# timsainb/noisereduce

Measured on AMD Instinct MI355X. Metric: Msamples/s reduce_noise (48 kHz mono, n_fft=1024), higher is better.
Workload: dtype f32

## Files before the change

include/mi355gate_debug.h:

```cpp
#ifndef MI355GATE_DEBUG_H
#define MI355GATE_DEBUG_H

#include "mi355gate.h"

#ifdef __cplusplus
extern "C" {
#endif

SG_API int sg_debug_dims(const sg_handle* h, int64_t dims[3]);
SG_API int sg_debug_range(const sg_handle* h, int64_t range[2]);
SG_API int sg_debug_counter(sg_handle* h, int32_t which, int64_t* value, void* stream);
SG_API int sg_debug_fetch(sg_handle* h, int32_t what, void* host, int64_t bytes, void* stream);

SG_API int sg_debug_clip_thresholds(sg_handle* h, double* host, int32_t n_noise, int32_t n_bins, void* stream);
SG_API int sg_debug_clip_batches(const sg_handle* h, int64_t* value);
SG_API int sg_debug_rows_batches(const sg_handle* h, int64_t* value);
#define SG_BWD_ROW 1
#define SG_BWD_FAST 2
#define SG_BWD_REG 3
#define SG_BWD_OLA 4
#define SG_BWD_ROWS 5
SG_API int sg_debug_backward_route(const sg_handle* h, int64_t* value);

#define SG_OPT_FORCE_UNFUSED 1
#define SG_OPT_FORCE_F64_DECIDE 3
#define SG_OPT_FORCE_NOSEAM 4
#define SG_OPT_FORCE_NOLEAN 5
#define SG_OPT_FORCE_SPLIT 6
#define SG_OPT_INJECT_HANDOFF_FAULT 7
#define SG_OPT_FORCE_NOROWGATE 10
#define SG_OPT_ROWGATE_TAP 11
#define SG_OPT_ROWGATE_SHAPE 12
#define SG_OPT_FLOOR_TEST 13
#define SG_OPT_TILE_ORDER 15
#define SG_OPT_EXACT_MATERIALISED 16
#define SG_OPT_FORCE_NOFAST 2

#define SG_STAGE_CHANNEL_MEAN 0
#define SG_STAGE_STFT_POWER 1
#define SG_STAGE_COLMAX 2
#define SG_STAGE_COLSTATS 3
#define SG_STAGE_DECIDE 4
#define SG_STAGE_STFT_MAG 5
#define SG_STAGE_NONSTAT_MASK 6
#define SG_STAGE_SMOOTH 7
#define SG_STAGE_APPLY_ISTFT 8
#define SG_STAGE_OLA 9
#define SG_STAGE_NOISE_STATS 10
#define SG_STAGE_PREP 11
#define SG_STAGE_STFT_MAX 12
#define SG_STAGE_STFT_BITS 13
#define SG_STAGE_APPLY_FAST 14
#define SG_STAGE_DECIDE_FAST 15
#define SG_STAGE_ONEPASS 16
#define SG_STAGE_ROW_GATE 17
#define SG_STAGE_IIR_CHAIN 18
#define SG_STAGE_IIR_MASK 19
#define SG_STAGE_RG_NOISE_POWER 20
#define SG_STAGE_RG_NOISE_FINAL 21
#define SG_STAGE_RG_DECIDE 22
#define SG_STAGE_RG_IIR 23
#define SG_STAGE_RG_FSMOOTH 24
#define SG_STAGE_RG_APPLY 25
#define SG_STAGE_RG_OLA 26
#define SG_N_STAGES 27
#define SG_STAGE_ST_EXPORT 27
#define SG_STAGE_ST_IMPORT 28
#define SG_N_STAGES_ALL 29
SG_API int sg_profile_enable(sg_handle* h, int32_t on);
SG_API int sg_profile_select(sg_handle* h, int64_t stage_mask);
SG_API int sg_profile_read(sg_handle* h, double* ms, int64_t* counts, int32_t n_stages, int32_t reset);
SG_API const char* sg_stage_name(int32_t stage);

#ifdef __cplusplus
}
#endif
#endif
```

noisereduce_amd/_ffi.py:

```python
import contextlib
import ctypes
import os
import threading
import weakref
from ctypes import (POINTER, Structure, byref, c_char_p, c_double, c_int, c_int32,
                    c_int64, c_void_p)

import numpy as np
import torch

_HERE = os.path.dirname(os.path.abspath(__file__))
LIB_PATH = os.path.join(_HERE, "libmi355gate.so")

SG_F32, SG_F64, SG_I16, SG_I32 = 0, 1, 2, 3
SG_VARIANT_S, SG_VARIANT_T = 0, 1
SG_E_INVALID, SG_E_UNSUPPORTED, SG_E_HIP, SG_E_NOMEM, SG_E_STATE, SG_E_HANDOFF = -1, -2, -3, -4, -5, -6
SG_N_STAGES = 27
SG_N_STAGES_ALL = 29
SG_OPT_FORCE_F64_DECIDE = 3
SG_OPT_FORCE_NOSEAM = 4
SG_OPT_FORCE_NOLEAN = 5
SG_OPT_FORCE_SPLIT = 6
SG_OPT_INJECT_HANDOFF_FAULT = 7
SG_OPT_FAST_INTEGER = 8
SG_OPT_FORCE_EXACT = 9
SG_OPT_FORCE_NOROWGATE = 10
SG_OPT_ROWGATE_TAP = 11
SG_OPT_ROWGATE_SHAPE = 12
SG_OPT_FLOOR_TEST = 13
SG_OPT_TILE_ORDER = 15
SG_OPT_EXACT_MATERIALISED = 16
SG_OPT_FORCE_UNFUSED = 1
SG_OPT_FORCE_NOFAST = 2
SG_BWD_ROW, SG_BWD_FAST, SG_BWD_REG, SG_BWD_OLA, SG_BWD_ROWS = 1, 2, 3, 4, 5

_TORCH_DTYPES = {torch.float32: SG_F32, torch.float64: SG_F64, torch.int16: SG_I16,
                 torch.int32: SG_I32}


class HandoffTimeout(RuntimeError):
    """SG_E_HANDOFF: a bounded inter-workgroup wait of a fused kernel timed out (the device was preempted for
    about a second); the outputs of the calls enqueued since the last check are invalid and must be re-run."""


class SgParams(Structure):
    _fields_ = [
        ("variant", c_int32), ("stationary", c_int32), ("n_fft", c_int32),
        ("win_length", c_int32), ("hop_length", c_int32), ("n_grad_freq", c_int32),
        ("n_grad_time", c_int32), ("smooth_mask", c_int32), ("chunk_size", c_int64),
        ("padding", c_int64), ("prop_decrease", c_double), ("n_std_thresh", c_double),
        ("top_db", c_double), ("ddof", c_int32), ("n_movemean", c_int32),
        ("nonstat_thresh", c_double), ("nonstat_slope", c_double), ("iir_b", c_double),
        ("max_workspace_bytes", c_int64),
    ]


class SgClip(Structure):
    _fields_ = [("x_offset", c_int64), ("n", c_int64), ("x_stride", c_int64), ("channels", c_int32),
                ("noise", c_int32), ("out_offset", c_int64), ("out_stride", c_int64)]


class SgNoiseSrc(Structure):
    _fields_ = [("offset", c_int64), ("n", c_int64), ("stride", c_int64), ("channels", c_int32), ("in_x", c_int32)]


class SgStreamRec(Structure):
    _fields_ = [("slot", c_int32), ("flush", c_int32), ("n_samples", c_int64), ("in_offset", c_int64),
                ("in_stride", c_int64), ("out_offset", c_int64), ("out_stride", c_int64)]


SG_STREAM_FIXED, SG_STREAM_NONSTATIONARY, SG_STREAM_ADAPTIVE = 0, 1, 2


class SgStreamDesc(Structure):
    _fields_ = [("n_slots", c_int32), ("channels", c_int32), ("max_block", c_int64), ("kind", c_int32),
                ("lookahead_frames", c_int32), ("forget", c_double), ("learn_frames", c_int64), ("exact", c_int32)]


SG_STREAM_HEAD_MAGIC, SG_STREAM_HEAD_VERSION = 0x54534753, 1


class SgStreamHead(Structure):
    _fields_ = [("magic", c_int32), ("version", c_int32), ("n_fft", c_int32), ("win_length", c_int32),
                ("hop_length", c_int32), ("channels", c_int32), ("kind", c_int32), ("n_grad_freq", c_int32),
# ... 707 lines not shown
```

noisereduce_amd/csrc/api.hip:

```cpp
#include <hip/hip_runtime.h>
#include <dlfcn.h>

#include <algorithm>
#include <cmath>
#include <cstdarg>
#include <cstdio>
#include <cstring>
#include <map>
#include <mutex>
#include <string>
#include <vector>

#include "../../include/mi355gate_debug.h"
#pragma clang fp contract(on)
#include "kernels.hpp"
#include "fused.hpp"
#include "czt.hpp"
#include "mixed.hpp"
#include "onepass.hpp"
#include "rowgate.hpp"
#include "rowbwd.hpp"
#include "fast512.hpp"
#include "onepass512.hpp"
#include "fast256.hpp"
// ... 11 lines not shown

#ifndef SG_TEAM_N
#define SG_TEAM_N 2048
#endif
#ifndef SG_SHORT_TEAMS
#define SG_SHORT_TEAMS 1
#endif
#ifndef SG_CHAIN_PAR
#define SG_CHAIN_PAR 1
#if OP_WHO
static unsigned* g_who_dev = nullptr;
#endif
#if OP_TRACE
static unsigned* g_trace_dev = nullptr;
static size_t g_trace_tiles = 0;
static int g_trace_ntt = 1;
#endif
#endif
#ifndef SG_STATS_TEAM
#define SG_STATS_TEAM 1
#endif
template <int N>
constexpr int team_threads() {
  return N >= SG_TEAM_N ? 256 : (!SG_SHORT_TEAMS ? 64 : (N <= 128 ? 16 : (N == 256 ? 32 : 64)));
}
template <int N>
constexpr int team_count(size_t elem) {
  return N >= SG_TEAM_N ? 1 : (team_threads<N>() < 64 ? 256 / team_threads<N>() : ((N * elem > 16384) ? 2 : 4));
}
#ifndef SG_APPLY_WAVES
#define SG_APPLY_WAVES 4
#endif

using namespace sg;

namespace {
thread_local std::string g_create_error;

struct DevBuf {
  void* p = nullptr;
  size_t bytes = 0;
};

std::string fmt(const char* f, ...) {
  char buf[512];
  va_list ap;
  va_start(ap, f);
  vsnprintf(buf, sizeof buf, f, ap);
  va_end(ap);
  return buf;
}
}

struct RegGeom;
struct sg_handle {
  sg_params p{};
  int n = 0, N = 0, W = 0, H = 0, F = 0, FS = 0, padL = 0;
  double sum_w = 0.0;
  double mag_scale = 1;
  DevBuf tw64, tw32, wfull64, wa32, ws32, wsq32, kf, kt;
  DevBuf thresh;
  bool has_thresh = false;
  DevBuf P, pmax, thr_rows, raw, M, seg, yn;
  DevBuf bits, K16, umax, need, T2;
  DevBuf nss;
  DevBuf alim;
  bool t2_ready = false;
  DevBuf logtab;
  DevBuf part;
  DevBuf tw512, invn;
  DevBuf seam;
  DevBuf ftab;
  int sm2_tt = 64;
  bool t_sm2_ok = true;
  DevBuf xbits, xpart, xticket, xtick2, ftab3, xexp, optab;
  DevBuf xin;
  DevBuf nsp, nsc;
  unsigned* err_host = nullptr;
  unsigned* err_dev = nullptr;
  unsigned inject_fault = 0;
  unsigned lose_now = 0;
  unsigned ticket_base = 0;
  unsigned epoch = 0;
  bool fast_integer = false;
  bool force_exact = false;
  bool exact_materialised = false;
  DevBuf norm64;
  unsigned need_era = 0;
  DevBuf xP, xraw, xM, xtmp, xseg;
  bool force_split = false;
  int rowgate_mode = 0;
  int64_t n_floor_lazy = 0, n_floor_apriori = 0;
  int tile_order = 0;
  int n_cu = 0;
  int floor_test = 0;
  int rg_shape = 16;
  bool rg_tap = false;
  bool dbg_rg = false;
  int dbg_bwd_route = 0;
  DevBuf rg_count;
  bool dbg_xbits = false;
  int dbg_trows = 16, dbg_tstep = 16, dbg_twords = 0, dbg_txw = 9;
  int64_t dbg_tf0 = 0;
  int dbg_ntt = 0;
  int big_M = 0;
  int big_czt = 0;
  DevBuf big_twM, big_tw2, big_ch, big_bh, big_W, big_W2;
  int czt_M = 0;
  bool mr_ok = false;
  MrPlan mr{};
  DevBuf mr_pt32, mr_pt64;
  DevBuf regtab;
  DevBuf czt_tw64, czt_ch64, czt_bh64, czt_tw32, czt_ch32, czt_bh32;
  bool force_noseam = false;
  bool force_nolean = false;
  bool fast_ok = false;
  const RegGeom* reg = nullptr;
  bool force_nofast = false;
  bool force_f64_decide = false;
  int64_t ktot = 1;
  bool fused_ok = false;
  double sum_abs_w = 0.0;
  int64_t dbg_units = 0, dbg_T = 0;
  bool dbg_has_P = false;
  bool dbg_has_raw = true;
  bool dbg_fused = false;
  bool dbg_fast = false;
  bool dbg_k16_only = false;
  Geom dbg_g{};
  int64_t dbg_db = 0, dbg_de = 0;
  bool force_unfused = false;
  bool roctx_on = false;
  bool prof_on = false;
  uint64_t prof_mask = ~0ull;
  int prof_override = -1;
// ... 95 lines not shown
    (void)hipEventCreate(&e);
    return e;
  }
  bool ranged = false;
  ProfScope(sg_handle* h_, int stage, hipStream_t st_) : h(h_), st(st_) {
    if (h->roctx_on && roctx().push) {
      roctx().push(sg_stage_name(h->prof_override >= 0 ? h->prof_override : stage));
      ranged = true;
    }
    if (!h->prof_on) return;
    const int booked = h->prof_override >= 0 ? h->prof_override : stage;
    if (!((h->prof_mask >> booked) & 1ull)) return;
    sg_handle::ProfRec r{h->prof_override >= 0 ? h->prof_override : stage, get(h), get(h)};
    (void)hipEventRecord(r.a, st);
    h->prof_live.push_back(r);
    idx = (int)h->prof_live.size() - 1;
  }
  ~ProfScope() {
    if (idx >= 0) (void)hipEventRecord(h->prof_live[idx].b, st);
    if (ranged) roctx().pop();
  }
};
}

#define HIPCHK(h, call)                                                                      \
  do {                                                                                       \
    hipError_t e_ = (call);                                                                  \
    if (e_ != hipSuccess) {                                                                  \
      (h)->err = fmt("%s failed: %s (%s:%d)", #call, hipGetErrorString(e_), __FILE__, __LINE__); \
      (void)hipGetLastError();  \
      return SG_E_HIP;                                                                       \
    }                                                                                        \
  } while (0)

#define FAIL(h, code, ...)      \
  do {                          \
    (h)->err = fmt(__VA_ARGS__); \
    return (code);              \
  } while (0)

static hipError_t set_lds(const void* kern, size_t bytes) {
  static std::mutex mu;
  static std::map<std::pair<int, const void*>, size_t> done;
  int dev = 0;
  (void)hipGetDevice(&dev);
  std::lock_guard<std::mutex> lk(mu);
  size_t& have = done[{dev, kern}];
  if (have >= bytes) return hipSuccess;
  hipError_t e = hipFuncSetAttribute(kern, hipFuncAttributeMaxDynamicSharedMemorySize, (int)bytes);
  if (e == hipSuccess) have = bytes;
  return e;
}

static int ensure(sg_handle* h, DevBuf& b, size_t bytes) {
  if (b.bytes >= bytes) return SG_OK;
  if (b.p) {
    HIPCHK(h, hipDeviceSynchronize());
    HIPCHK(h, hipFree(b.p));
    b.p = nullptr;
    b.bytes = 0;
  }
  hipError_t e = hipMalloc(&b.p, bytes);
  if (e != hipSuccess) {
    b.p = nullptr;
    FAIL(h, SG_E_NOMEM, "workspace allocation of %zu bytes failed: %s", bytes, hipGetErrorString(e));
  }
  b.bytes = bytes;
  return SG_OK;
}

static int ensure_zeroed(sg_handle* h, DevBuf& b, size_t bytes, hipStream_t st, bool* fresh = nullptr) {
  const bool grow = b.bytes < bytes;
  int rc = ensure(h, b, bytes);
  if (rc) return rc;
  if (fresh) *fresh = grow;
  if (grow) HIPCHK(h, hipMemsetAsync(b.p, 0, b.bytes, st));
  return SG_OK;
}

static int upload(sg_handle* h, DevBuf& b, const void* src, size_t bytes) {
  int rc = ensure(h, b, bytes);
  if (rc) return rc;
  HIPCHK(h, hipMemcpy(b.p, src, bytes, hipMemcpyHostToDevice));
  return SG_OK;
}

static void free_buf(DevBuf& b) {
  if (b.p) (void)hipFree(b.p);
  b.p = nullptr;
  b.bytes = 0;
}

static int64_t frames_for(const sg_handle* h, int64_t L) {
  if (h->p.variant == SG_VARIANT_S) return (L + 2 * (int64_t)(h->W / 2) - h->W) / h->H + 1;
  return 1 + (L + 2 * (int64_t)(h->n / 2) - h->n) / h->H;
}
static int64_t outlen_for(const sg_handle* h, int64_t L) {
  int64_t T = frames_for(h, L);
  if (h->p.variant == SG_VARIANT_S) return (T - 1) * h->H + h->W - 2 * (int64_t)(h->W / 2);
  return (T - 1) * (int64_t)h->H + (h->n - 2 * (int64_t)(h->n / 2));
}

static Geom make_geom(const sg_handle* h, int64_t Lp) {
  Geom g;
  g.n = h->n; g.W = h->W; g.H = h->H; g.F = h->F; g.FS = h->FS; g.padL = h->padL;
  g.T = frames_for(h, Lp);
  g.Lout = outlen_for(h, Lp);
  return g;
}
// ... 779 lines not shown
          {&h->tw512, fast::OP_TAB_TW512, 4096}, {&h->tw32, fast::OP_TAB_TW1024, 4096}, {&h->wfull64, fast::OP_TAB_WIN64, 8192},
          {&h->tw64, fast::OP_TAB_TW64, 8192}, {&h->ftab3, fast::OP_TAB_MCONST, 1536}, {&h->xexp, fast::OP_TAB_EXP8, 2048}};
      for (const auto& pt : parts) {
        if (!pt.b->p || pt.b->bytes < pt.bytes) { h->err = "one-pass table arena: a source table is missing"; rc = SG_E_STATE; break; }
        if (hipMemcpy((char*)h->optab.p + pt.off, pt.b->p, pt.bytes, hipMemcpyDeviceToDevice) != hipSuccess) {
          h->err = "one-pass table arena: hipMemcpy failed"; rc = SG_E_HIP; break;
        }
      }
    }
  }
  const RegGeom* rg = h->reg;
  if (!rc && rg && p->smooth_mask && p->n_grad_freq <= rg->op.max_nf && p->n_grad_time <= rg->op.max_nt) {
    const int nf = p->n_grad_freq, nt = p->n_grad_time;
    auto wt = [&](int d) { const int ad = d < 0 ? -d : d; return ad <= nt ? nt + 1 - ad : 0; };
    auto wf = [&](int d) { const int ad = d < 0 ? -d : d; return ad <= nf ? nf + 1 - ad : 0; };
    const bool two = rg == &REG2048;
    const int ex = 64 * (two ? 3 : 1 + rg->tab_kb);
    std::vector<unsigned long long> tb(ex + 256, 0ull);
    for (int l = 0; l < 64; ++l) {
      const int q = l / 16, j = l % 16;
      for (int e = 0; e < 8; ++e) {
        const int k = 8 * q + e;
        const int r1 = e < 4 ? 4 * q + e : 16 + 4 * q + (e - 4);
        if (two) {
          tb[l] |= (unsigned long long)wf(k - 24 - j) << (8 * e);
          tb[64 + l] |= (unsigned long long)wf(k + 8 - j) << (8 * e);
          tb[128 + l] |= (unsigned long long)wt(r1 - nt - j) << (8 * e);
        } else {
          tb[l] |= (unsigned long long)wf(k - 8 - j) << (8 * e);
          for (int b = 0; b < rg->tab_kb; ++b) tb[64 * (1 + b) + l] |= (unsigned long long)wt(32 * b + r1 - nt - j) << (8 * e);
        }
      }
    }
    for (int v = 0; v < 256; ++v)
      for (int e = 0; e < 8; ++e) tb[ex + v] |= (unsigned long long)((v >> e) & 1) << (8 * e);
    rc = upload(h, h->regtab, tb.data(), tb.size() * 8);
  }
  if (!rc) rc = ensure(h, h->thresh, (size_t)h->FS * sizeof(double));
  if (rc) {
    g_create_error = h->err;
    sg_destroy(h);
    return rc;
  }
  *out = h;
  return SG_OK;
}

extern "C" int sg_destroy(sg_handle* h) {
  if (!h) return SG_OK;
  (void)hipDeviceSynchronize();
  for (auto& r : h->prof_live) { (void)hipEventDestroy(r.a); (void)hipEventDestroy(r.b); }
  for (auto e : h->prof_pool) (void)hipEventDestroy(e);
  if (h->err_host) (void)hipHostFree(h->err_host);
  for (DevBuf* b : {&h->tw64, &h->tw32, &h->wfull64, &h->wa32, &h->ws32, &h->wsq32, &h->kf, &h->kt, &h->thresh,
                    &h->P, &h->pmax, &h->thr_rows, &h->raw, &h->M, &h->seg, &h->yn, &h->bits, &h->K16, &h->umax,
                    &h->need, &h->T2, &h->part, &h->tw512, &h->invn, &h->seam, &h->ftab, &h->xbits, &h->xpart,
                    &h->xticket, &h->xtick2, &h->ftab3, &h->xexp, &h->optab, &h->nsp, &h->nsc, &h->xin, &h->czt_tw64, &h->czt_ch64,
                    &h->czt_bh64, &h->czt_tw32, &h->czt_ch32, &h->czt_bh32, &h->logtab, &h->big_twM, &h->big_tw2,
                    &h->big_ch, &h->big_bh, &h->big_W, &h->big_W2, &h->xP, &h->xraw, &h->xM, &h->xtmp, &h->xseg, &h->rg_count, &h->alim, &h->nss, &h->mr_pt32, &h->mr_pt64, &h->regtab})
    free_buf(*b);
  sg::rg_free(h->rg);
  sg::rw_free(h->rw);
  delete h;
  return SG_OK;
}

extern "C" int sg_n_frames(const sg_handle* h, int64_t L, int64_t* n_frames) {
  if (!h || !n_frames) return SG_E_INVALID;
  *n_frames = frames_for(h, L);
  return SG_OK;
}
extern "C" int sg_output_length(const sg_handle* h, int64_t L, int64_t* out_len) {
  if (!h || !out_len) return SG_E_INVALID;
  *out_len = outlen_for(h, L);
  return SG_OK;
}

static int64_t ws_budget(const sg_handle* h) {
  return h->p.max_workspace_bytes > 0 ? h->p.max_workspace_bytes : (int64_t)8 << 30;
}

static size_t unit_bytes(const sg_handle* h, const Geom& g, bool lean) {
  size_t cells = (size_t)g.T * g.FS;
  if (lean) return (size_t)g.T * ((g.F + 63) / 64) * 8 + cells * 2 + (size_t)g.FS * 16 + 64 +
           (size_t)(g.T / 16 + 2) * 6 * 256 * 4;
  return cells * (8 + 4 + 4 + 2) + (size_t)g.T * g.n * 4 + (size_t)g.FS * 16 +
         (size_t)(g.T / NS_TT + 1) * 2 * g.FS * 8 * 2 +
         (size_t)(g.T / 8 + 1) * 2 * g.FS * 8;
}

static int64_t units_per_batch(const sg_handle* h, const Geom& g, int64_t total, bool lean = false) {
  int64_t ub = ws_budget(h) / (int64_t)unit_bytes(h, g, lean);
  ub = std::max<int64_t>(1, std::min<int64_t>(ub, 32768));
  return std::min(ub, total);
}

static int ensure_ws(sg_handle* h, const Geom& g, int64_t ub, bool lean = false) {
  size_t cells = (size_t)ub * g.T * g.FS;
  int rc;
  if (!lean) {
    if ((rc = ensure(h, h->P, cells * 8))) return rc;
    if ((rc = ensure(h, h->raw, cells * 4))) return rc;
    if ((rc = ensure(h, h->M, cells * 4))) return rc;
    if ((rc = ensure(h, h->seg, std::max((size_t)ub * g.T * g.n * 4, cells * 4)))) return rc;
  }
  if ((rc = ensure(h, h->pmax, (size_t)ub * g.FS * 8))) return rc;
  if ((rc = ensure(h, h->thr_rows, (size_t)ub * g.FS * 8))) return rc;
// ... 4 lines not shown
#define SG_STAT_SLICES_MAX 64
#endif
#ifndef SG_STAT_FRAMES_PER_SLICE
#define SG_STAT_FRAMES_PER_SLICE 36
#endif
static int stat_slices(const Geom& g, int64_t ub) {
  int64_t blocks = (int64_t)((g.F + 63) / 64) * ub;
  int64_t nts = (2048 + blocks - 1) / blocks;
  nts = std::max<int64_t>(1, std::min<int64_t>(nts, std::min<int64_t>(SG_STAT_SLICES_MAX, std::max<int64_t>(1, g.T / 16))));
  return (int)nts;
}

static int stage_power(sg_handle* h, const View& v, const Geom& g, int64_t ub, hipStream_t st) {
  if (ub >= 16) {
    HIPCHK(h, hipMemsetAsync(h->pmax.p, 0, (size_t)ub * g.FS * 8, st));
    ProfScope ps(h, SG_STAGE_STFT_POWER, st);
    HIPCHK(h, stft_any<double>(h, v, g, ub, (double*)h->P.p, nullptr, nullptr, 1.0, st,
                               (unsigned long long*)h->pmax.p));
    return SG_OK;
  }
  {
    ProfScope ps(h, SG_STAGE_STFT_POWER, st);
    HIPCHK(h, stft_any<double>(h, v, g, ub, (double*)h->P.p, nullptr, nullptr, 1.0, st));
  }
  ProfScope ps(h, SG_STAGE_COLMAX, st);
  const int nts = stat_slices(g, ub);
  int rc = ensure(h, h->part, (size_t)ub * nts * 2 * g.FS * 8);
  if (rc) return rc;
  dim3 grid((g.F + 63) / 64, (unsigned)ub, nts);
  hipLaunchKernelGGL(k_colmax, grid, dim3(64 * STAT_TG), 0, st, (const double*)h->P.p, g, (double*)h->part.p);
  HIPCHK(h, hipGetLastError());
  hipLaunchKernelGGL(k_colmax_final, dim3(grid_1d(ub * g.FS, 256)), dim3(256), 0, st, (const double*)h->part.p, g,
                     nts, (double*)h->pmax.p, ub);
  HIPCHK(h, hipGetLastError());
  return SG_OK;
}

static int stage_colstats(sg_handle* h, const Geom& g, int64_t ub, double* thresh_out, hipStream_t st) {
  ProfScope ps(h, SG_STAGE_COLSTATS, st);
  const int nts = stat_slices(g, ub);
  int rc = ensure(h, h->part, (size_t)ub * nts * 2 * g.FS * 8);
  if (rc) return rc;
  dim3 grid((g.F + 63) / 64, (unsigned)ub, nts);
  hipLaunchKernelGGL(k_colstats, grid, dim3(64 * STAT_TG), 0, st, (const double*)h->P.p, g,
                     (const double*)h->pmax.p, h->mag_scale, h->p.top_db, (double*)h->part.p);
  HIPCHK(h, hipGetLastError());
  hipLaunchKernelGGL(k_colstats_final, dim3(grid_1d(ub * g.FS, 256)), dim3(256), 0, st,
                     (const double*)h->part.p, g, nts, (const double*)h->pmax.p, h->mag_scale,
                     h->p.n_std_thresh, h->p.ddof, thresh_out, ub);
  HIPCHK(h, hipGetLastError());
  return SG_OK;
}

static int stage_stats(sg_handle* h, const View& v, const Geom& g, int64_t ub, double* thresh_out, hipStream_t st,
                       bool gate_consts = false) {
  if (ub < 16) {
    {
      ProfScope ps(h, SG_STAGE_STFT_POWER, st);
      HIPCHK(h, stft_any<double>(h, v, g, ub, (double*)h->P.p, nullptr, nullptr, 1.0, st));
    }
    ProfScope ps(h, SG_STAGE_COLSTATS, st);
    const int nts = (int)std::max<int64_t>(1, std::min<int64_t>(std::min(stat_slices(g, ub), STAT_TG * STAT1_MAXS), g.T / SG_STAT_FRAMES_PER_SLICE));
    int rc = ensure(h, h->part, (size_t)ub * nts * STAT1_NP * g.FS * 8);
    if (rc) return rc;
    dim3 grid((g.F + 63) / 64, (unsigned)ub, nts);
    hipLaunchKernelGGL(k_colstats1, grid, dim3(64 * STAT_TG), 0, st, (const double*)h->P.p, g, h->mag_scale,
                       (double*)h->part.p, db_fast_consts(h));
    HIPCHK(h, hipGetLastError());
    GateConsts gc{};
    if (gate_consts && ub == 1 && grid.x <= 62) {
      if ((rc = ensure(h, h->T2, (size_t)g.FS * 8))) return rc;
      if ((rc = ensure_zeroed(h, h->alim, 256, st))) return rc;
      gc.T2 = (double*)h->T2.p; gc.alim_b = (unsigned*)h->alim.p + 2; gc.sum_abs_w = h->sum_abs_w;
    }
    hipLaunchKernelGGL(k_colstats1_final, dim3((unsigned)((g.FS + 63) / 64), (unsigned)ub), dim3(64 * STAT_TG), 0, st,
                       (const double*)h->part.p, (const double*)h->P.p, g, nts, h->mag_scale, h->p.top_db,
                       h->p.n_std_thresh, h->p.ddof, (double*)h->pmax.p, thresh_out, gc);
    HIPCHK(h, hipGetLastError());
    if (gc.T2 != nullptr) h->t2_ready = true;
    return SG_OK;
  }
  int rc = stage_power(h, v, g, ub, st);
  if (rc) return rc;
  return stage_colstats(h, g, ub, thresh_out, st);
}

static int stage_decide(sg_handle* h, const Geom& g, int64_t ub, const double* thresh, int64_t ustride,
                        hipStream_t st) {
  ProfScope ps(h, SG_STAGE_DECIDE, st);
  int64_t cells = ub * g.T * g.FS;
  hipLaunchKernelGGL(k_decide, dim3(grid_1d(cells, 256)), dim3(256), 0, st, (const double*)h->P.p, g,
                     (const double*)h->pmax.p, thresh, ustride, h->mag_scale, h->p.top_db, (float*)h->raw.p, ub);
  HIPCHK(h, hipGetLastError());
  return SG_OK;
}

static int handoff_prepare(sg_handle* h, hipStream_t st);
static int handoff_next_epoch(sg_handle* h, hipStream_t st);
static int stage_prep_floor(sg_handle* h, const View& v, const Geom& g, int64_t ub, ThreshConsts* tc_out, hipStream_t st,
                            const View* v_exact, unsigned* live_host, unsigned stamp);
template <int MODE>
static hipError_t launch_bits_any(const sg_handle* h, const View& v, const Geom& g, int64_t units, const ThreshConsts& tc,
                                  unsigned long long* pmax_bits, unsigned long long* bits, int wpr, hipStream_t st);

static fast::RegArgs reg_args(const sg_handle* h, const RegGeom* r, const View& v, const Geom& g) {
  fast::RegArgs A{};
  A.view = v; A.g = g;
  A.win = (const float*)h->wa32.p;
  A.win64 = (const double*)h->wfull64.p;
  A.tw = (const fast::cf*)(h->*r->tw).p;
  A.tw64 = (const cx<double>*)h->tw64.p;
  A.mag_scale = h->mag_scale; A.top_db = h->p.top_db;
  A.wsq = (const float*)h->wsq32.p;
  A.invn = (const float*)h->invn.p;
  return A;
}

template <typename ARGS>
static hipError_t reg_launch(void (*kern)(ARGS), dim3 grid, size_t lds, hipStream_t st, const ARGS& A) {
  hipError_t e = set_lds(reinterpret_cast<const void*>(kern), lds);
  if (e != hipSuccess) return e;
  hipLaunchKernelGGL(kern, grid, dim3(256), lds, st, A);
  return hipGetLastError();
}

static int stage_decide_reg(sg_handle* h, const RegGeom* r, const View& v, const Geom& g, int64_t ub, const ThreshConsts& tc,
                            unsigned long long* bits, hipStream_t st, const FloorLazy& fl = FloorLazy{}, bool redo = false) {
  ProfScope ps(h, redo ? SG_STAGE_STFT_MAX : SG_STAGE_DECIDE_FAST, st);
  fast::RegArgs A = reg_args(h, r, v, g);
  A.tc = tc;
  A.bits = bits;
  A.fl = fl;
  HIPCHK(h, reg_launch(r->decide[redo], dim3((unsigned)((g.T + r->frames - 1) / r->frames), (unsigned)ub), r->lds, st, A));
// ... 10 lines not shown
  HIPCHK(h, reg_launch(r->mag, dim3((unsigned)((g.T + r->frames - 1) / r->frames), (unsigned)ub), r->lds, st, A));
  return SG_OK;
}

static int launch_seam(sg_handle* h, const RegGeom* r, const fast::RegArgs& A, int64_t ub, hipStream_t st) {
  if (A.n_tiles < 2) return SG_OK;
  fast::SeamArgs S{};
  S.view = A.view; S.g = A.g; S.om = A.om; S.h_begin = A.h_begin; S.h_end = A.h_end; S.normalize = A.normalize;
  S.invn = A.invn; S.wsq = A.wsq; S.part = A.part; S.n_tiles = A.n_tiles;
  hipLaunchKernelGGL(r->seam, dim3((unsigned)(A.n_tiles - 1), (unsigned)ub), dim3(r->hop), 0, st, S);
  HIPCHK(h, hipGetLastError());
  return SG_OK;
}

static int reg_seam_tiles(sg_handle* h, const RegGeom* r, int64_t hb, int64_t he, int64_t ub, fast::RegArgs* A) {
  const int64_t tiles = (he - hb + 3 + r->frames - 1) / r->frames;
  int rc = ensure(h, h->seam, (size_t)ub * tiles * 6 * r->hop * sizeof(float));
  if (rc) return rc;
  A->part = (float*)h->seam.p;
  A->n_tiles = (int)tiles;
  return SG_OK;
}

static int stage_apply_reg(sg_handle* h, const RegGeom* r, const View& v, const Geom& g, int64_t ub, const OutMap& om,
                           const float* mask_f ,
                           int normalize, hipStream_t st) {
  ProfScope ps(h, SG_STAGE_APPLY_FAST, st);
  fast::RegArgs A = reg_args(h, r, v, g);
  A.Mf = mask_f;
  A.K = (const unsigned short*)h->K16.p;
  A.inv_ktot = (float)(1.0 / (double)h->ktot);
  A.om = om;
  A.normalize = normalize;
  A.h_begin = (om.p0 + g.padL) / r->hop;
  A.h_end = (om.p1 - 1 + g.padL) / r->hop + 1;
  const int64_t nh = A.h_end - A.h_begin;
  if (nh <= 0) return SG_OK;
  const int64_t tiles = (nh + 3 + r->frames - 1) / r->frames;
  const bool seam = tiles >= 2 && !h->force_noseam;
  A.n_tiles = (int)tiles;
  int rc;
  if (seam && (rc = reg_seam_tiles(h, r, A.h_begin, A.h_end, ub, &A))) return rc;
  const dim3 grid((unsigned)(seam ? tiles : (nh + r->hops - 1) / r->hops), (unsigned)ub);
  HIPCHK(h, reg_launch(r->apply[mask_f == nullptr], grid, r->lds, st, A));
  if (seam) return launch_seam(h, r, A, ub, st);
  return SG_OK;
}

struct FloorSetup {
  bool lazy = false;
  ThreshConsts tc{};
  FloorLazy fl{};
};
static int floor_setup(sg_handle* h, const Geom& g, int64_t ub, int nb, hipStream_t st, FloorSetup* out) {
  int rc;
  if ((rc = handoff_prepare(h, st))) return rc;
  const unsigned live_stamp = h->err_host[1];
  const unsigned need_tag = h->epoch & 0x3fffffffu;
  const unsigned era = h->epoch >> 30;
  if (era != h->need_era || need_tag == 0u) {
    if (h->need.p) HIPCHK(h, hipMemsetAsync(h->need.p, 0, h->need.bytes, st));
    if (h->alim.p) HIPCHK(h, hipMemsetAsync((char*)h->alim.p + 4, 0, 4, st));
    h->need_era = era;
  }
  FloorSetup f;
  f.lazy = need_tag != 0u &&
           (h->floor_test == 2 || (h->floor_test == 0 && !(live_stamp != 0u && h->epoch - live_stamp <= 16u)));
  if (f.lazy) {
    const int wpr = (g.F + 63) / 64;
    if ((rc = ensure(h, h->bits, (size_t)ub * g.T * wpr * 8))) return rc;
    if ((rc = ensure_zeroed(h, h->need, (size_t)ub * 4, st))) return rc;
    if ((rc = ensure(h, h->T2, (size_t)g.FS * 8))) return rc;
    if ((rc = ensure_zeroed(h, h->alim, 256, st))) return rc;
    if (!h->t2_ready) {
      ProfScope ps(h, SG_STAGE_PREP, st);
      hipLaunchKernelGGL(k_prep_thresh_lazy, dim3(1), dim3(256), 0, st, (const double*)h->thresh.p, g.F, h->mag_scale,
                         h->sum_abs_w, h->p.top_db, (double*)h->T2.p, (unsigned*)h->alim.p, nb);
      HIPCHK(h, hipGetLastError());
      h->t2_ready = true;
    }
    f.tc = ThreshConsts{(const double*)h->T2.p, (const double*)h->thresh.p, (const double*)h->pmax.p, (const int*)h->need.p,
                        need_tag};
    f.fl = FloorLazy{(unsigned*)h->alim.p, nb, h->err_dev + 1, h->epoch};
  }
  *out = f;
  return SG_OK;
}

static bool onepass_small_ok(const sg_handle* h, const Geom& g, const OutMap& om, const OnePassSmall& S, const DevBuf& tab) {
  if (h->force_nofast || h->force_split || h->force_f64_decide || h->force_unfused || !h->fused_ok) return false;
  if (h->p.variant != SG_VARIANT_S || !h->p.stationary || !h->p.smooth_mask) return false;
  if (h->p.n_grad_freq > S.max_nf || h->p.n_grad_time > S.max_nt || g.F != S.F || !tab.p) return false;
  if (h->tile_order == 1) return false;
  const int64_t hb = (om.p0 + g.padL) / S.hop, he = (om.p1 - 1 + g.padL) / S.hop + 1;
  return he > hb;
}
template <typename LAUNCH>
static int stage_onepass_small(sg_handle* h, const View& v, const View& vx, const Geom& g, int64_t ub, const OutMap& om,
                               hipStream_t st, const OnePassSmall& S, fast::OnePassRegArgs P, const DevBuf& tab, LAUNCH launch) {
  int rc;
  FloorSetup fs;
  if ((rc = floor_setup(h, g, ub, (g.FS + 63) / 64, st, &fs))) return rc;
  const bool lazy = fs.lazy;
  ++(lazy ? h->n_floor_lazy : h->n_floor_apriori);
  const int wpr = (g.F + 63) / 64;
  if (!lazy && (rc = stage_prep_floor(h, v, g, ub, &fs.tc, st, &vx, h->err_dev + 1, h->epoch))) return rc;
  const ThreshConsts& tc = fs.tc;
  P.A.tc = tc;
  P.A.fl = fs.fl;
  P.A.inv_ktot = (float)(1.0 / (double)h->ktot);
  P.A.om = om;
  P.A.normalize = 1;
  P.A.h_begin = (om.p0 + g.padL) / S.hop;
  P.A.h_end = (om.p1 - 1 + g.padL) / S.hop + 1;
  const int64_t nh = P.A.h_end - P.A.h_begin;
  const int64_t n_tiles = (nh + S.extra + S.NH - 1) / S.NH, ntt = n_tiles + 2;
  if ((rc = ensure_zeroed(h, h->xbits, (size_t)ub * ntt * S.tile_words * 8, st))) return rc;
  P.xbits = (unsigned long long*)h->xbits.p;
  P.ticket = (unsigned*)h->xticket.p;
  P.ticket_base = h->ticket_base;
  h->ticket_base += (unsigned)(ub * ntt);
  P.epoch = h->epoch;
  const bool lose = (h->lose_now & 3u) != 0;
  P.poll_epoch = lose ? ~h->epoch : h->epoch;
  P.spin_max = lose ? 0 : fast::OP_SPIN_MAX;
  P.err = h->err_dev;
  P.nf = h->p.n_grad_freq; P.nt = h->p.n_grad_time; P.n_tiles = (int)n_tiles;
// ... 378 lines not shown
    D.tw512 = (const fast::cf*)h->tw512.p;
    D.tw1024 = (const fast::cf*)h->tw32.p;
    D.tw64 = (const cx<double>*)h->tw64.p;
    D.tc = tc;
    D.mag_scale = h->mag_scale; D.top_db = h->p.top_db;
    D.bits = (unsigned long long*)h->bits.p;
    D.wpr = wpr;
    D.t_begin = db; D.t_end = de;
    D.quads_per_wave = 1;
    const int64_t quads = (D.t_end - D.t_begin + 3) / 4;
    const int64_t per_block = (int64_t)WAVES * D.quads_per_wave;
    size_t lds = (size_t)(fast::FN + WAVES * fast::WAVE_CX_H) * sizeof(fast::cf) + (T2_FLOATS + 1024) * sizeof(float);
    auto kern = fast::k_decide_fast<WAVES>;
    HIPCHK(h, set_lds(reinterpret_cast<const void*>(kern), lds));
    dim3 grid((unsigned)((quads + per_block - 1) / per_block), (unsigned)ub);
    hipLaunchKernelGGL(kern, grid, dim3(WAVES * 64), lds, st, D);
    HIPCHK(h, hipGetLastError());
  } else if (r) {
    if ((rc = stage_decide_reg(h, r, v, g, ub, tc, (unsigned long long*)h->bits.p, st, fs.fl))) return rc;
  } else if (!h->force_f64_decide) {
    ProfScope ps(h, SG_STAGE_STFT_BITS, st);
    HIPCHK(h, launch_decide_lds(h, v, g, ub, tc, (unsigned long long*)h->bits.p, wpr, st));
  } else {
    ProfScope ps(h, SG_STAGE_STFT_BITS, st);
    HIPCHK(h, launch_bits_any<1>(h, v, g, ub, tc,
                             (unsigned long long*)h->pmax.p, (unsigned long long*)h->bits.p, wpr, st));
  }
  if (lazy) {
    {
      ProfScope ps(h, SG_STAGE_STFT_MAX, st);
      HIPCHK(h, launch_bits_any<0>(h, v, g, ub, tc, (unsigned long long*)h->pmax.p, (unsigned long long*)h->bits.p, wpr, st));
    }
    if ((rc = stage_decide_reg(h, r, v, g, ub, tc, (unsigned long long*)h->bits.p, st, fs.fl, true))) return rc;
  }
  { int rc2 = stage_smooth_bits(h, g, ub, fast, tb, te, st); if (rc2) return rc2; }
  const int nf = h->p.n_grad_freq, nt = h->p.n_grad_time;
  int64_t cells = ub * g.T * g.FS;
  if (fast) return SG_OK;
  if (reg_geom(h) && h->p.prop_decrease == 1.0) return SG_OK;
  h->dbg_k16_only = k16_apply_geom(h) && h->p.prop_decrease == 1.0;
  h->dbg_g = g;
  if (h->dbg_k16_only) return SG_OK;
  hipLaunchKernelGGL(k_k16_to_mask, dim3(grid_1d(cells / 8, 256)), dim3(256), 0, st, (const unsigned short*)h->K16.p,
                     g, nf, nt, 1.0f / (float)h->ktot, (float)h->p.prop_decrease, 1, h->p.smooth_mask ? 1 : 0,
                     (float*)h->M.p, ub);
  HIPCHK(h, hipGetLastError());
  return SG_OK;
}

static int handoff_next_epoch(sg_handle* h, hipStream_t st) {
  if (++h->epoch == 0) {
    if (h->xbits.p) HIPCHK(h, hipMemsetAsync(h->xbits.p, 0, h->xbits.bytes, st));
    if (h->xpart.p) HIPCHK(h, hipMemsetAsync(h->xpart.p, 0, h->xpart.bytes, st));
    h->epoch = 1;
    if (h->err_host) h->err_host[1] = 0u;
  }
  return SG_OK;
}

static int handoff_prepare(sg_handle* h, hipStream_t st) {
  {
    bool fresh = false;
    int rc = ensure_zeroed(h, h->xticket, 64, st, &fresh);
    if (rc) return rc;
    if (fresh) h->ticket_base = 0;
  }
  if (!h->err_host) {
    HIPCHK(h, hipHostMalloc((void**)&h->err_host, 64, hipHostMallocMapped));
    *h->err_host = 0u;
    h->err_host[1] = 0u;
    HIPCHK(h, hipHostGetDevicePointer((void**)&h->err_dev, h->err_host, 0));
  }
  if (*h->err_host != 0u) {
    const unsigned e = *h->err_host;
    *h->err_host = 0u;
    FAIL(h, SG_E_HANDOFF, "a tile hand-off of an EARLIER call on this handle timed out (code %u): that call's output "
                          "is invalid (call sg_check_errors after a call to learn about it in time)", e);
  }
  h->lose_now = 0;
  if (h->inject_fault) {
    *h->err_host = h->inject_fault & 7u;
    h->lose_now = (h->inject_fault >> 3) & 7u;
    h->inject_fault = 0;
  }
  return handoff_next_epoch(h, st);
}

static int handoff_verdict(sg_handle* h) {
  if (h->err_host && *h->err_host != 0u) {
    const unsigned e = *h->err_host;
    *h->err_host = 0u;
    FAIL(h, SG_E_HANDOFF, "a tile hand-off timed out (code %u: %s%s%s): the output of the call(s) enqueued since the "
                          "last check is invalid; re-run them (SG_OPT_FORCE_SPLIT + SG_OPT_FORCE_NOLEAN select the "
                          "kernels without in-launch hand-offs)",
         e, (e & 1u) ? "mask bits " : "", (e & 2u) ? "partial hops (one-pass gate) " : "",
         (e & 4u) ? "partial hops (fused apply)" : "");
  }
  return SG_OK;
}

extern "C" int sg_check_errors(sg_handle* h, void* stream) {
  if (!h) return SG_E_INVALID;
  HIPCHK(h, hipStreamSynchronize((hipStream_t)stream));
  return handoff_verdict(h);
}

static int stage_apply_fast(sg_handle* h, const View& v, const Geom& g, int64_t ub, const OutMap& om,
                            const float* mask_f , int normalize,
                            hipStream_t st) {
  ProfScope ps(h, SG_STAGE_APPLY_FAST, st);
  constexpr int WAVES = SG_APPLY_WAVES;
  fast::ApplyArgs A;
  A.view = v; A.g = g; A.om = om;
  A.K = (const unsigned short*)h->K16.p;
  A.Mf = mask_f;
  A.normalize = normalize;
  A.win = (const float*)h->wa32.p;
  A.wsq = (const float*)h->wsq32.p;
  A.invn = (const float*)h->invn.p;
  A.tw512 = (const fast::cf*)h->tw512.p;
  A.tw1024 = (const fast::cf*)h->tw32.p;
  A.kscale = mask_f ? (float)(1.0 / 512.0) : (float)(1.0 / ((double)h->ktot * 512.0));
  A.h_begin = (om.p0 + g.padL) / 256;
  A.h_end = (om.p1 - 1 + g.padL) / 256 + 1;
  const int64_t nh = A.h_end - A.h_begin;
  if (nh <= 0) return SG_OK;
  constexpr int NF = 4 * WAVES, NH = NF - 3;
  size_t lds = (size_t)(fast::FN + WAVES * fast::WAVE_CX) * sizeof(fast::cf);
  const int64_t tiles_seam = (nh + 3 + NF - 1) / NF;
  const bool seam = !h->force_noseam && tiles_seam >= 2;
  const bool lean = !h->force_nolean;
  const bool inkernel = seam && lean;
  A.part = nullptr;
  A.part2 = nullptr;
  A.epoch = 0;
  A.err = nullptr;
  A.n_tiles = 0;
  A.ticket = nullptr;
  if (inkernel) {
    int rc = ensure_zeroed(h, h->xpart, (size_t)ub * tiles_seam * 3 * 256 * 8, st);
    if (rc) return rc;
    if ((rc = handoff_prepare(h, st))) return rc;
    A.part2 = (unsigned long long*)h->xpart.p;
    A.epoch = h->epoch;
    A.err = h->err_dev;
    A.n_tiles = (int)tiles_seam;
    if ((rc = ensure_zeroed(h, h->xtick2, (size_t)ub * 64, st))) return rc;
    A.ticket = (unsigned*)h->xtick2.p;
  } else if (seam) {
    int rc = ensure(h, h->seam, (size_t)ub * tiles_seam * 6 * 256 * sizeof(float));
    if (rc) return rc;
    A.part = (float*)h->seam.p;
    A.n_tiles = (int)tiles_seam;
  }
  dim3 grid((unsigned)(seam ? tiles_seam : (nh + NH - 1) / NH), (unsigned)ub);
  auto go = [&](auto kern, size_t lds_bytes) -> hipError_t {
    hipError_t e = set_lds(reinterpret_cast<const void*>(kern), lds_bytes);
    if (e != hipSuccess) return e;
    hipLaunchKernelGGL(kern, grid, dim3(WAVES * 64), lds_bytes, st, A);
    return hipGetLastError();
  };
  const size_t lds_lean = (size_t)(fast::FN + WAVES * fast::WAVE_CX_H) * sizeof(fast::cf) + 1024 * sizeof(float) + 16;
  const bool lose = inkernel && (h->lose_now & 4u);
  if (mask_f) {
    if (lose) HIPCHK(h, go(fast::k_apply_fast<WAVES, false, true, true>, lds_lean));
    else if (lean) HIPCHK(h, go(fast::k_apply_fast<WAVES, false, true>, lds_lean));
    else HIPCHK(h, go(fast::k_apply_fast<WAVES, false, false>, lds));
  } else {
    if (lose) HIPCHK(h, go(fast::k_apply_fast<WAVES, true, true, true>, lds_lean));
    else if (lean) HIPCHK(h, go(fast::k_apply_fast<WAVES, true, true>, lds_lean));
    else HIPCHK(h, go(fast::k_apply_fast<WAVES, true, false>, lds));
  }
  HIPCHK(h, hipGetLastError());
  if (seam && !inkernel) {
    hipLaunchKernelGGL(fast::k_ola_seam<NF>, dim3((unsigned)(tiles_seam - 1), (unsigned)ub), dim3(256), 0, st, A);
    HIPCHK(h, hipGetLastError());
  }
  return SG_OK;
}

static bool onepass_ok(const sg_handle* h, const Geom& g, const OutMap& om) {
  if (h->force_split || h->force_f64_decide || h->force_noseam || h->force_nolean) return false;
  if (!h->p.smooth_mask || h->p.n_grad_freq > 8 || h->p.n_grad_time > fast::OP_MAX_NT || !h->ftab3.p || !h->optab.p) return false;
  if (g.F != 513) return false;
  const int64_t hb = (om.p0 + g.padL) / 256, he = (om.p1 - 1 + g.padL) / 256 + 1;
  return (he - hb + 3 + 15) / 16 >= 2;
}

static int stage_onepass(sg_handle* h, const View& v, const View& vx, const Geom& g, int64_t ub, const OutMap& om,
                         hipStream_t st) {
  constexpr int WAVES = 4, NF = 16;
  int rc;
  FloorSetup fs;
  if ((rc = floor_setup(h, g, ub, OP_ALIM_BLOCKS, st, &fs))) return rc;
  const bool lazy = fs.lazy;
  const ThreshConsts& tc = fs.tc;
  ++(lazy ? h->n_floor_lazy : h->n_floor_apriori);
  if (!lazy && (rc = stage_prep_floor(h, v, g, ub, &fs.tc, st, &vx, h->err_dev + 1, h->epoch))) return rc;
  fast::OnePassArgs P;
  P.x_exact = vx.x; P.stride_exact = vx.stride; P.dtype_exact = vx.dtype;
  fast::ApplyArgs& A = P.A;
  A.view = v; A.g = g; A.om = om;
  A.K = nullptr; A.Mf = nullptr;
  A.normalize = 1;
  A.win = (const float*)h->wa32.p;
  A.wsq = (const float*)h->wsq32.p;
  A.invn = (const float*)h->invn.p;
  A.tw512 = (const fast::cf*)h->tw512.p;
  A.tw1024 = (const fast::cf*)h->tw32.p;
  const bool prop = h->p.prop_decrease != 1.0;
  A.kscale = prop ? (float)(1.0 / 512.0) : (float)(1.0 / ((double)h->ktot * 512.0));
  A.h_begin = (om.p0 + g.padL) / 256;
  A.h_end = (om.p1 - 1 + g.padL) / 256 + 1;
  const int64_t nh = A.h_end - A.h_begin;
  const int64_t n_tiles = (nh + 3 + NF - 1) / NF;
  const int64_t ntt = n_tiles + 2;
  if ((rc = ensure_zeroed(h, h->xpart, (size_t)ub * n_tiles * 3 * 256 * 8, st))) return rc;
  A.part = nullptr;
  A.part2 = nullptr;
  A.epoch = 0;
  A.err = nullptr;
  A.n_tiles = (int)n_tiles;
  if ((rc = ensure_zeroed(h, h->xbits, (size_t)ub * ntt * fast::OP_TILE_WORDS * 8, st))) return rc;
  P.alim = lazy ? (unsigned*)h->alim.p : nullptr;
  {
    constexpr int64_t SPAN = (NF - 1) * 256 + 1024;
    const int64_t sp0 = (A.h_begin - 3 - NF) * 256 - g.padL, sp1 = (A.h_begin - 3 + n_tiles * NF) * 256 - g.padL + SPAN;
    const int64_t inside = std::max<int64_t>(0, std::min<int64_t>(v.Lp, sp1) - std::max<int64_t>(0, sp0));
    const int64_t q = (v.Lp - inside + ntt - 1) / ntt;
    if (q > 0x7fffffff) FAIL(h, SG_E_UNSUPPORTED, "one-pass gate: window of %lld samples", (long long)v.Lp);
    P.scan_q = (int)q;
  }
  P.tab = (const char*)h->optab.p;
  P.tc = tc;
  P.mag_scale = h->mag_scale; P.top_db = h->p.top_db;
  P.xbits = (unsigned long long*)h->xbits.p;
  P.part2 = (unsigned long long*)h->xpart.p;
  P.ticket = (unsigned*)h->xticket.p;
  P.epoch = h->epoch;
  P.err = h->err_dev;
  P.ticket_base = h->ticket_base;
  const bool persist = lazy && h->tile_order == 0 && !(h->lose_now & 3u) && ub * ntt >= 2;
  if (persist && h->n_cu == 0) {
    int dev = 0, cus = 0;
    HIPCHK(h, hipGetDevice(&dev));
    HIPCHK(h, hipDeviceGetAttribute(&cus, hipDeviceAttributeMultiprocessorCount, dev));
    h->n_cu = cus > 0 ? cus : 256;
  }
  static const int pg_per_cu = [] { const char* e = getenv("SG_ONEPASS_WG_PER_CU"); int v = e ? atoi(e) : 3; return v >= 1 && v <= 3 ? v : 3; }();
#if OP_MAX_ITERS == 1
  const unsigned pgrid = persist ? (unsigned)(ub * ntt) : 0u;
#else
  const unsigned pgrid = persist ? (unsigned)std::min<int64_t>(ub * ntt, (int64_t)pg_per_cu * h->n_cu) : 0u;
#endif
  P.total_tiles = (unsigned)(ub * ntt);
  if (h->tile_order == 1) P.ticket_base = 0xffffffffu;
  else h->ticket_base += (unsigned)(ub * ntt) + (OP_MAX_ITERS == 1 ? 0u : pgrid);
  P.nf = h->p.n_grad_freq; P.nt = h->p.n_grad_time;
  P.prop = (float)h->p.prop_decrease;
  P.inv_ktot = 1.0f / (float)h->ktot;
#if OP_WHO
  if (!g_who_dev) HIPCHK(h, hipMalloc((void**)&g_who_dev, 4096 * 16));
  HIPCHK(h, hipMemsetAsync(g_who_dev, 0, 4096 * 16, st));
  P.who = g_who_dev;
#endif
#if OP_TRACE
  {
    static unsigned* tr = nullptr;
    static size_t tr_slots = 0;
    const size_t slots = (size_t)ub * ntt * 4;
    if (!tr || tr_slots < slots) {
      HIPCHK(h, hipMalloc((void**)&tr, slots * 64));
      tr_slots = slots;
      static unsigned** trp = &tr;
      static size_t* trn = &tr_slots;
      static bool reg = false;
      if (!reg) {
        reg = true;
        atexit([] {
          std::vector<unsigned> hst(*trn * 16);
          if (hipMemcpy(hst.data(), *trp, hst.size() * 4, hipMemcpyDeviceToHost) != hipSuccess) return;
          double sum[14] = {0}, w = 0, mx = 0;
          for (size_t i = 0; i < *trn; ++i) {
            if (hst[i * 16 + 15] != 1u) continue;
            w += 1;
            double tot = 0;
            for (int k = 0; k < 14; ++k) { sum[k] += hst[i * 16 + k]; tot += hst[i * 16 + k]; }
            mx = std::max(mx, tot);
          }
          fprintf(stderr, "[OP_TRACE] completed waves %.0f; average shader cycles per wave and phase:", w);
          double tot = 0;
          for (int k = 0; k < 14; ++k) { fprintf(stderr, " %d:%.0f", k, sum[k] / (w > 0 ? w : 1)); tot += sum[k] / (w > 0 ? w : 1); }
          fprintf(stderr, "  sum %.0f  longest wave %.0f\n", tot, mx);
        });
      }
    }
    HIPCHK(h, hipMemsetAsync(tr, 0, slots * 64, st));
    P.trace = tr;
    g_trace_dev = tr; g_trace_tiles = (size_t)ub * ntt; g_trace_ntt = (int)ntt;
  }
#endif
  {
    ProfScope ps(h, SG_STAGE_ONEPASS, st);
    const size_t lds = (size_t)(fast::FN + WAVES * fast::WAVE_CX_H) * sizeof(fast::cf) + (1024 + T2_FLOATS) * sizeof(float) +
                       256 * 8 + 514 * 8 + 32 + (prop ? 528 : 0);
    auto go = [&](auto kern) -> hipError_t {
      hipError_t e = set_lds(reinterpret_cast<const void*>(kern), lds);
      if (e != hipSuccess) return e;
      hipLaunchKernelGGL(kern, dim3(persist ? pgrid : (unsigned)(ub * ntt)), dim3(WAVES * 64), lds, st, P);
      return hipGetLastError();
    };
    if (persist && prop) HIPCHK(h, go(fast::k_gate_onepass<WAVES, true, false, false, true>));
    else if (persist) HIPCHK(h, go(fast::k_gate_onepass<WAVES, false, false, false, true>));
    else if (h->lose_now & 3u) HIPCHK(h, go(fast::k_gate_onepass<WAVES, false, true>));
    else if (prop) HIPCHK(h, go(fast::k_gate_onepass<WAVES, true>));
    else HIPCHK(h, go(fast::k_gate_onepass<WAVES, false>));
  }
  if (lazy) {
    ProfScope ps(h, SG_STAGE_STFT_MAX, st);
    const int wpr = (g.F + 63) / 64;
    HIPCHK(h, launch_bits_any<0>(h, vx, g, ub, tc,
                             (unsigned long long*)h->pmax.p, (unsigned long long*)h->bits.p, wpr, st));
    if ((rc = handoff_next_epoch(h, st))) return rc;
    P.epoch = h->epoch;
    P.ticket = (unsigned*)h->xticket.p + 8;
    P.ticket_base = 0;
    const size_t lds = (size_t)(fast::FN + WAVES * fast::WAVE_CX_H) * sizeof(fast::cf) + (1024 + T2_FLOATS) * sizeof(float) +
                       256 * 8 + 514 * 8 + 32 + (prop ? 528 : 0);
    auto redo = [&](auto kern) -> hipError_t {
      hipError_t e = set_lds(reinterpret_cast<const void*>(kern), lds);
      if (e != hipSuccess) return e;
      hipLaunchKernelGGL(kern, dim3((unsigned)(ub * ntt)), dim3(WAVES * 64), lds, st, P);
      return hipGetLastError();
    };
    if (prop) HIPCHK(h, redo(fast::k_gate_onepass<WAVES, true, false, true>));
    else HIPCHK(h, redo(fast::k_gate_onepass<WAVES, false, false, true>));
    HIPCHK(h, hipGetLastError());
  }
  h->dbg_xbits = true;
  h->dbg_trows = 16; h->dbg_tstep = 16; h->dbg_twords = fast::OP_TILE_WORDS; h->dbg_txw = fast::OP_XW;
  h->dbg_tf0 = A.h_begin - 3;
  h->dbg_ntt = (int)ntt;
  h->dbg_db = std::max<int64_t>(0, A.h_begin - 3 - NF);
  h->dbg_de = std::min<int64_t>(g.T, A.h_begin - 3 + NF * (n_tiles + 1));
  return SG_OK;
}

template <int WAVES, bool KMASK>
static hipError_t launch_apply_fast64(fast::Apply64Args& A, int64_t nh, int64_t ub, hipStream_t st) {
  constexpr int NH = 4 * WAVES - 3;
  const size_t lds = (size_t)(fast::FN + WAVES * 4 * fast::FSLOTS_D + 17) * sizeof(fast::cd);
  auto kern = fast::k_apply_fast64<WAVES, KMASK>;
  hipError_t e = set_lds(reinterpret_cast<const void*>(kern), lds);
  if (e != hipSuccess) return e;
  hipLaunchKernelGGL(kern, dim3((unsigned)((nh + NH - 1) / NH), (unsigned)ub), dim3(WAVES * 64), lds, st, A);
  return hipGetLastError();
}

static int stage_apply_fast64(sg_handle* h, const View& v, const Geom& g, int64_t ub, const OutMap& om, hipStream_t st,
                              const double* mask_f64 = nullptr) {
  ProfScope ps(h, SG_STAGE_APPLY_FAST, st);
  fast::Apply64Args A;
  A.view = v; A.g = g; A.om = om;
  A.K = (const unsigned short*)h->K16.p;
  A.Mf = mask_f64;
  A.win = (const double*)h->wfull64.p;
  A.norm = (const double*)h->norm64.p;
  A.tw1024 = (const fast::cd*)h->tw64.p;
  A.kscale = mask_f64 ? 1.0 / 512.0 : 1.0 / ((double)h->ktot * 512.0);
  A.prop = h->p.prop_decrease;
  A.nf = h->p.smooth_mask ? h->p.n_grad_freq : 0;
  A.nt = h->p.smooth_mask ? h->p.n_grad_time : 0;
  A.h_begin = (om.p0 + g.padL) / 256;
  A.h_end = (om.p1 - 1 + g.padL) / 256 + 1;
  const int64_t nh = A.h_end - A.h_begin;
  if (nh <= 0) return SG_OK;
  static const int waves_env = getenv("SG_APPLY64_WAVES") ? atoi(getenv("SG_APPLY64_WAVES")) : 0;
  const bool wide = waves_env ? waves_env == 8 : nh >= 64;
  if (mask_f64) {
// ... 159 lines not shown
        else
          hipLaunchKernelGGL(exact::kx_prop_only<double>, gr, dim3(256), 0, st, (const double*)h->xraw.p, g, p, (double*)h->xM.p, nb);
      } else if (!h->exact_materialised && exact::xsm_lds_bytes(nf, nt) <= 150 * 1024 && 2 * nf < exact::XSM_KMAX && 2 * nt < exact::XSM_KMAX && nb <= 65535 &&
                 (g.T + exact::XSM_TT - 1) / exact::XSM_TT <= 65535) {
        const size_t lds = exact::xsm_lds_bytes(nf, nt);
        const dim3 gt((unsigned)((g.F + exact::XSM_FB - 1) / exact::XSM_FB), (unsigned)((g.T + exact::XSM_TT - 1) / exact::XSM_TT), (unsigned)nb);
        if (h->p.stationary) {
          auto kern = exact::kx_smooth_tiled<float>;
          HIPCHK(h, set_lds(reinterpret_cast<const void*>(kern), lds));
          hipLaunchKernelGGL(kern, gt, dim3(exact::XSM_THREADS), lds, st, (const float*)h->xraw.p, g, nf, nt, p, prop_before, (double*)h->xM.p);
        } else {
          auto kern = exact::kx_smooth_tiled<double>;
          HIPCHK(h, set_lds(reinterpret_cast<const void*>(kern), lds));
          hipLaunchKernelGGL(kern, gt, dim3(exact::XSM_THREADS), lds, st, (const double*)h->xraw.p, g, nf, nt, p, prop_before, (double*)h->xM.p);
        }
      } else {
        if (h->p.stationary)
          hipLaunchKernelGGL(exact::kx_smooth_f<float>, gr, dim3(256), 0, st, (const float*)h->xraw.p, g, nf, (double*)h->xtmp.p, nb);
        else
          hipLaunchKernelGGL(exact::kx_smooth_f<double>, gr, dim3(256), 0, st, (const double*)h->xraw.p, g, nf, (double*)h->xtmp.p, nb);
        HIPCHK(h, hipGetLastError());
        hipLaunchKernelGGL(exact::kx_smooth_t, gr, dim3(256), 0, st, (const double*)h->xtmp.p, g, nt, nf, p, prop_before,
                           (double*)h->xM.p, nb);
      }
      HIPCHK(h, hipGetLastError());
    }
    if (apply64) {
      if ((rc = stage_apply_fast64(h, v, g, nb, om, st, (const double*)h->xM.p))) return rc;
      h->dbg_units = 0;
      continue;
    }
    {
      ProfScope ps(h, SG_STAGE_APPLY_ISTFT, st);
      HIPCHK(h, xapply_any(h, v, g, nb, (const double*)h->xM.p, (double*)h->xseg.p, st));
    }
    const int64_t np = om.p1 - om.p0;
    if (np > 0) {
      ProfScope ps(h, SG_STAGE_OLA, st);
      hipLaunchKernelGGL(exact::kx_ola, dim3((unsigned)((np + 255) / 256), (unsigned)nb), dim3(256), 0, st, v, g, om,
                         (const double*)h->xseg.p, (const double*)h->wfull64.p);
      HIPCHK(h, hipGetLastError());
    }
    h->dbg_units = 0;
  }
  return SG_OK;
}

static int run_S(sg_handle* h, View v, int64_t total_units, const OutMap& om, hipStream_t st) {
  Geom g = make_geom(h, v.Lp);
  if (v.Lp < h->W) FAIL(h, SG_E_INVALID, "signal window of %lld samples is shorter than win_length=%d",
                        (long long)v.Lp, h->W);
  if (h->p.stationary && !h->has_thresh)
    FAIL(h, SG_E_STATE, "stationary gate: call sg_noise_stats or sg_set_noise_threshold first");
  if (h->force_exact || ((om.dtype == SG_I16 || om.dtype == SG_I32) && !h->fast_integer))
    return exact_fused_ok(h, g) ? run_S_exact_fused(h, v, total_units, om, st) : run_S_exact(h, v, total_units, om, st);
  const bool onepass = h->fused_ok && !h->force_unfused && h->fast_ok && !h->force_nofast && onepass_ok(h, g, om);
  const RegGeom* r = reg_geom(h);
  const bool onepass_r = r && onepass_reg_ok(h, r, g, om);
  const bool lean = onepass || onepass_r || (h->fused_ok && !h->force_unfused && h->fast_ok && !h->force_nofast &&
                                             h->p.prop_decrease == 1.0);
  int64_t ub = units_per_batch(h, g, total_units, lean);
  int rc = ensure_ws(h, g, ub, lean);
  if (rc) return rc;
  const View vx = v;
  if (v.dtype != SG_F32 && ((h->fast_ok && !h->force_nofast && (onepass || (!h->p.stationary && nonstat2_ok(h, g)))) || onepass_r)) {
    const int64_t rows = total_units / std::max<int64_t>(1, v.n_chunks), len = v.hi - v.lo;
    const size_t bytes = (size_t)rows * len * sizeof(float);
    if (len > 0 && bytes <= ((size_t)16 << 30)) {
      if ((rc = ensure(h, h->xin, bytes))) return rc;
      ProfScope ps(h, SG_STAGE_PREP, st);
      hipLaunchKernelGGL(k_to_f32, dim3(grid_1d(rows * len, 256)), dim3(256), 0, st, v.x, v.dtype, v.stride, v.lo, len, rows,
                         (float*)h->xin.p);
      HIPCHK(h, hipGetLastError());
      v.x = (const float*)h->xin.p - v.lo;
      v.dtype = SG_F32;
      v.stride = len;
    }
  }
  for (int64_t u0 = 0; u0 < total_units; u0 += ub) {
    int64_t nb = std::min(ub, total_units - u0);
    v.unit0 = u0;
    const bool fused = h->fused_ok && !h->force_unfused;
    const bool geom_fast = h->fast_ok && !h->force_nofast;
    const bool fast = fused && geom_fast && h->p.prop_decrease == 1.0;
    if (onepass) {
      View vxb = vx;
      vxb.unit0 = u0;
      if ((rc = stage_onepass(h, v, vxb, g, nb, om, st))) return rc;
      h->dbg_units = nb; h->dbg_T = g.T; h->dbg_has_P = false; h->dbg_fused = true; h->dbg_fast = true;
      continue;
    }
    if (onepass_r) {
      View vxb = vx;
      vxb.unit0 = u0;
      if ((rc = stage_onepass_reg(h, r, v, vxb, g, nb, om, st))) return rc;
      h->dbg_units = nb; h->dbg_T = g.T; h->dbg_has_P = false; h->dbg_fused = true; h->dbg_fast = true; h->dbg_k16_only = false;
      continue;
    }
    if (fast) {
      const int64_t hb = (om.p0 + g.padL) / 256, he = (om.p1 - 1 + g.padL) / 256 + 1;
      const int64_t tb = std::max<int64_t>(0, hb - 3), te = std::min<int64_t>(g.T, he);
      if ((rc = stage_fused_mask(h, v, g, nb, true, tb, std::max(te, tb + 1), st))) return rc;
      if ((rc = stage_apply_fast(h, v, g, nb, om, nullptr, 1, st))) return rc;
      h->dbg_units = nb; h->dbg_T = g.T; h->dbg_has_P = false; h->dbg_fused = true; h->dbg_fast = true;
      continue;
    }
    h->dbg_fast = geom_fast || (fused && r && h->p.prop_decrease == 1.0);
    if (fused) {
      if ((rc = stage_fused_mask(h, v, g, nb, false, 0, g.T, st))) return rc;
    } else {
      if (h->p.stationary) {
        if ((rc = stage_power(h, v, g, nb, st))) return rc;
        if ((rc = stage_decide(h, g, nb, (const double*)h->thresh.p, 0, st))) return rc;
      } else if (nonstat2_ok(h, g)) {
        if ((rc = stage_nonstat_mask2(h, v, g, nb, true, st))) return rc;
      } else if (nonstat2_chain_ok(h, g)) {
// ... 102 lines not shown
    hipLaunchKernelGGL((fast::k_row_gate<8, 2>), dim3((unsigned)nb), dim3(512), lds, st, A);
  } else {
    HIPCHK(h, set_lds(reinterpret_cast<const void*>(fast::k_row_gate<16, 1>), lds));
    hipLaunchKernelGGL((fast::k_row_gate<16, 1>), dim3((unsigned)nb), dim3(1024), lds, st, A);
  }
  HIPCHK(h, hipGetLastError());
  return SG_OK;
}

static bool dtype_ok(int d) { return d >= SG_F32 && d <= SG_I32; }

extern "C" int sg_workspace_bytes(const sg_handle* h, int64_t C, int64_t N, int32_t chunked, int64_t* bytes) {
  if (!h || !bytes || C < 1 || N < 1) return SG_E_INVALID;
  const int64_t cs = h->p.chunk_size, pad = h->p.padding;
  const int64_t Lp = chunked ? cs + 2 * pad : N + 2 * pad;
  const int64_t units = chunked ? C * ((N + cs - 1) / cs) : C;
  if (Lp < h->W) return SG_E_INVALID;
  const Geom g = make_geom(h, Lp);
  const bool geom_fast = h->fast_ok && !h->force_nofast;
  const bool onepass = h->p.variant == SG_VARIANT_S && h->fused_ok && !h->force_unfused && geom_fast && !h->force_split &&
                       !h->force_f64_decide && !h->force_noseam && !h->force_nolean && h->p.smooth_mask &&
                       h->p.n_grad_freq <= 8 && h->p.n_grad_time <= fast::OP_MAX_NT && h->ftab3.p != nullptr;
  const bool lean = h->p.variant == SG_VARIANT_S && h->fused_ok && !h->force_unfused && geom_fast &&
                    (onepass || h->p.prop_decrease == 1.0);
  const int64_t ub = units_per_batch(h, g, units, lean);
  int64_t total = ub * (int64_t)unit_bytes(h, g, lean);
  if (geom_fast) {
    const int64_t kept = chunked ? cs : N;
    const int64_t n_tiles = (kept / 256 + 1 + 3 + 15) / 16 + 1;
    total += ub * n_tiles * 3 * 256 * 8 + ub * 64;
    if (onepass) total += ub * (n_tiles + 2) * (int64_t)fast::OP_TILE_WORDS * 8;
    total += C * N * (int64_t)sizeof(float);
  }
  if (h->big_M) {
    const int64_t nb = big_batch(h, units * g.T);
    total += 2 * nb * (int64_t)h->big_M * (int64_t)sizeof(big::cd);
  }
  if (h->p.variant == SG_VARIANT_S && (h->force_exact || !h->fast_integer)) {
    int64_t ex = exact_units_per_batch(h, g, units) * (int64_t)exact_unit_bytes(g);
    if (h->big_M) ex += 2 * big_batch(h, units * g.T) * (int64_t)h->big_M * (int64_t)sizeof(big::cd);
    if (h->force_exact) total = ex;
    else total = std::max(total, ex);
  }
  *bytes = total;
  return SG_OK;
}

extern "C" int sg_noise_stats(sg_handle* h, const void* noise_dev, int dtype, int64_t C, int64_t n,
                              int64_t row_stride, void* stream) {
  if (!h) return SG_E_INVALID;
  if (!noise_dev || !dtype_ok(dtype) || C < 1 || n < 1) FAIL(h, SG_E_INVALID, "sg_noise_stats: bad argument");
  if (h->p.variant != SG_VARIANT_S) FAIL(h, SG_E_INVALID, "sg_noise_stats is a variant-S entry point");
  if (n < h->W) FAIL(h, SG_E_INVALID, "noise clip of %lld samples is shorter than win_length=%d", (long long)n, h->W);
#ifdef SG_EXP_SKIP_STATS
  if (h->has_thresh && h->t2_ready) return SG_OK;
#endif
  hipStream_t st = (hipStream_t)stream;
  struct Tag {
    sg_handle* h;
    explicit Tag(sg_handle* h_) : h(h_) { h->prof_override = SG_STAGE_NOISE_STATS; }
    ~Tag() { h->prof_override = -1; }
  } tag(h);
  int rc = SG_OK;
  View v{};
  v.x = noise_dev; v.dtype = dtype; v.stride = row_stride;
  if (C > 1) {
    if ((rc = ensure(h, h->yn, (size_t)n * sizeof(double)))) return rc;
    ProfScope ps(h, SG_STAGE_CHANNEL_MEAN, st);
    hipLaunchKernelGGL(k_channel_mean, dim3(grid_1d(n, 256)), dim3(256), 0, st, noise_dev, dtype, C, n,
                       row_stride, (double*)h->yn.p);
    HIPCHK(h, hipGetLastError());
    v.x = h->yn.p; v.dtype = SG_F64; v.stride = n;
  }
  v.N = n; v.lo = 0; v.hi = n; v.cs = 0; v.pad = 0; v.Lp = n; v.n_chunks = 1; v.unit0 = 0;
  Geom g = make_geom(h, n);
  if ((rc = ensure_ws(h, g, 1))) return rc;
  h->t2_ready = false;
  if ((rc = stage_stats(h, v, g, 1, (double*)h->thresh.p, st, h->fast_ok || h->reg))) return rc;
  h->has_thresh = true;
  return SG_OK;
}

extern "C" int sg_get_noise_threshold(sg_handle* h, double* thresh_host, int32_t n_bins, void* stream) {
  if (!h) return SG_E_INVALID;
  if (!thresh_host || n_bins != h->F) FAIL(h, SG_E_INVALID, "sg_get_noise_threshold: n_bins must be %d", h->F);
  if (!h->has_thresh) FAIL(h, SG_E_STATE, "no noise threshold set");
  HIPCHK(h, hipMemcpyAsync(thresh_host, h->thresh.p, (size_t)h->F * sizeof(double), hipMemcpyDeviceToHost,
                           (hipStream_t)stream));
  HIPCHK(h, hipStreamSynchronize((hipStream_t)stream));
  return handoff_verdict(h);
}

extern "C" int sg_set_noise_threshold(sg_handle* h, const double* thresh_host, int32_t n_bins, void* stream) {
  if (!h) return SG_E_INVALID;
  if (!thresh_host || n_bins != h->F) FAIL(h, SG_E_INVALID, "sg_set_noise_threshold: n_bins must be %d", h->F);
  h->t2_ready = false;
  HIPCHK(h, hipMemcpyAsync(h->thresh.p, thresh_host, (size_t)h->F * sizeof(double), hipMemcpyHostToDevice,
                           (hipStream_t)stream));
  HIPCHK(h, hipStreamSynchronize((hipStream_t)stream));
  h->has_thresh = true;
  return SG_OK;
}

extern "C" int sg_get_noise_threshold_dev(sg_handle* h, double* thresh_dev, int32_t n_bins, void* stream) {
  if (!h) return SG_E_INVALID;
  if (!thresh_dev || n_bins != h->F) FAIL(h, SG_E_INVALID, "sg_get_noise_threshold_dev: n_bins must be %d", h->F);
  if (!h->has_thresh) FAIL(h, SG_E_STATE, "no noise threshold set");
  HIPCHK(h, hipMemcpyAsync(thresh_dev, h->thresh.p, (size_t)h->F * sizeof(double), hipMemcpyDeviceToDevice,
                           (hipStream_t)stream));
  return SG_OK;
}

extern "C" int sg_set_noise_threshold_dev(sg_handle* h, const double* thresh_dev, int32_t n_bins, void* stream) {
  if (!h) return SG_E_INVALID;
  if (!thresh_dev || n_bins != h->F) FAIL(h, SG_E_INVALID, "sg_set_noise_threshold_dev: n_bins must be %d", h->F);
  h->t2_ready = false;
  HIPCHK(h, hipMemcpyAsync(h->thresh.p, thresh_dev, (size_t)h->F * sizeof(double), hipMemcpyDeviceToDevice,
                           (hipStream_t)stream));
  h->has_thresh = true;
  return SG_OK;
}

extern "C" int sg_process_chunks(sg_handle* h, const void* in_dev, int in_dtype, void* out_dev, int out_dtype,
                                 int64_t C, int64_t N, int64_t in_stride, int64_t out_stride,
                                 int64_t start_frame, int64_t end_frame, int32_t chunked, int64_t halo_left,
                                 int64_t halo_right, void* stream) {
  if (!h) return SG_E_INVALID;
  if (h->p.variant != SG_VARIANT_S) FAIL(h, SG_E_INVALID, "sg_process_chunks is a variant-S entry point");
  if (!in_dev || !out_dev || !dtype_ok(in_dtype) || !dtype_ok(out_dtype) || C < 1 || N < 1)
    FAIL(h, SG_E_INVALID, "sg_process_chunks: bad argument");
  if (start_frame < 0 || end_frame > N || start_frame >= end_frame)
    FAIL(h, SG_E_INVALID, "sg_process_chunks: bad frame range [%lld, %lld)", (long long)start_frame,
         (long long)end_frame);
  const int64_t cs = h->p.chunk_size, pad = h->p.padding;
  if (halo_left < 0 || halo_right < 0) FAIL(h, SG_E_INVALID, "sg_process_chunks: negative halo");
  View v{};
  v.x = in_dev; v.dtype = in_dtype; v.stride = in_stride; v.N = N; v.pad = pad;
  v.lo = -halo_left; v.hi = N + halo_right;
  OutMap om{};
  om.out = out_dev; om.dtype = out_dtype; om.stride = out_stride; om.g0 = start_frame;
  om.g_lo = start_frame; om.g_hi = end_frame;
  int64_t units;
  if (chunked) {
    int64_t ich1 = start_frame / cs, ich2 = (end_frame - 1) / cs;
    int64_t n_chunks = ich2 - ich1 + 1;
    v.cs = cs; v.Lp = cs + 2 * pad; v.n_chunks = (int32_t)n_chunks; v.c0 = ich1;
    om.p0 = pad; om.p1 = pad + cs; om.g_step = cs;
    units = C * n_chunks;
  } else {
    v.cs = 0; v.Lp = end_frame + 2 * pad; v.n_chunks = 1;
    om.p0 = pad; om.p1 = pad + end_frame; om.g_step = 0;
    om.g_lo = 0; om.g0 = 0;
    units = C;
  }
  return run_S(h, v, units, om, (hipStream_t)stream);
}

extern "C" int sg_filter_padded(sg_handle* h, const void* chunk_dev, int in_dtype, void* out_dev, int out_dtype,
                                int64_t C, int64_t Lp, int64_t in_stride, int64_t out_stride, void* stream) {
  if (!h) return SG_E_INVALID;
  if (h->p.variant != SG_VARIANT_S) FAIL(h, SG_E_INVALID, "sg_filter_padded is a variant-S entry point");
  if (!chunk_dev || !out_dev || !dtype_ok(in_dtype) || !dtype_ok(out_dtype) || C < 1 || Lp < 1)
    FAIL(h, SG_E_INVALID, "sg_filter_padded: bad argument");
  View v{};
  v.x = chunk_dev; v.dtype = in_dtype; v.stride = in_stride; v.N = Lp; v.lo = 0; v.hi = Lp; v.cs = 0; v.pad = 0; v.Lp = Lp; v.n_chunks = 1;
  OutMap om{};
  om.out = out_dev; om.dtype = out_dtype; om.stride = out_stride;
  om.p0 = 0; om.p1 = Lp; om.g_step = 0; om.g0 = 0; om.g_lo = 0; om.g_hi = Lp;
// ... 176 lines not shown
    HIPCHK(h, hipGetLastError());
    return SG_OK;
  }
  int64_t ub = units_per_batch(h, g, B);
  rc = ensure_ws(h, g, ub);
  if (rc) return rc;
  if ((rc = ensure(h, h->yn, (size_t)ub * Lq * sizeof(float)))) return rc;
  for (int64_t u0 = 0; u0 < B; u0 += ub) {
    const int64_t nb = std::min(ub, B - u0);
    {
      dim3 grid((unsigned)((Lq + 255) / 256), (unsigned)nb);
      const char* src = (const char*)grad_out_dev + (size_t)u0 * go_stride * (dtype == SG_F64 ? 8 : 4);
      hipLaunchKernelGGL(k_env_scale, grid, dim3(256), 0, st, (const void*)src, dtype, go_stride, g,
                         (const float*)h->wsq32.p, (float*)h->yn.p, Lq);
      HIPCHK(h, hipGetLastError());
    }
    View v{};
    v.x = h->yn.p; v.dtype = SG_F32; v.stride = Lq; v.N = Lq; v.lo = 0; v.hi = Lq; v.cs = 0; v.pad = 0; v.Lp = Lq;
    v.n_chunks = 1; v.unit0 = 0;
    Geom gb = g;
    gb.Lout = L;
    OutMap om{};
    om.out = (char*)grad_x_dev + (size_t)u0 * gx_stride * (dtype == SG_F64 ? 8 : 4);
    om.dtype = dtype; om.stride = gx_stride;
    om.p0 = 0; om.p1 = L; om.g_step = 0; om.g0 = 0; om.g_lo = 0; om.g_hi = L;
    const float* mk = mask_dev + (size_t)u0 * g.T * g.FS;
    if (h->fast_ok && !h->force_nofast) {
      h->dbg_bwd_route = SG_BWD_FAST;
      if ((rc = stage_apply_fast(h, v, gb, nb, om, mk, 0, st))) return rc;
    } else if (const RegGeom* r = reg_geom(h)) {
      h->dbg_bwd_route = SG_BWD_REG;
      if ((rc = stage_apply_reg(h, r, v, gb, nb, om, mk, 0, st))) return rc;
    } else {
      h->dbg_bwd_route = SG_BWD_OLA;
      if ((rc = stage_apply_ola(h, v, gb, nb, mk, om, 0, st))) return rc;
    }
  }
  return SG_OK;
}

extern "C" int sg_stft(sg_handle* h, const void* x_dev, int dtype, int64_t B, int64_t L, int64_t stride,
                       double* z_dev, void* stream) {
  if (!h) return SG_E_INVALID;
  if (!x_dev || !z_dev || !dtype_ok(dtype) || B < 1 || L < h->W) FAIL(h, SG_E_INVALID, "sg_stft: bad argument");
  View v{};
  v.x = x_dev; v.dtype = dtype; v.stride = stride; v.N = L; v.lo = 0; v.hi = L; v.cs = 0; v.pad = 0; v.Lp = L; v.n_chunks = 1; v.unit0 = 0;
  Geom g = make_geom(h, L);
  HIPCHK(h, stft_any<double>(h, v, g, B, nullptr, nullptr, z_dev, h->mag_scale, (hipStream_t)stream));
  return SG_OK;
}

extern "C" int sg_set_option(sg_handle* h, int32_t option, int64_t value) {
  if (!h) return SG_E_INVALID;
  switch (option) {
    case SG_OPT_FORCE_UNFUSED: h->force_unfused = value != 0; return SG_OK;
    case SG_OPT_FORCE_NOFAST: h->force_nofast = value != 0; return SG_OK;
    case SG_OPT_FORCE_F64_DECIDE: h->force_f64_decide = value != 0; return SG_OK;
    case SG_OPT_FORCE_NOSEAM: h->force_noseam = value != 0; return SG_OK;
    case SG_OPT_FORCE_NOLEAN: h->force_nolean = value != 0; return SG_OK;
    case SG_OPT_FORCE_SPLIT: h->force_split = value != 0; return SG_OK;
    case SG_OPT_FAST_INTEGER: h->fast_integer = value != 0; return SG_OK;
    case SG_OPT_FORCE_EXACT: h->force_exact = value != 0; return SG_OK;
    case SG_OPT_FORCE_NOROWGATE:
      if (value < 0 || value > 2) FAIL(h, SG_E_INVALID, "SG_OPT_FORCE_NOROWGATE: 0 (auto), 1 (never) or 2 (always)");
      h->rowgate_mode = (int)value;
      return SG_OK;
    case SG_OPT_ROWGATE_TAP: h->rg_tap = value != 0; return SG_OK;
    case SG_OPT_ROWGATE_SHAPE:
      if (value != 8 && value != 16) FAIL(h, SG_E_INVALID, "SG_OPT_ROWGATE_SHAPE: 8 or 16 waves");
      h->rg_shape = (int)value;
      return SG_OK;
    case SG_OPT_INJECT_HANDOFF_FAULT: h->inject_fault = (unsigned)value & 63u; return SG_OK;
    case SG_OPT_TILE_ORDER:
      if (value < 0 || value > 2) FAIL(h, SG_E_INVALID, "SG_OPT_TILE_ORDER: 0 (persistent workgroups), 1 (block index) or 2 (one ticket per workgroup)");
      h->tile_order = (int)value;
      return SG_OK;
    case SG_OPT_EXACT_MATERIALISED: h->exact_materialised = value != 0; return SG_OK;
    case SG_OPT_FLOOR_TEST:
      if (value < 0 || value > 2) FAIL(h, SG_E_INVALID, "SG_OPT_FLOOR_TEST: 0 (predicted), 1 (a priori) or 2 (in the gate kernel)");
      h->floor_test = (int)value;
      return SG_OK;
  }
  FAIL(h, SG_E_INVALID, "sg_set_option: unknown option %d", option);
}

extern "C" int sg_get_option(const sg_handle* h, int32_t option, int64_t* value) {
  if (!h || !value) return SG_E_INVALID;
  switch (option) {
    case SG_OPT_FORCE_UNFUSED: *value = h->force_unfused; return SG_OK;
    case SG_OPT_FORCE_NOFAST: *value = h->force_nofast; return SG_OK;
    case SG_OPT_FORCE_F64_DECIDE: *value = h->force_f64_decide; return SG_OK;
    case SG_OPT_FORCE_NOSEAM: *value = h->force_noseam; return SG_OK;
    case SG_OPT_FORCE_NOLEAN: *value = h->force_nolean; return SG_OK;
    case SG_OPT_FORCE_SPLIT: *value = h->force_split; return SG_OK;
    case SG_OPT_FAST_INTEGER: *value = h->fast_integer; return SG_OK;
    case SG_OPT_FORCE_EXACT: *value = h->force_exact; return SG_OK;
    case SG_OPT_FORCE_NOROWGATE: *value = h->rowgate_mode; return SG_OK;
    case SG_OPT_ROWGATE_TAP: *value = h->rg_tap; return SG_OK;
    case SG_OPT_ROWGATE_SHAPE: *value = h->rg_shape; return SG_OK;
    case SG_OPT_INJECT_HANDOFF_FAULT: *value = h->inject_fault; return SG_OK;
    case SG_OPT_TILE_ORDER: *value = h->tile_order; return SG_OK;
    case SG_OPT_EXACT_MATERIALISED: *value = h->exact_materialised; return SG_OK;
    case SG_OPT_FLOOR_TEST: *value = h->floor_test; return SG_OK;
  }
  return SG_E_INVALID;
}

extern "C" int sg_profile_enable(sg_handle* h, int32_t on) {
  if (!h) return SG_E_INVALID;
  h->prof_on = on != 0;
  return SG_OK;
}

extern "C" int sg_profile_select(sg_handle* h, int64_t stage_mask) {
  if (!h) return SG_E_INVALID;
  h->prof_mask = stage_mask == 0 ? ~0ull : (uint64_t)stage_mask;
  return SG_OK;
}

extern "C" int sg_profile_read(sg_handle* h, double* ms, int64_t* counts, int32_t n_stages, int32_t reset) {
  if (!h) return SG_E_INVALID;
  if (n_stages != SG_N_STAGES && n_stages != SG_N_STAGES_ALL)
    FAIL(h, SG_E_INVALID, "sg_profile_read: n_stages must be %d (or %d)", SG_N_STAGES, SG_N_STAGES_ALL);
  for (auto& r : h->prof_live) {
    HIPCHK(h, hipEventSynchronize(r.b));
    float t = 0.f;
    HIPCHK(h, hipEventElapsedTime(&t, r.a, r.b));
    h->prof_ms[r.stage] += (double)t;
    h->prof_cnt[r.stage] += 1;
    h->prof_pool.push_back(r.a);
    h->prof_pool.push_back(r.b);
  }
  h->prof_live.clear();
  for (int i = 0; i < SG_N_STAGES_ALL; ++i) {
    if (ms && i < n_stages) ms[i] = h->prof_ms[i];
    if (counts && i < n_stages) counts[i] = h->prof_cnt[i];
    if (reset) { h->prof_ms[i] = 0; h->prof_cnt[i] = 0; }
  }
  return SG_OK;
}

extern "C" const char* sg_stage_name(int32_t stage) {
  static const char* names[SG_N_STAGES_ALL] = {"k_channel_mean", "k_stft<double> (power)", "k_colmax", "k_colstats",
                                           "k_decide", "k_mag_fast* / k_stft<float> (magnitude)",
                                           "k_box_mask / k_iir_sigmoid / k_boxcar_sigmoid (non-stationary mask, other paths)",
                                           "mask smoothing (k_smooth_bits2 / k_smooth_tiled / k_smooth_f+k_smooth_t)",
                                           "k_apply_istft", "k_ola",
                                           "noise statistics (all kernels)", "k_unit_absmax+k_prep_thresh",
                                           "k_stft_bits<max> (floor pre-pass)", "k_stft_bits<decide>",
                                           "k_apply_fast (fft+mask+ifft+ola)",
                                           "k_decide_fast (f32 stft + exact f64 refine)",
                                           "k_gate_onepass (fft+decide+smooth+mask+ifft+ola)",
                                           "k_row_gate (fft+row stats+decide+smooth+mask+ifft+ola)",
                                           "k_iir_chain_par (tile carries; serial: k_iir_part / k_iir_comb + k_iir_chain)",
                                           "k_iir_mask<nt> (recurrence+sigmoid+smoothing)",
                                           "k_rg_noise_power (clips: noise transform)",
                                           "k_rg_noise_final (clips: thresholds)",
                                           "k_rg_decide (clips: transform + bits / magnitudes)",
                                           "k_rg_iir (clips: recurrence + sigmoid)",
                                           "k_rg_fsmooth (clips: frequency smoothing)",
                                           "k_rg_apply (clips: time smoothing + mask + inverse transform)",
                                           "k_rg_ola (clips: overlap-add)",
                                           "k_st_export (stream state -> payload)",
                                           "k_st_import (payload -> stream state)"};
  return (stage >= 0 && stage < SG_N_STAGES_ALL) ? names[stage] : "?";
}

extern "C" int sg_debug_dims(const sg_handle* h, int64_t dims[3]) {
  if (!h || !dims) return SG_E_INVALID;
  dims[0] = h->dbg_units; dims[1] = h->dbg_T; dims[2] = h->FS;
  return SG_OK;
}

extern "C" int sg_debug_range(const sg_handle* h, int64_t range[2]) {
  if (!h || !range) return SG_E_INVALID;
  range[0] = h->dbg_db; range[1] = h->dbg_de;
  return SG_OK;
}

extern "C" int sg_debug_counter(sg_handle* h, int32_t which, int64_t* value, void* stream) {
  if (!h || !value) return SG_E_INVALID;
  if (which == 1 || which == 2) {
    *value = which == 1 ? h->n_floor_lazy : h->n_floor_apriori;
    return SG_OK;
  }
  if (which == 3) {
    HIPCHK(h, hipStreamSynchronize((hipStream_t)stream));
    *value = h->err_host ? (int64_t)h->err_host[1] : 0;
    return SG_OK;
  }
#if OP_TRACE
  if (which == 8) {
    HIPCHK(h, hipStreamSynchronize((hipStream_t)stream));
    std::vector<unsigned> t(g_trace_tiles * 64);
    HIPCHK(h, hipMemcpy(t.data(), g_trace_dev, t.size() * 4, hipMemcpyDeviceToHost));
    int64_t bad = 0;
    auto last_phase = [&](size_t tk, int w) { int lp = -1; for (int k = 0; k < 14; ++k) if (t[(tk * 4 + w) * 16 + k]) lp = k; return lp; };
    for (size_t tk = 0; tk < g_trace_tiles; ++tk) {
      const int jt = (int)(tk % g_trace_ntt) - 1;
      const bool halo = jt < 0 || jt >= g_trace_ntt - 2;
      bool ok = true;
      for (int w = 0; w < 4; ++w) ok = ok && (halo ? last_phase(tk, w) >= 5 : t[(tk * 4 + w) * 16 + 15] == 1u);
      if (ok) continue;
      if (++bad > 8) continue;
      fprintf(stderr, "[trace] ticket %zu (unit %zu tile %d%s):", tk, tk / g_trace_ntt, jt, halo ? " halo" : "");
      for (int w = 0; w < 4; ++w) {
        const unsigned who = t[(tk * 4 + w) * 16 + 14];
        fprintf(stderr, "  w%d wg %d iter %u last phase %d", w, (int)(who & 0xffffu) - 1, who >> 16, last_phase(tk, w));
      }
      fprintf(stderr, "\n");
    }
    *value = bad;
    return SG_OK;
  }
#endif
#if OP_WHO
  if (which == 16) {
    HIPCHK(h, hipStreamSynchronize((hipStream_t)stream));
    std::vector<unsigned> w(4096 * 4);
    HIPCHK(h, hipMemcpy(w.data(), g_who_dev, w.size() * 4, hipMemcpyDeviceToHost));
    const long long T = *value;
    if (T < 0) {
      for (long long t = 0; t < 4096; ++t)
        if (w[t * 4] | w[t * 4 + 2])
          fprintf(stderr, "[whoall] %lld %d %u %u %d %u %u\n", t, (int)(w[t * 4] & 0xffffu) - 1, w[t * 4] >> 16, w[t * 4 + 1], (int)(w[t * 4 + 2] & 0xffffu) - 1, w[t * 4 + 2] >> 16, w[t * 4 + 3]);
      return SG_OK;
    }
    for (long long t = std::max<long long>(0, T - 14); t <= std::min<long long>(4095, T + 3); ++t)
      fprintf(stderr, "[who] ticket %lld: drawn by wg %d (iteration %u) while on tile %u; started by wg %d (iteration %u); past its bits poll: %u\n", t,
              (int)(w[t * 4] & 0xffffu) - 1, w[t * 4] >> 16, w[t * 4 + 1], (int)(w[t * 4 + 2] & 0xffffu) - 1, w[t * 4 + 2] >> 16, w[t * 4 + 3]);
    return SG_OK;
  }
#endif
  if (which >= 4 && which <= 15) {
    HIPCHK(h, hipStreamSynchronize((hipStream_t)stream));
    *value = h->err_host ? (int64_t)h->err_host[which] : 0;
    return SG_OK;
  }
  if (which != 0) FAIL(h, SG_E_INVALID, "sg_debug_counter: unknown counter %d", which);
  *value = 0;
  if (!h->rg_count.p) return SG_OK;
  HIPCHK(h, hipStreamSynchronize((hipStream_t)stream));
  unsigned v = 0;
  HIPCHK(h, hipMemcpy(&v, h->rg_count.p, sizeof(v), hipMemcpyDeviceToHost));
  *value = (int64_t)v;
  return SG_OK;
}

extern "C" int sg_debug_fetch(sg_handle* h, int32_t what, void* host, int64_t bytes, void* stream) {
  if (!h) return SG_E_INVALID;
  if (!host || h->dbg_units == 0) FAIL(h, SG_E_STATE, "sg_debug_fetch: nothing processed yet");
  size_t cells = (size_t)h->dbg_units * h->dbg_T * h->FS;
  const void* src;
  size_t need;
  switch (what) {
    case 0:
      if (h->dbg_fused) FAIL(h, SG_E_STATE, "fused path keeps the raw mask as bits: fetch field 3");
      if (!h->dbg_has_raw)
        FAIL(h, SG_E_STATE, "the one-kernel non-stationary mask does not materialise the raw mask: set SG_OPT_FORCE_UNFUSED");
      src = h->raw.p; need = cells * 4; break;
    case 3:
      if (!h->dbg_fused) FAIL(h, SG_E_STATE, "bit field only exists on the fused path");
      src = h->bits.p; need = (size_t)h->dbg_units * h->dbg_T * ((h->F + 63) / 64) * 8; break;
    case 1:
      if (h->dbg_fast && h->dbg_fused)
        FAIL(h, SG_E_STATE, "fast path keeps the smoothed mask as uint16 counts in the apply kernel's lane order");
      if (h->dbg_fused && h->dbg_k16_only) {
        HIPCHK(h, hipDeviceSynchronize());
        hipLaunchKernelGGL(k_k16_to_mask, dim3(grid_1d((int64_t)cells / 8, 256)), dim3(256), 0, (hipStream_t)stream,
                           (const unsigned short*)h->K16.p, h->dbg_g, h->p.n_grad_freq, h->p.n_grad_time, 1.0f / (float)h->ktot,
                           (float)h->p.prop_decrease, 1, h->p.smooth_mask ? 1 : 0, (float*)h->M.p, (int64_t)h->dbg_units);
        HIPCHK(h, hipGetLastError());
      }
      src = h->M.p; need = cells * 4; break;
    case 2:
      if (!h->dbg_has_P) FAIL(h, SG_E_STATE, "power field only exists for stationary gates");
      src = h->P.p; need = cells * 8; break;
    case 4:
      if (!h->dbg_rg || !h->rg_tap) FAIL(h, SG_E_STATE, "row-gate power tile: set SG_OPT_ROWGATE_TAP and run TorchGate.forward");
      src = h->M.p; need = (size_t)h->dbg_units * 64 * fast::RG_PP * 4; break;
    default: FAIL(h, SG_E_INVALID, "sg_debug_fetch: unknown field %d", what);
  }
  if ((size_t)bytes != need) FAIL(h, SG_E_INVALID, "sg_debug_fetch: need %zu bytes, got %lld", need, (long long)bytes);
  HIPCHK(h, hipStreamSynchronize((hipStream_t)stream));
  { int rc = handoff_verdict(h); if (rc) return rc; }
  if (what == 3 && h->dbg_xbits) {
    const int wpr = (h->F + 63) / 64;
    const int TW = h->dbg_twords ? h->dbg_twords : fast::OP_TILE_WORDS, XW = h->dbg_txw;
    const size_t words = (size_t)h->dbg_units * h->dbg_ntt * TW;
    std::vector<unsigned long long> tmp(words);
    HIPCHK(h, hipMemcpy(tmp.data(), h->xbits.p, words * 8, hipMemcpyDeviceToHost));
    unsigned long long* dst = (unsigned long long*)host;
    std::memset(dst, 0, need);
    for (int64_t u = 0; u < h->dbg_units; ++u)
      for (int64_t j = 0; j < h->dbg_ntt; ++j)
        for (int i = 0; i < h->dbg_trows; ++i) {
          const int64_t t = h->dbg_tf0 + (j - 1) * h->dbg_tstep + i;
          if (t < 0 || t >= h->dbg_T) continue;
          for (int w = 0; w < wpr; ++w)
          {
            const unsigned long long* gr = &tmp[((size_t)u * h->dbg_ntt + j) * TW + (i * XW + w) * 2];
            dst[(u * h->dbg_T + t) * wpr + w] = (gr[0] & 0xffffffffull) | (gr[1] << 32);
          }
        }
    return SG_OK;
  }
  HIPCHK(h, hipMemcpy(host, src, need, hipMemcpyDeviceToHost));
  return SG_OK;
}

static void* rg_prof_begin(void* ctx, int stage, hipStream_t st) { return new ProfScope((sg_handle*)ctx, stage, st); }
static void rg_prof_end(void* tok) { delete (ProfScope*)tok; }

static sg::RgCtx rg_ctx(sg_handle* h) {
  sg::RgCtx c{};
  c.n = h->n; c.N = h->N; c.W = h->W; c.H = h->H; c.F = h->F; c.FS = h->FS; c.padL = h->padL;
  c.mag_scale = h->mag_scale; c.tw64 = h->tw64.p; c.wfull64 = (const double*)h->wfull64.p;
  c.stationary = h->p.stationary; c.cs = h->p.chunk_size; c.pad = h->p.padding;
  c.nf = h->p.smooth_mask ? h->p.n_grad_freq : 0;
  c.nt = h->p.smooth_mask ? h->p.n_grad_time : 0;
  c.prop = h->p.prop_decrease; c.top_db = h->p.top_db; c.n_std = h->p.n_std_thresh; c.iir_b = h->p.iir_b;
  c.nthresh = h->p.nonstat_thresh; c.slope = h->p.nonstat_slope; c.ddof = h->p.ddof;
  c.hook_ctx = h; c.prof_begin = rg_prof_begin; c.prof_end = rg_prof_end;
  return c;
}

static bool rg_variant_ok(sg_handle* h) {
  if (h->p.variant != SG_VARIANT_S) { h->err = "sg_process_clips is a variant-S entry point"; return false; }
  return true;
}

extern "C" int sg_clips_workspace_bytes(const sg_handle* h, const sg_noise_src* noise, int32_t n_noise, const sg_clip* clips,
                                        int64_t n_clips, int64_t* bytes) {
  if (!h || !bytes || n_clips < 0 || (n_clips > 0 && !clips) || n_noise < 0 || (n_noise > 0 && !noise)) return SG_E_INVALID;
  sg_handle* hm = const_cast<sg_handle*>(h);
  if (!rg_variant_ok(hm)) return SG_E_INVALID;
  return sg::rg_workspace_bytes(rg_ctx(hm), noise, n_noise, clips, n_clips, bytes, &hm->err);
}

extern "C" int sg_process_clips(sg_handle* h, const void* x_dev, int in_dtype, const void* noise_dev, int noise_dtype,
                                const sg_noise_src* noise, int32_t n_noise, const sg_clip* clips, int64_t n_clips,
                                void* out_dev, int out_dtype, int64_t max_workspace_bytes, void* stream) {
  if (!h) return SG_E_INVALID;
  if (!rg_variant_ok(h)) return SG_E_INVALID;
  if (n_clips < 0 || (n_clips > 0 && (!clips || !x_dev || !out_dev)) || !dtype_ok(in_dtype) || !dtype_ok(out_dtype) ||
      n_noise < 0 || (n_noise > 0 && !noise) || (h->p.stationary && n_noise > 0 && !dtype_ok(noise_dtype) && noise_dev))
    FAIL(h, SG_E_INVALID, "sg_process_clips: bad argument");
  if (n_clips == 0) return SG_OK;
  return sg::rg_process(&h->rg, rg_ctx(h), x_dev, in_dtype, noise_dev, noise_dtype, noise, n_noise, clips, n_clips, out_dev,
                        out_dtype, max_workspace_bytes, (hipStream_t)stream, &h->err);
}

extern "C" int sg_debug_clip_thresholds(sg_handle* h, double* host, int32_t n_noise, int32_t n_bins, void* stream) {
  if (!h || !host || n_bins != h->F) return SG_E_INVALID;
  return sg::rg_thresholds(h->rg, host, n_noise, n_bins, (hipStream_t)stream, &h->err);
}

extern "C" int sg_debug_clip_batches(const sg_handle* h, int64_t* value) {
  if (!h || !value) return SG_E_INVALID;
  *value = sg::rg_last_batches(h->rg);
  return SG_OK;
}

static int64_t rw_budget(const sg_handle* h) { return h->p.max_workspace_bytes > 0 ? h->p.max_workspace_bytes : 0; }

extern "C" int sg_process_rows(sg_handle* h, const void* x_dev, int dtype, int64_t B, int64_t L, int64_t x_stride,
                               const int64_t* lengths, const void* xn_dev, int64_t Bn, int64_t Ln, int64_t xn_stride,
                               const int64_t* xn_lengths, void* out_dev, int out_dtype, int64_t out_stride,
                               float* mask_out_dev, void* stream) {
  if (!h) return SG_E_INVALID;
  if (h->p.variant != SG_VARIANT_T) FAIL(h, SG_E_INVALID, "sg_process_rows is a variant-T entry point");
  if (!x_dev || !out_dev || (dtype != SG_F32 && dtype != SG_F64) || (out_dtype != SG_F32 && out_dtype != SG_F64) || B < 1 ||
      x_stride < L || out_stride < 0)
    FAIL(h, SG_E_INVALID, "sg_process_rows: bad argument");
  if (L < 2 * (int64_t)h->W) FAIL(h, SG_E_INVALID, "x must be bigger than %d", 2 * h->W);
  if (xn_dev) {
    if (Ln < 2 * (int64_t)h->W) FAIL(h, SG_E_INVALID, "xn must be bigger than %d", 2 * h->W);
    if (Bn != 1 && Bn != B) FAIL(h, SG_E_INVALID, "xn rows (%lld) must be 1 or the batch size", (long long)Bn);
  }
  return sg::rw_process(&h->rw, rg_ctx(h), h->p.n_movemean, x_dev, dtype, B, L, x_stride, lengths, xn_dev, Bn, Ln, xn_stride,
                        xn_lengths, out_dev, out_dtype, out_stride, mask_out_dev, rw_budget(h), (hipStream_t)stream, &h->err);
}

extern "C" int sg_process_rows_backward(sg_handle* h, const void* grad_out_dev, int dtype, int64_t B, int64_t L,
                                        int64_t go_stride, const int64_t* lengths, const float* mask_dev, void* grad_x_dev,
                                        int64_t gx_stride, void* stream) {
  if (!h) return SG_E_INVALID;
  if (h->p.variant != SG_VARIANT_T) FAIL(h, SG_E_INVALID, "sg_process_rows_backward is a variant-T entry point");
  if (!grad_out_dev || !grad_x_dev || !mask_dev || B < 1 || (dtype != SG_F32 && dtype != SG_F64) || gx_stride < L ||
      L < 2 * (int64_t)h->W)
    FAIL(h, SG_E_INVALID, "sg_process_rows_backward: bad argument");
  h->dbg_bwd_route = SG_BWD_ROWS;
  return sg::rw_backward(&h->rw, rg_ctx(h), grad_out_dev, dtype, B, L, go_stride, lengths, mask_dev, grad_x_dev, gx_stride,
                         rw_budget(h), (hipStream_t)stream, &h->err);
}

extern "C" int sg_debug_rows_batches(const sg_handle* h, int64_t* value) {
// ... 69 lines not shown
  if (!h || !bytes || n_slots < 1 || channels < 1 || max_block < 1 || lookahead_frames < 0) return SG_E_INVALID;
  sg_handle* hm = const_cast<sg_handle*>(h);
  *bytes = sg::st_state_bytes(rg_ctx(hm), !h->p.stationary, n_slots, channels, max_block, h->p.stationary ? 0 : lookahead_frames);
  return SG_OK;
}

extern "C" int sg_stream_create_adaptive(sg_handle* h, int32_t n_slots, int32_t channels, int64_t max_block, double forget,
                                         int64_t learn_frames, sg_stream_bank** out) {
  if (!h || !out) return SG_E_INVALID;
  if (h->p.variant != SG_VARIANT_S) FAIL(h, SG_E_INVALID, "sg_stream_create_adaptive is a variant-S entry point");
  sg::StBank* b = nullptr;
  const sg::StAdaptive ad{forget, learn_frames};
  int rc = sg::st_create(&b, rg_ctx(h), n_slots, channels, max_block, false, 0, &ad, false, &h->err);
  if (rc) return rc;
  *out = new sg_stream_bank{h, b};
  return SG_OK;
}

extern "C" int sg_stream_state_bytes_adaptive(const sg_handle* h, int32_t n_slots, int32_t channels, int64_t max_block,
                                              int64_t* bytes) {
  if (!h || !bytes || n_slots < 1 || channels < 1 || max_block < 1 || !h->p.stationary) return SG_E_INVALID;
  sg_handle* hm = const_cast<sg_handle*>(h);
  *bytes = sg::st_state_bytes(rg_ctx(hm), false, n_slots, channels, max_block, 0, true);
  return SG_OK;
}

extern "C" int sg_stream_noise_profile(sg_stream_bank* b, int32_t slot, double* thresh_host, int32_t n_bins, void* stream) {
  if (!b) return SG_E_INVALID;
  sg_handle* h = b->h;
  if (!thresh_host) FAIL(h, SG_E_INVALID, "sg_stream_noise_profile: thresh_host is null");
  if (n_bins != h->F) FAIL(h, SG_E_INVALID, "sg_stream_noise_profile: n_bins must be %d", h->F);
  return sg::st_noise_profile(b->b, slot, thresh_host, (hipStream_t)stream, &h->err);
}

extern "C" int sg_stream_bank_emitted(const sg_stream_bank* b, int64_t n, int64_t* emitted) {
  if (!b || !emitted || n < 0) return SG_E_INVALID;
  *emitted = sg::st_bank_emitted(b->b, n);
  return SG_OK;
}

extern "C" int sg_stream_destroy(sg_stream_bank* b) {
  if (!b) return SG_OK;
  sg::st_destroy(b->b);
  delete b;
  return SG_OK;
}

extern "C" int sg_stream_set_threshold(sg_stream_bank* b, const int32_t* slots, int32_t n_slots, const double* thresh_host,
                                       int32_t n_bins, void* stream) {
  if (!b) return SG_E_INVALID;
  sg_handle* h = b->h;
  if (n_bins != h->F) FAIL(h, SG_E_INVALID, "sg_stream_set_threshold: n_bins must be %d", h->F);
  if (!thresh_host && !h->has_thresh) FAIL(h, SG_E_STATE, "no noise threshold set");
  return sg::st_set_threshold(b->b, slots, n_slots, thresh_host ? nullptr : (const double*)h->thresh.p, thresh_host,
                              (hipStream_t)stream, &h->err);
}

extern "C" int sg_stream_push(sg_stream_bank* b, const void* in_dev, int in_dtype, void* out_dev, int out_dtype,
                              const sg_stream_rec* recs, int32_t n_recs, void* stream) {
  if (!b) return SG_E_INVALID;
  sg_handle* h = b->h;
  if (n_recs < 0 || (n_recs > 0 && !recs) || !dtype_ok(in_dtype) || !dtype_ok(out_dtype))
    FAIL(h, SG_E_INVALID, "sg_stream_push: bad argument (float32 / float64 buffers)");
  return sg::st_push(b->b, in_dev, in_dtype, out_dev, out_dtype, recs, n_recs, (hipStream_t)stream, &h->err);
}

extern "C" int sg_stream_reset(sg_stream_bank* b, const int32_t* slots, int32_t n_slots, void* stream) {
  if (!b) return SG_E_INVALID;
  return sg::st_reset(b->b, slots, n_slots, (hipStream_t)stream, &b->h->err);
}

extern "C" int sg_stream_emitted(const sg_handle* h, int64_t n, int64_t* emitted) {
  if (!h || !emitted || n < 0) return SG_E_INVALID;
  *emitted = sg::st_emitted(h->W, h->H, h->p.smooth_mask ? h->p.n_grad_time : 0, n);
  return SG_OK;
}

extern "C" int sg_stream_counters(const sg_stream_bank* b, int32_t slot, int64_t* n, int64_t* emitted) {
  if (!b || !n || !emitted) return SG_E_INVALID;
  return sg::st_counters(b->b, slot, n, emitted, &b->h->err);
}

static sg_stream_head stream_signature(const sg_handle* h) {
  sg_stream_head s{};
  s.n_fft = h->p.n_fft; s.win_length = h->W; s.hop_length = h->H;
  s.n_grad_freq = h->p.n_grad_freq; s.n_grad_time = h->p.n_grad_time; s.smooth_mask = h->p.smooth_mask ? 1 : 0;
  s.prop_decrease = h->p.prop_decrease; s.n_std_thresh = h->p.n_std_thresh; s.top_db = h->p.top_db;
  s.iir_b = h->p.iir_b; s.nonstat_thresh = h->p.nonstat_thresh; s.nonstat_slope = h->p.nonstat_slope;
  return s;
}

extern "C" int sg_stream_export_bytes(const sg_stream_bank* b, int32_t slot, int64_t* bytes) {
  if (!b || !bytes) return SG_E_INVALID;
  return sg::st_export_bytes(b->b, slot, bytes, &b->h->err);
}

extern "C" int sg_stream_head_bytes(const sg_stream_head* head, int64_t* bytes) {
  if (!head || !bytes) return SG_E_INVALID;
  return sg::st_head_bytes(*head, bytes);
}

extern "C" int sg_stream_export(sg_stream_bank* b, const int32_t* slots, int32_t n_slots, void* blob_dev, const int64_t* offsets,
                                sg_stream_head* heads_out, void* stream) {
  if (!b) return SG_E_INVALID;
  return sg::st_export(b->b, slots, n_slots, blob_dev, offsets, stream_signature(b->h), heads_out, (hipStream_t)stream, &b->h->err);
}
// ... 7 lines not shown
```

noisereduce_amd/csrc/kernels.hpp:

```cpp
#pragma once
#include <hip/hip_runtime.h>
#include <stdint.h>

#include "fft_wave.hpp"
#include "geom.hpp"

namespace sg {


__global__ void k_to_f32(const void* __restrict__ x, int dtype, int64_t stride, int64_t lo, int64_t len, int64_t rows,
                         float* __restrict__ out) {
  const int64_t n = rows * len;
  for (int64_t i = (int64_t)blockIdx.x * blockDim.x + threadIdx.x; i < n; i += (int64_t)gridDim.x * blockDim.x) {
    const int64_t r = i / len, j = i - r * len;
    out[i] = (float)load_sample(x, dtype, r * stride + lo + j);
  }
}

template <typename TC, int N, int WAVES, int FPW, int NT = 64>
__global__ __launch_bounds__(WAVES * NT) void k_stft(View view, Geom g, const cx<TC>* __restrict__ tw_g,
                                                     const TC* __restrict__ wfull,
                                                     double* __restrict__ P_out, float* __restrict__ mag_out,
                                                     double* __restrict__ z_out, double z_scale,
                                                     unsigned long long* __restrict__ pmax_bits) {
// ... 257 lines not shown
    double m = 0.0;
    if (f < g.F) {
#pragma unroll 8
      for (int ts = 0; ts < nts; ++ts) m = nanmax(m, pmax_part[(u * nts + ts) * g.FS + f]);
    }
    pmax[i] = m;
  }
}

__global__ __launch_bounds__(64 * STAT_TG) void k_colstats(const double* __restrict__ P, Geom g,
                                                           const double* __restrict__ pmax, double mag_scale,
                                                           double top_db, double* __restrict__ s_part) {
  __shared__ double r1[STAT_TG][64], r2[STAT_TG][64];
  const int l = threadIdx.x & 63;
  const int f = blockIdx.x * 64 + l;
  const int tg = threadIdx.x >> 6;
  const int64_t u = blockIdx.y;
  const int ts = blockIdx.z, nts = gridDim.z;
  const int64_t tb = g.T * ts / nts, te = g.T * (ts + 1) / nts;
  double s1 = 0.0, s2 = 0.0;
  if (f < g.F) {
    const double mdb = cell_db(pmax[u * g.FS + f], mag_scale);
    for (int64_t t = tb + tg; t < te; t += STAT_TG) {
      double d = cell_db(P[(u * g.T + t) * g.FS + f], mag_scale) - mdb;
      d = (d != d) ? d : fmax(d, -top_db);
      s1 += d;
      s2 += d * d;
    }
  }
  r1[tg][l] = s1;
  r2[tg][l] = s2;
  __syncthreads();
  if (tg == 0 && f < g.F) {
    for (int i = 1; i < STAT_TG; ++i) {
      s1 += r1[i][l];
      s2 += r2[i][l];
    }
    s_part[((u * nts + ts) * 2 + 0) * g.FS + f] = s1;
    s_part[((u * nts + ts) * 2 + 1) * g.FS + f] = s2;
  }
}

constexpr int STAT1_NP = 5;
#ifndef STAT1_BATCH
#define STAT1_BATCH 16
#endif

__device__ __forceinline__ void min2_push(double& m1, double& m2, double x) {
  const double lo = fmin(m1, x), hi = fmax(m1, x);
  m1 = lo;
  m2 = fmin(m2, hi);
}

__global__ __launch_bounds__(64 * STAT_TG) void k_colstats1(const double* __restrict__ P, Geom g, double mag_scale,
                                                            double* __restrict__ part ,
                                                            DbFast dbk) {
  __shared__ double r[STAT1_NP][STAT_TG][64];
  __shared__ __attribute__((aligned(16))) double s_tab[256];
  s_tab[threadIdx.x] = dbk.tab[threadIdx.x];
  __syncthreads();
  const int l = threadIdx.x & 63;
  const int f = blockIdx.x * 64 + l;
  const int tg = threadIdx.x >> 6;
  const int64_t u = blockIdx.y;
  const int ts = blockIdx.z, nts = gridDim.z;
  const int64_t tb = g.T * ts / nts, te = g.T * (ts + 1) / nts;
  double mx = 0.0, m1 = 1e300, m2 = 1e300, s1 = 0.0, s2 = 0.0;
  if (f < g.F) {
    const double* col = P + (u * g.T) * g.FS + f;
    const double p0 = col[0];
    double pivot = 0.0;
    constexpr int NB = STAT1_BATCH;
    for (int64_t t0 = tb + tg; t0 < te; t0 += NB * STAT_TG) {
      double pv[NB];
#pragma unroll
      for (int q = 0; q < NB; ++q) {
        const int64_t t = t0 + q * STAT_TG;
        pv[q] = t < te ? col[t * g.FS] : 0.0;
      }
      if (t0 == tb + tg) pivot = cell_db(p0, mag_scale);
#pragma unroll
      for (int q = 0; q < NB; ++q) {
        if (t0 + q * STAT_TG < te) {
          mx = fmax(mx, pv[q]);
          min2_push(m1, m2, pv[q]);
          const double d = db_fast(pv[q], s_tab, dbk, mag_scale) - pivot;
          s1 += d;
          s2 += d * d;
        }
      }
    }
  }
  r[0][tg][l] = mx; r[1][tg][l] = m1; r[2][tg][l] = m2; r[3][tg][l] = s1; r[4][tg][l] = s2;
  __syncthreads();
  if (tg == 0 && f < g.F) {
    for (int i = 1; i < STAT_TG; ++i) {
      mx = fmax(mx, r[0][i][l]);
      min2_push(m1, m2, r[1][i][l]);
      min2_push(m1, m2, r[2][i][l]);
      s1 += r[3][i][l];
      s2 += r[4][i][l];
    }
    double* o = part + ((u * nts + ts) * STAT1_NP) * (int64_t)g.FS + f;
    o[0] = mx; o[g.FS] = m1; o[2 * g.FS] = m2; o[3 * g.FS] = s1; o[4 * g.FS] = s2;
  }
}

constexpr int STAT1_MAXS = 16;
struct GateConsts {
  double* T2;
  unsigned* alim_b;
  double sum_abs_w;
};
__global__ __launch_bounds__(64 * STAT_TG) void k_colstats1_final(const double* __restrict__ part,
                                                                  const double* __restrict__ P, Geom g, int nts,
                                                                  double mag_scale, double top_db, double n_std,
                                                                  int ddof, double* __restrict__ pmax,
                                                                  double* __restrict__ thresh, GateConsts gc) {
  __shared__ double r[3][STAT_TG][64];
  const int l = threadIdx.x & 63, tg = threadIdx.x >> 6;
  const int f = blockIdx.x * 64 + l;
  const int64_t u = blockIdx.y;
  const int64_t i = u * g.FS + f;
  const bool live = f < g.F;
  const double Tn = (double)g.T;
  double mx = 0.0, s1 = 0.0, s2 = 0.0;
  const double p0 = live ? P[(u * g.T) * g.FS + f] : 1.0;
  double m1[STAT1_MAXS];
  {
    const int fc = live ? f : g.F - 1;
    double a0[STAT1_MAXS], a3[STAT1_MAXS], a4[STAT1_MAXS];
#pragma unroll
    for (int k = 0; k < STAT1_MAXS; ++k) {
      const int ts = tg + STAT_TG * k;
      const double* o = part + ((u * nts + (ts < nts ? ts : nts - 1)) * STAT1_NP) * (int64_t)g.FS + fc;
      a0[k] = o[0];
      m1[k] = o[g.FS];
      a3[k] = o[3 * g.FS];
      a4[k] = o[4 * g.FS];
    }
#pragma unroll
    for (int k = 0; k < STAT1_MAXS; ++k) {
      const bool on = live && tg + STAT_TG * k < nts;
      if (on) {
        mx = fmax(mx, a0[k]);
        s1 += a3[k];
        s2 += a4[k];
      } else {
        m1[k] = 1e300;
      }
    }
  }
  r[0][tg][l] = mx;
  __syncthreads();
#pragma unroll
  for (int k = 0; k < STAT_TG; ++k) mx = fmax(mx, r[0][k][l]);
  const double mdb = cell_db(mx, mag_scale);
  const double pivot = live ? cell_db(p0, mag_scale) : 0.0;
  {
    const double dfl = (mdb - top_db) - pivot;
    const double am = (exp10((mdb - top_db) / 20.0) - 2.220446049250313e-16) / mag_scale;
    const double Pfl = am > 0.0 ? am * am : 0.0;
    unsigned km = 0u;
#pragma unroll
    for (int k = 0; k < STAT1_MAXS; ++k) km |= (m1[k] < Pfl ? 1u : 0u) << k;
    unsigned wor = km;
    for (int off = 32; off > 0; off >>= 1) wor |= (unsigned)__shfl_xor((int)wor, off);
    {
      while (wor) {
        const int k = __ffs((int)wor) - 1;
        wor &= wor - 1u;
        const int ts = tg + STAT_TG * k;
        bool both = false;
        if ((km >> k) & 1u) {
          const double* o = part + ((u * nts + ts) * STAT1_NP) * (int64_t)g.FS + f;
          const double a1 = o[g.FS], a2 = o[2 * g.FS];
          both = a1 < Pfl && a2 < Pfl;
          if (a1 < Pfl && !both) {
            const double d = cell_db(a1, mag_scale) - pivot;
            if (d < dfl) {
              s1 += dfl - d;
              s2 += dfl * dfl - d * d;
            }
          }
        }
        unsigned long long todo = __ballot(both);
        while (todo) {
          const int src = __ffsll((long long)todo) - 1;
          todo &= todo - 1;
          const int fb = blockIdx.x * 64 + src;
          const double Pfl_s = __shfl(Pfl, src), piv_s = __shfl(pivot, src), dfl_s = __shfl(dfl, src);
          const int64_t tb = g.T * ts / nts, te = g.T * (ts + 1) / nts;
          double c1 = 0.0, c2 = 0.0;
          for (int64_t t0 = tb + l; t0 < te; t0 += 64 * 4) {
            double pv[4];
#pragma unroll
            for (int q = 0; q < 4; ++q) {
              const int64_t t = t0 + 64 * q;
              pv[q] = t < te ? P[(u * g.T + t) * g.FS + fb] : 1e300;
            }
#pragma unroll
            for (int q = 0; q < 4; ++q)
              if (pv[q] < Pfl_s) {
                const double d = cell_db(pv[q], mag_scale) - piv_s;
                if (d < dfl_s) {
                  c1 += dfl_s - d;
                  c2 += dfl_s * dfl_s - d * d;
                }
              }
          }
          for (int off = 32; off > 0; off >>= 1) {
            c1 += __shfl_xor(c1, off);
            c2 += __shfl_xor(c2, off);
          }
          if (l == src) {
            s1 += c1;
            s2 += c2;
          }
        }
      }
    }
  }
  __syncthreads();
  r[1][tg][l] = s1; r[2][tg][l] = s2;
  __syncthreads();
  if (tg != 0) return;
  double thr_out = (double)NAN;
  s1 = 0.0; s2 = 0.0;
#pragma unroll
  for (int k = 0; k < STAT_TG; ++k) {
    s1 += r[1][k][l];
    s2 += r[2][k][l];
  }
  if (live) {
    pmax[i] = mx;
    double var = (s2 - s1 * s1 / Tn) / (Tn - (double)ddof);
    if (var < 0.0) var = 0.0;
    thr_out = (pivot + s1 / Tn) + sqrt(var) * n_std;
    thresh[i] = thr_out;
  } else if (f < g.FS) {
    pmax[i] = 0.0;
  }
  if (gc.T2 == nullptr || u != 0) return;
  const double eps = 2.220446049250313e-16;
  double mn = 1e300;
  if (live) {
    const double zero_db = 20.0 * log10(eps);
    double t2;
    if (thr_out != thr_out) {
      t2 = 1e300;
    } else if (zero_db > thr_out) {
      t2 = -1.0;
    } else {
      const double tm = (exp10(thr_out / 20.0) - eps) / mag_scale;
      t2 = tm > 0.0 ? tm * tm : 0.0;
    }
    gc.T2[f] = t2;
    mn = fmin(mn, thr_out);
  }
  for (int off = 32; off > 0; off >>= 1) mn = fmin(mn, __shfl_xor(mn, off));
  if (l == 0) {
    const double lim = (exp10((mn + top_db - 1e-6) / 20.0) - eps) / (gc.sum_abs_w * mag_scale);
    unsigned bits = 0u;
    if (lim > 0.0) bits = __float_as_uint(__double2float_rd(lim * (1.0 - 1e-6)));
    gc.alim_b[blockIdx.x] = bits;
  }
}

__global__ void k_colstats_final(const double* __restrict__ s_part, Geom g, int nts,
                                 const double* __restrict__ pmax, double mag_scale, double n_std, int ddof,
                                 double* __restrict__ thresh, int64_t n_units) {
  const int64_t n = n_units * g.FS;
  for (int64_t i = (int64_t)blockIdx.x * blockDim.x + threadIdx.x; i < n; i += (int64_t)gridDim.x * blockDim.x) {
    const int64_t u = i / g.FS;
    const int f = (int)(i % g.FS);
    if (f >= g.F) continue;
    double s1 = 0.0, s2 = 0.0;
#pragma unroll 8
    for (int ts = 0; ts < nts; ++ts) {
      s1 += s_part[((u * nts + ts) * 2 + 0) * g.FS + f];
      s2 += s_part[((u * nts + ts) * 2 + 1) * g.FS + f];
    }
    const double Tn = (double)g.T;
    const double mean_d = s1 / Tn;
    double var = (s2 - s1 * s1 / Tn) / (Tn - (double)ddof);
    if (var < 0.0) var = 0.0;
    thresh[i] = (cell_db(pmax[i], mag_scale) + mean_d) + sqrt(var) * n_std;
  }
}

__global__ void k_decide(const double* __restrict__ P, Geom g, const double* __restrict__ pmax,
                         const double* __restrict__ thresh, int64_t thresh_ustride, double mag_scale,
                         double top_db, float* __restrict__ raw, int64_t n_units) {
  const int64_t cells = n_units * g.T * g.FS;
  for (int64_t i = (int64_t)blockIdx.x * blockDim.x + threadIdx.x; i < cells;
       i += (int64_t)gridDim.x * blockDim.x) {
    const int f = (int)(i % g.FS);
    if (f >= g.F) continue;
    const int64_t u = i / (g.T * g.FS);
    double db = cell_db(P[i], mag_scale);
    double fl = cell_db(pmax[u * g.FS + f], mag_scale) - top_db;
    db = fmax(db, fl);
    raw[i] = (fl == fl && db > thresh[u * thresh_ustride + f]) ? 1.0f : 0.0f;
  }
}

__global__ void k_t2_rows(const double* __restrict__ thresh, int64_t thresh_ustride, const double* __restrict__ pmax,
                          Geom g, double mag_scale, double top_db, double* __restrict__ T2, int64_t n_units) {
  const double eps = 2.220446049250313e-16;
  const int64_t n = n_units * g.FS;
  for (int64_t i = (int64_t)blockIdx.x * blockDim.x + threadIdx.x; i < n; i += (int64_t)gridDim.x * blockDim.x) {
    const int64_t u = i / g.FS;
    const int f = (int)(i % g.FS);
    double t2 = 0.0;
    if (f < g.F) {
      const double th = thresh[u * thresh_ustride + f];
      const double fl = cell_db(pmax[i], mag_scale) - top_db;
      if (th != th || fl != fl) {
        t2 = 1e300;
// ... 394 lines not shown
```

noisereduce_amd/csrc/onepass.hpp:

```cpp
#pragma once
#include "fastpath.hpp"

namespace sg {
namespace fast {

constexpr int OP_XW = 9;
constexpr int OP_TILE_WORDS = 16 * OP_XW * 2;
constexpr int OP_MAX_NT = 16;
constexpr int OP_KP = 528;
constexpr int OP_TAB_WIN = 0, OP_TAB_WSQ = 4096, OP_TAB_INVN = 8192, OP_TAB_TW512 = 9216, OP_TAB_TW1024 = 13312,
              OP_TAB_WIN64 = 17408, OP_TAB_TW64 = 25600, OP_TAB_MCONST = 33792, OP_TAB_EXP8 = 35328, OP_TAB_BYTES = 37376;

#ifndef OP_LATE_ARGS
#define OP_LATE_ARGS 1
#endif
#ifndef OP_TRACE
#define OP_TRACE 0
#endif
#ifndef OP_ARGCHECK
#define OP_ARGCHECK 0
#endif
#ifndef OP_TILECOUNT
#define OP_TILECOUNT 0
#endif
#ifndef OP_NO_LOOPTOP_WAIT
#define OP_NO_LOOPTOP_WAIT 0
#endif
#ifndef OP_BACKOFF
#define OP_BACKOFF 0
#endif
#if OP_BACKOFF
#define OP_POLL_SLEEP(spin) do { if ((spin) >= 8) __builtin_amdgcn_s_sleep(127); else __builtin_amdgcn_s_sleep(1); } while (0)
#else
#define OP_POLL_SLEEP(spin) __builtin_amdgcn_s_sleep(1)
#endif
#ifndef OP_WHO
#define OP_WHO 0
#endif
#ifndef OP_GLOBAL_DRAW
#define OP_GLOBAL_DRAW 0
#endif
#if OP_GLOBAL_DRAW
#define OP_DRAW_TICKET(p64) __hip_atomic_fetch_add((__attribute__((address_space(1))) unsigned*)(p64), 1u, __ATOMIC_RELAXED, __HIP_MEMORY_SCOPE_AGENT)
#else
#define OP_DRAW_TICKET(p64) atomicAdd((unsigned*)(uintptr_t)(p64), 1u)
#endif
#ifndef OP_DRAW_TOP
#define OP_DRAW_TOP 0
#endif
#ifndef OP_RESTAGE
#define OP_RESTAGE 0
#endif
#ifndef OP_MAX_ITERS
#define OP_MAX_ITERS 0
#endif
#ifndef OP_LATE_START_US
#define OP_LATE_START_US 0
#endif
#ifndef OP_EXP_STALL_NS
#define OP_EXP_STALL_NS 0
#endif
#ifndef OP_INPLACE
#define OP_INPLACE 0
#endif
struct OnePassArgs {
  ApplyArgs A;
  const void* x_exact;
  int64_t stride_exact;
  int dtype_exact;
  const char* tab;
  ThreshConsts tc;
  double mag_scale, top_db;
  unsigned long long* xbits;
  unsigned* ticket;
  unsigned ticket_base;
  unsigned epoch;
  unsigned* err;
  int nf, nt;
  float prop, inv_ktot;
  unsigned long long* part2;
  unsigned* alim;
  int scan_q;
  unsigned total_tiles;
#if OP_TRACE
  unsigned* trace;
#endif
#if OP_WHO
  unsigned* who;
#endif
};

#if OP_LATE_ARGS
#define OP_XARG(type, member) (*(const __attribute__((address_space(4))) type*)(kp4 + __builtin_offsetof(OnePassArgs, member)))
#else
#define OP_XARG(type, member) (P.member)
#endif
__device__ __forceinline__ double op_exact_power(const OnePassArgs& P, int64_t row, int64_t chunk, int64_t t, int f,
                                                 int lane) {
#if OP_LATE_ARGS
  const __attribute__((address_space(4))) char* kp4 = (const __attribute__((address_space(4))) char*)__builtin_amdgcn_kernarg_segment_ptr();
  asm volatile("" : "+s"(kp4));
#endif
  const int64_t s0 = t * OP_XARG(int32_t, A.g.H) - OP_XARG(int32_t, A.g.padL);
  const int64_t v_cs = OP_XARG(int64_t, A.view.cs), v_pad = OP_XARG(int64_t, A.view.pad), v_Lp = OP_XARG(int64_t, A.view.Lp),
                v_lo = OP_XARG(int64_t, A.view.lo), v_hi = OP_XARG(int64_t, A.view.hi), x_stride = OP_XARG(int64_t, stride_exact);
  const void* const x_exact = (const void*)(uintptr_t)OP_XARG(unsigned long long, x_exact);
  const int x_dtype = OP_XARG(int, dtype_exact);
  const char* const tab = (const char*)(uintptr_t)OP_XARG(unsigned long long, tab);
  double re = 0.0, im = 0.0;
#pragma unroll 4
  for (int i = 0; i < 16; ++i) {
    const int m = lane + 64 * i;
    double xs = 0.0;
    {
      const int64_t sp = s0 + m;
      const int64_t gi = chunk * v_cs - v_pad + sp;
      if (sp >= 0 && sp < v_Lp && gi >= v_lo && gi < v_hi) xs = load_sample(x_exact, x_dtype, row * x_stride + gi);
    }
    const double xv = xs * reinterpret_cast<const double*>(tab + OP_TAB_WIN64)[m];
    const int j = (f * m) & 1023;
    cx<double> w = reinterpret_cast<const cx<double>*>(tab + OP_TAB_TW64)[j & 511];
    if (j >= 512) { w.x = -w.x; w.y = -w.y; }
    re += xv * w.x;
    im += xv * w.y;
  }
  for (int off = 32; off > 0; off >>= 1) {
    re += __shfl_xor(re, off);
    im += __shfl_xor(im, off);
  }
  return re * re + im * im;
}

#ifndef OP_ABLATE
#define OP_ABLATE 0
#endif
#ifndef OP_TRACE
#define OP_TRACE 0
#endif
#if OP_TRACE
#define OP_STAMP(i)                                                                                   \
  do {                                                                                                \
    const long long t_now_ = clock64();                                                               \
    if (lane == 0 && t_slot_) t_slot_[i] = (unsigned)(t_now_ - t_prev_);                              \
    t_prev_ = t_now_;                                                                                 \
  } while (0)
#else
#define OP_STAMP(i) do { } while (0)
#endif

#ifndef OP_LATE_P
#define OP_LATE_P 1
#endif
#ifndef OP_OCC
#define OP_OCC 3
#endif
#define OP_DONE { if (PERSIST) continue; return; }
template <int WAVES, bool PROP, bool LOSE = false, bool REDO = false, bool PERSIST = false>
__global__ __launch_bounds__(WAVES * 64, OP_OCC) void k_gate_onepass(OnePassArgs Pk) {
  static_assert(WAVES == 4, "tile = 16 frames");
  static_assert(!PERSIST || (!LOSE && !REDO), "the persistent loop is the lazy first launch only");
  extern __shared__ __attribute__((aligned(16))) char smem[];
  cf* tw512 = reinterpret_cast<cf*>(smem);
  cf* regions = tw512 + FN;
  float* swin = reinterpret_cast<float*>(regions + WAVES * WAVE_CX_H);
  float* s_t2 = swin + 1024;
  unsigned long long* s_exp = reinterpret_cast<unsigned long long*>(s_t2 + T2_FLOATS);
  double* s_t2d = reinterpret_cast<double*>(s_exp + 256);
  unsigned* s_misc = reinterpret_cast<unsigned*>(s_t2d + 514);
  unsigned char* s_ef = reinterpret_cast<unsigned char*>(s_misc + 8);
  constexpr int NF = 4 * WAVES;
  constexpr int SPAN = (NF - 1) * 256 + 1024, XPITCH = 288;
  static_assert((SPAN / 256) * XPITCH <= WAVES * WAVE_CX_H * 2, "span must fit the exchange slices");
  constexpr int NQ = SPAN / 256;
  static_assert(SPAN % 256 == 0 && WAVES * 64 == 256, "one sample per thread and row");
  constexpr int SCAN_REG = 5;

  if (REDO && Pk.alim[1] != Pk.tc.need_tag) return;
#if OP_LATE_START_US
  if (PERSIST && (blockIdx.x % 5u) == 1u) {
    const unsigned long long t0_ = wall_clock64();
    while ((long long)(wall_clock64() - t0_) < (long long)OP_LATE_START_US * 100 * (1 + (blockIdx.x % 7u))) __builtin_amdgcn_s_sleep(8);
  }
#endif
  double t2pre[3];
  unsigned alim_v = 0u;
  {
    const int tid = threadIdx.x, lane = tid & 63;
    static_assert(FN == 2 * WAVES * 64 && WAVES * 64 == 256, "one pass of the prologue loads per thread");
    const cf tw_a = reinterpret_cast<const cf*>(Pk.tab + OP_TAB_TW512)[(tid >> 4) * (tid & 15)];
    const cf tw_b = reinterpret_cast<const cf*>(Pk.tab + OP_TAB_TW512)[((tid + 256) >> 4) * (tid & 15)];
    const float4 w4 = reinterpret_cast<const float4*>(Pk.tab + OP_TAB_WIN)[tid];
    const unsigned long long e8 = reinterpret_cast<const unsigned long long*>(Pk.tab + OP_TAB_EXP8)[tid];
    t2pre[0] = Pk.tc.T2[perm_inv(tid)];
    t2pre[1] = Pk.tc.T2[perm_inv(tid + 256)];
    t2pre[2] = Pk.tc.T2[perm_inv(512)];
    if (!REDO && Pk.alim != nullptr) {
      int z = 2 + min(lane & 15, OP_ALIM_BLOCKS - 1);
      asm volatile("" : "+v"(z));
      alim_v = Pk.alim[z];
    }
    if (tid == 0) {
      s_misc[PERSIST ? 4 : 0] = Pk.ticket_base == 0xffffffffu ? blockIdx.x : atomicAdd(Pk.ticket, 1u) - Pk.ticket_base;
      s_misc[1] = 0u;
    }
    tw512[tid] = tw_a;
    tw512[tid + 256] = tw_b;
    reinterpret_cast<float4*>(swin)[tid] = w4;
    s_exp[tid] = e8;
    if constexpr (PROP) {
      for (int f = tid; f <= 512; f += WAVES * 64) {
        const int lo = max(-Pk.nf, -f), hi = min(Pk.nf, 512 - f);
        int sum = 0;
        for (int a = lo; a <= hi; ++a) sum += Pk.nf + 1 - (a < 0 ? -a : a);
        s_ef[f] = (unsigned char)sum;
      }
    }
    if constexpr (PERSIST) {
#pragma unroll
      for (int k = 0; k < 3; ++k) {
        const int i = tid + k * WAVES * 64;
        if (i > 512) break;
        s_t2[t2_pos(i)] = t2_to_f32(t2pre[k], 4.0);
        s_t2d[i] = t2pre[k];
      }
      for (int off = 1; off < 16; off <<= 1) alim_v = min(alim_v, (unsigned)__shfl_xor((int)alim_v, off));
      if (tid == 0) s_misc[2] = alim_v;
#if OP_TILECOUNT == 2
      if (tid == 0) { s_misc[3] = Pk.total_tiles; s_misc[6] = (unsigned)(uintptr_t)Pk.err; s_misc[7] = (unsigned)((uintptr_t)Pk.err >> 32); }
#endif
    }
  }
  __syncthreads();

  struct TileSrc {
    const float* sp;
    bool blk_vec;
    const float* sc_base;
    int sc_n1;
    int64_t s0b, sc_lo, sc_last, sc_lenA, sc_c0, sc_c1;
  };
  auto tile_src = [](const OnePassArgs& P, int64_t row, int64_t chunk, int jt, bool test) -> TileSrc {
    const ApplyArgs& A = P.A;
    TileSrc S;
    const int64_t tf_tile = A.h_begin - 3 + (int64_t)jt * NF;
    S.s0b = tf_tile * 256 - A.g.padL;
    const int64_t gb = chunk * A.view.cs - A.view.pad + S.s0b;
    S.sp = (const float*)A.view.x + row * A.view.stride + gb;
    S.blk_vec = A.view.dtype == 0 && tf_tile >= 0 && tf_tile + NF <= A.g.T && S.s0b >= 0 && S.s0b + SPAN <= A.view.Lp &&
                gb >= A.view.lo && gb + SPAN <= A.view.hi && (reinterpret_cast<uintptr_t>(S.sp) & 15) == 0;
    S.sc_base = nullptr;
    S.sc_n1 = 0;
    S.sc_lo = S.sc_last = S.sc_lenA = S.sc_c0 = S.sc_c1 = 0;
    if (test) {
      const int64_t g0 = chunk * A.view.cs - A.view.pad;
      const int64_t s_lo = max<int64_t>(0, A.view.lo - g0), s_hi = min<int64_t>(A.view.Lp, A.view.hi - g0);
      const int64_t sp0 = (A.h_begin - 3 - NF) * 256 - A.g.padL;
      const int64_t sp1 = (A.h_begin - 3 + (int64_t)A.n_tiles * NF) * 256 - A.g.padL + SPAN;
      const int64_t first = min(s_hi, max(s_lo, sp0));
      S.sc_lo = s_lo;
      S.sc_last = max(s_lo, min(s_hi, sp1));
      S.sc_lenA = first - s_lo;
      S.sc_c0 = (int64_t)(jt + 1) * P.scan_q;
      S.sc_c1 = min(S.sc_c0 + P.scan_q, S.sc_lenA + (s_hi - S.sc_last));
      if (A.view.dtype == 0 && S.sc_c1 > S.sc_c0 && S.sc_c1 - S.sc_c0 <= SCAN_REG * WAVES * 64 &&
          (S.sc_c1 <= S.sc_lenA || S.sc_c0 >= S.sc_lenA)) {
        S.sc_base = (const float*)A.view.x + row * A.view.stride + g0 +
                    (S.sc_c1 <= S.sc_lenA ? s_lo + S.sc_c0 : S.sc_last + (S.sc_c0 - S.sc_lenA));
        S.sc_n1 = (int)(S.sc_c1 - S.sc_c0) - 1;
      }
    }
    return S;
  };
  float q[NQ];
  float sc[SCAN_REG];
  bool pf = false;

#if OP_EXP_STALL_NS
  const unsigned long long op_exp_t0_ = wall_clock64();
#endif
  for (unsigned iter = 0; iter == 0u || PERSIST; ++iter) {
  const OnePassArgs& P = (PERSIST || OP_LATE_P) ? *late_args<OnePassArgs>() : Pk;
  int tid = threadIdx.x;
#if OP_ARGCHECK
#if OP_ARGCHECK == 2
  if (PERSIST && threadIdx.x == 1) {
    const unsigned* a_ = reinterpret_cast<const unsigned*>(&P);
    const unsigned* b_ = reinterpret_cast<const unsigned*>(&Pk);
    bool same_ = true;
    for (unsigned w_ = 0; w_ < sizeof(OnePassArgs) / 4; ++w_) same_ = same_ && a_[w_] == b_[w_];
    if (!same_) atomicOr_system(Pk.err, 0x80u);
  }
#else
  if (PERSIST && threadIdx.x == 0 && (P.total_tiles != Pk.total_tiles || P.epoch != Pk.epoch || P.xbits != Pk.xbits || P.A.view.x != Pk.A.view.x))
    atomicOr_system(Pk.err, 0x80u);
#endif
#endif
#if OP_TRACE
  long long t_prev_ = clock64();
  unsigned* t_slot_ = nullptr;
#endif
  if constexpr (PERSIST) {
    asm volatile("" : "+v"(tid));
    if (iter != 0u) {
#if !OP_NO_LOOPTOP_WAIT
      asm volatile("s_waitcnt lgkmcnt(0)" ::: "memory");
#endif
      __syncthreads();
    }
#if OP_DRAW_TOP
    if (iter != 0u) {
      if (threadIdx.x == 0) s_misc[4u + (iter & 1u)] = atomicAdd(P.ticket, 1u) - P.ticket_base;
      __syncthreads();
    }
#endif
  }
  const ApplyArgs& A = P.A;
  const Geom& G = A.g;
  const int lane = tid & 63, wave = tid >> 6;
  const int g = lane >> 4, c = lane & 15;
  const unsigned tk_slot = PERSIST ? 4u + (iter & 1u) : 0u;
  const int ntt = A.n_tiles + 2;
  const unsigned ticket = PERSIST ? (unsigned)__builtin_amdgcn_readfirstlane((int)s_misc[tk_slot]) : s_misc[0];
#if OP_TILECOUNT == 2
  if (PERSIST && threadIdx.x == 0 && P.total_tiles != s_misc[3]) {
    unsigned* e_ = (unsigned*)(((uintptr_t)s_misc[7] << 32) | (uintptr_t)s_misc[6]);
    atomicOr_system(e_, 0x40u);
    atomicMax_system(e_ + 6, P.total_tiles);
    atomicMax_system(e_ + 7, iter);
  }
  if (PERSIST && ticket >= s_misc[3]) return;
#endif
#if OP_WHO
  if (PERSIST && threadIdx.x == 0 && ticket < 4096u) P.who[ticket * 4 + 2] = (blockIdx.x + 1u) | (iter << 16);
#endif
  if (PERSIST && ticket >= P.total_tiles) return;
#if OP_TILECOUNT == 1
  if (PERSIST && threadIdx.x == 0) { atomicAdd_system(P.err + 4, 1u); atomicAdd_system(P.err + 5, ticket); }
#endif
#if OP_RESTAGE
  if (PERSIST && iter != 0u) {
    const int t_ = threadIdx.x;
    tw512[t_] = reinterpret_cast<const cf*>(P.tab + OP_TAB_TW512)[(t_ >> 4) * (t_ & 15)];
    tw512[t_ + 256] = reinterpret_cast<const cf*>(P.tab + OP_TAB_TW512)[((t_ + 256) >> 4) * (t_ & 15)];
    reinterpret_cast<float4*>(swin)[t_] = reinterpret_cast<const float4*>(P.tab + OP_TAB_WIN)[t_];
    s_exp[t_] = reinterpret_cast<const unsigned long long*>(P.tab + OP_TAB_EXP8)[t_];
#pragma unroll
    for (int k = 0; k < 3; ++k) {
      const int i = t_ + k * WAVES * 64;
      if (i > 512) break;
      const double v_ = P.tc.T2[perm_inv(i)];
      s_t2[t2_pos(i)] = t2_to_f32(v_, 4.0);
      s_t2d[i] = v_;
    }
  }
#endif
  if (PERSIST && tid == 0) {
    s_misc[1] = 0u;
#if OP_TK_LATE
    s_misc[tk_slot ^ 1u] = 0xffffffffu;
#endif
  }
#if OP_TRACE
  t_slot_ = P.trace + ((size_t)ticket * 4 + wave) * 16;
  if (lane == 0) t_slot_[14] = (blockIdx.x + 1u) | (iter << 16);
#endif
  OP_STAMP(0);
  const int64_t u = ticket / (unsigned)ntt;
  const int jt = (int)(ticket % (unsigned)ntt) - 1;
  const bool halo_tile = jt < 0 || jt >= A.n_tiles;
  const unsigned gu = (unsigned)(A.view.unit0 + u), nch = (unsigned)A.view.n_chunks;
  const int64_t row = gu / nch;
  const int64_t chunk = A.view.c0 + gu % nch;
  const bool lazy = PERSIST || P.alim != nullptr;
  const int need = (lazy && !REDO) ? 0 : need_of(P.tc, u);
  if (REDO && need == 0) return;
  if (!REDO && lazy && ticket == 0u && tid == 0) P.ticket[8] = 0u;
  const bool floor_live = need == 1;

  auto t2eff = [&](int f, double v) -> double {
    if (floor_live) {
      double fl = cell_db(P.tc.pmax[u * G.FS + f], P.mag_scale) - P.top_db;
      if (fl > P.tc.thresh[f]) v = -1.0;
    }
    if (need & 2) v = T2_NEVER;
    return v;
  };
  const int64_t tf_tile = A.h_begin - 3 + (int64_t)jt * NF;
  const int64_t tq = tf_tile + 4 * wave;
  const int64_t t = tq + g;
  const bool fvalid = t >= 0 && t < G.T;
  cf* fb = regions + wave * WAVE_CX_H + frame_base_h(g);

  bool blk_vec;
  {
    const bool test = !REDO && lazy;
    const TileSrc S = tile_src(P, row, chunk, jt, test);
    blk_vec = S.blk_vec;
    const int64_t s0b = S.s0b;
    auto fill_t2 = [&]() {
      if constexpr (!PERSIST) {
#pragma unroll
        for (int k = 0; k < 3; ++k) {
          const int i = tid + k * WAVES * 64;
          if (i > 512) break;
          const double v = t2eff(perm_inv(i), t2pre[k]);
          s_t2[t2_pos(i)] = t2_to_f32(v, 4.0);
          s_t2d[i] = v;
        }
      }
    };
    float* xs = reinterpret_cast<float*>(regions);
    unsigned mi = 0u;
    auto ab = [](float x) -> unsigned { return __float_as_uint(x) & 0x7fffffffu; };
    if (!pf) {
      if (S.blk_vec) {
#pragma unroll
        for (int k = 0; k < NQ; ++k) q[k] = S.sp[tid + k * 256];
      }
      if (S.sc_base != nullptr) {
#pragma unroll
        for (int k = 0; k < SCAN_REG; ++k) sc[k] = S.sc_base[min(tid + k * WAVES * 64, S.sc_n1)];
      }
    }
    fill_t2();
    if (blk_vec) {
#pragma unroll
      for (int k = 0; k < NQ; ++k) {
        xs[k * XPITCH + tid] = q[k];
        mi = max(mi, ab(q[k]));
      }
    } else {
      for (int i = tid; i < SPAN; i += WAVES * 64) {
        const float xv = (float)view_sample(A.view, row, chunk, s0b + i);
        xs[(i >> 8) * XPITCH + (i & 255)] = xv;
        mi = max(mi, ab(xv));
      }
    }
    if (test) {
      if (S.sc_base != nullptr) {
#pragma unroll
        for (int k = 0; k < SCAN_REG; ++k) mi = max(mi, ab(sc[k]));
      } else {
        for (int64_t i = S.sc_c0 + tid; i < S.sc_c1; i += WAVES * 64)
          mi = max(mi, ab((float)view_sample(A.view, row, chunk, i < S.sc_lenA ? S.sc_lo + i : S.sc_last + (i - S.sc_lenA))));
      }
      unsigned alim_t = PERSIST ? s_misc[2] : alim_v;
      if constexpr (!PERSIST)
        for (int off = 1; off < 16; off <<= 1) alim_t = min(alim_t, (unsigned)__shfl_xor((int)alim_t, off));
      const bool hit = mi >= alim_t;
      if (__any(hit)) {
        const bool nonfinite = __any(mi >= 0x7f800000u);
        double* pm = const_cast<double*>(P.tc.pmax) + u * G.FS;
        for (int f = lane; f < G.FS; f += 64) pm[f] = 0.0;
        if (lane == 0) {
          atomicMax(reinterpret_cast<unsigned*>(const_cast<int*>(P.tc.need_floor)) + u, (P.tc.need_tag << 2) | (nonfinite ? 2u : 1u));
          P.alim[1] = P.tc.need_tag;
          P.err[1] = P.epoch;
        }
      }
    }
  }
  __syncthreads();
  OP_STAMP(1);

  cf v[32];
  float nrm2 = 0.f;
  {
    const float* xs = reinterpret_cast<const float*>(regions) + (4 * wave + g) * XPITCH + 2 * c;
    const float2* wl = reinterpret_cast<const float2*>(swin + 2 * c);
    if (blk_vec) {
#pragma unroll
      for (int r = 0; r < 32; ++r) {
        const float2 x2 = *reinterpret_cast<const float2*>(xs + (r >> 3) * XPITCH + 32 * (r & 7));
        const float2 w2 = wl[16 * r];
        v[r] = {x2.x * w2.x, x2.y * w2.y};
      }
    } else {
#pragma unroll
      for (int r = 0; r < 32; ++r) {
        float2 x2 = *reinterpret_cast<const float2*>(xs + (r >> 3) * XPITCH + 32 * (r & 7));
        if (!fvalid) x2 = make_float2(0.f, 0.f);
        const float2 w2 = wl[16 * r];
        v[r] = {x2.x * w2.x, x2.y * w2.y};
      }
    }
  }
  __syncthreads();
  OP_STAMP(2);
  {
#pragma unroll
    for (int r = 0; r < 32; ++r) nrm2 += v[r].x * v[r].x + v[r].y * v[r].y;
    nrm2 += __shfl_xor(nrm2, 1);
    nrm2 += __shfl_xor(nrm2, 2);
    nrm2 += __shfl_xor(nrm2, 4);
    nrm2 += __shfl_xor(nrm2, 8);
  }
  {
    int z0 = 0;
    asm volatile("" : "+v"(z0));
// ... 11 lines not shown
    if (l0) whi = {-w16.y, w16.x};
  }
  rg_lane0_to_entries(v, l0);
  {
    const cf r0 = v[0], r31 = v[31];
    cf xa, xb;
    split_pair(r0, r31, wlo, xa, xb);
    v[0] = {l0 ? r0.x : xa.x, l0 ? r0.y : xa.y};
    v[31] = {l0 ? r31.x : xb.x, l0 ? r31.y : xb.y};
#pragma unroll
    for (int sl = 1; sl < 16; ++sl) {
      const cf w = mul_tw<false>(sl < 8 ? wlo : whi, twc<32>(sl), tws<32>(sl));
      cf ya, yb;
      split_pair(v[sl], v[31 - sl], w, ya, yb);
      v[sl] = ya;
      v[31 - sl] = yb;
    }
  }
#define OP_PA(sl) v[sl]
#define OP_PB(sl) v[31 - (sl)]
  const cf raw0 = v[0], raw8 = v[31];
#else
  cf pa[16], pb[16];
  const cf raw0 = v[0], raw8 = v[8];
  const bool l0 = c == 0;
  cf wlo = reinterpret_cast<const cf*>(P.tab + OP_TAB_TW1024)[c];
  asm volatile("" : "+v"(wlo.x), "+v"(wlo.y));
  cf whi = wlo;
  {
    const cf w16 = reinterpret_cast<const cf*>(P.tab + OP_TAB_TW1024)[16];
    if (l0) whi = {-w16.y, w16.x};
  }
  {
    auto sel = [&](cf a0, cf a1) -> cf { return {l0 ? a0.x : a1.x, l0 ? a0.y : a1.y}; };
    auto split = [&](cf a, cf b2, cf w, cf& xa, cf& xb) { split_pair(a, b2, w, xa, xb); };
    split(v[0], v[31], wlo, pa[0], pb[0]);
#pragma unroll
    for (int sl = 1; sl < 16; ++sl) {
      const cf a = sl < 8 ? v[sl] : sel(v[8 + sl], v[sl]);
      const cf b2 = sl < 8 ? sel(v[16 - sl], v[31 - sl]) : sel(v[39 - sl], v[31 - sl]);
      const cf w = mul_tw<false>(sl < 8 ? wlo : whi, twc<32>(sl), tws<32>(sl));
      split(a, b2, w, pa[sl], pb[sl]);
    }
  }

#define OP_PA(sl) pa[sl]
#define OP_PB(sl) pb[sl]
#endif
  OP_STAMP(4);
#if OP_EXP_STALL_NS
  if (PERSIST && iter == 0u)
    while ((long long)(wall_clock64() - op_exp_t0_) * 10 < (long long)OP_EXP_STALL_NS) __builtin_amdgcn_s_sleep(2);
#endif
  unsigned long long myword;
  {
    int zt = 0;
    asm volatile("" : "+v"(zt));
    const float* t2 = s_t2 + c * T2_PITCH + zt;
    const float t2_512 = s_t2[T2_POS512];
    const float d2 = nrm2 > 0.f ? 8.0f * 2.3283064e-10f * nrm2 : -1.0f;
    unsigned pA = 0, pB = 0, nA = 0, nB = 0;
    auto decideA = [&](float Pw, float T) {
      const float nd = T - Pw;
      const float e = fmaf(-nd, nd, d2 * (Pw + T));
      pA = __builtin_amdgcn_alignbit(pA, __float_as_uint(nd), 31);
      nA = __builtin_amdgcn_alignbit(nA, __float_as_uint(e), 31);
    };
    auto decideB = [&](float Pw, float T) {
      const float nd = T - Pw;
      const float e = fmaf(-nd, nd, d2 * (Pw + T));
      pB = __builtin_amdgcn_alignbit(pB, __float_as_uint(nd), 31);
      nB = __builtin_amdgcn_alignbit(nB, __float_as_uint(e), 31);
    };
    bool pred512 = false, amb512 = false;
    {
      const float Pk = OP_PA(0).x * OP_PA(0).x + OP_PA(0).y * OP_PA(0).y;
      const float Pn = OP_PB(0).x * OP_PB(0).x + OP_PB(0).y * OP_PB(0).y;
      const float x0 = 2.f * (raw0.x + raw0.y), xN = 2.f * (raw0.x - raw0.y);
      const float P256 = 4.f * (raw8.x * raw8.x + raw8.y * raw8.y);
      decideA(l0 ? x0 * x0 : Pk, t2[0]);
      decideB(l0 ? P256 : Pn, t2[31]);
      const float P5 = xN * xN, d5 = P5 - t2_512;
      pred512 = l0 && d5 > 0.f;
      amb512 = l0 && d5 * d5 <= d2 * (P5 + t2_512);
    }
#pragma unroll
    for (int sl = 1; sl < 16; ++sl) {
      if ((sl & 3) == 0) __builtin_amdgcn_sched_barrier(0);
      decideA(OP_PA(sl).x * OP_PA(sl).x + OP_PA(sl).y * OP_PA(sl).y, t2[sl]);
      decideB(OP_PB(sl).x * OP_PB(sl).x + OP_PB(sl).y * OP_PB(sl).y, t2[31 - sl]);
    }
    __builtin_amdgcn_sched_barrier(0);
    unsigned pred = (__brev(pA) >> 16) | (pB << 16);
    unsigned amb = ~((__brev(nA) >> 16) | (nB << 16));
    if (need == 2) { pred = 0; amb = 0; pred512 = false; amb512 = false; }
    if (!fvalid) { amb = 0; amb512 = false; pred = 0; pred512 = false; }
    if ((OP_ABLATE & 8) == 0 && __ballot(amb != 0 || amb512) != 0ull) {
      float* park = reinterpret_cast<float*>(regions + wave * WAVE_CX_H) + lane;
      static_assert(64 * 32 * 4 <= WAVE_CX_H * 8, "parked registers must fit the wave's slice");
#pragma unroll
      for (int i = 0; i < 16; ++i) {
        park[(2 * i) * 64] = OP_PB(i).x;
        park[(2 * i + 1) * 64] = OP_PB(i).y;
      }
      while (true) {
        const unsigned long long pending = __ballot(amb != 0 || amb512);
// ... 408 lines not shown
  const float poison = s_misc[1] != 0u ? __uint_as_float(0x7fc00000u) : 0.f;
  {
    const int64_t pb0 = e_tf * 256 - e_padL;
    const int64_t gi00 = e_chunk * e_gstep + (pb0 - e_p0);
    float* dbase = (float*)e_out + (e_row * e_ostride + gi00 - e_g0);
    float* dst0 = dbase + s4;
    const bool tile_fast = e_odtype == 0 && e_normalize && e_tf >= 3 && e_tf + NF + 2 < e_T &&
                           e_tf >= e_hbegin && e_tf + NF + 2 < e_hend && pb0 >= e_p0 &&
                           pb0 + NF * 256 <= e_p1 && pb0 + NF * 256 <= e_Lout && gi00 >= e_glo &&
                           gi00 + NF * 256 <= e_ghi && (reinterpret_cast<uintptr_t>(dbase) & 15) == 0 && WAVES == 4;
    if (tile_fast) {
      constexpr int R = WAVE_CX_H * 2;
      auto ld4 = [&](int off) { return *reinterpret_cast<const float4*>(&fr[off + s4]); };
      auto fin = [&](float4 a, int jj) {
        a.x = (a.x + poison) * n4.x; a.y = (a.y + poison) * n4.y; a.z = (a.z + poison) * n4.z; a.w = (a.w + poison) * n4.w;
        *reinterpret_cast<float4*>(dst0 + jj * 256) = a;
      };
      if (wave == 3) {
#pragma unroll
        for (int it = 0; it < 4; ++it) fin(ld4(it * R + 3 * HPITCH), 3 + 4 * it);
        OP_STAMP(13);
        if constexpr (PERSIST && OP_PF_AT == 5) prefetch_next();
        OP_DONE;
      }
      {
        const float4 a4 = ld4((WAVES - 1) * R + (wave + 4) * HPITCH);
        unsigned long long* dst = e_part2 + (((size_t)e_u * e_ntiles + e_jt) * 3 + wave) * 256 + s4;
        const op_v4u ga = {__float_as_uint(a4.x + poison), e_epoch, __float_as_uint(a4.y + poison), e_epoch};
        const op_v4u gb = {__float_as_uint(a4.z + poison), e_epoch, __float_as_uint(a4.w + poison), e_epoch};
        op_st16_sc1(dst, ga);
        op_st16_sc1(dst + 2, gb);
      }
#pragma unroll
      for (int it = 1; it < 4; ++it) {
        float4 a4 = ld4((it - 1) * R + (wave + 4) * HPITCH);
        const float4 f4 = ld4(it * R + wave * HPITCH);
        a4.x += f4.x; a4.y += f4.y; a4.z += f4.z; a4.w += f4.w;
        fin(a4, wave + 4 * it);
      }
      {
        float4 a4 = ld4(wave * HPITCH);
        const unsigned long long* src = e_part2 + (((size_t)e_u * e_ntiles + e_jt - 1) * 3 + wave) * 256 + s4;
        op_v4u ga, gb;
        for (int spin = 0;; ++spin) {
          asm volatile("global_load_dwordx4 %0, %2, off sc1\n\tglobal_load_dwordx4 %1, %2, off offset:16 sc1\n\ts_waitcnt vmcnt(0)"
                       : "=&v"(ga), "=&v"(gb) : "v"(src) : "memory");
          const unsigned e = e_epoch;
          if ((OP_ABLATE & 16) || (!LOSE && ga[1] == e && ga[3] == e && gb[1] == e && gb[3] == e)) break;
          if (LOSE || spin >= OP_SPIN_MAX) {
            atomicOr_system(e_err, 2u);
#if OP_WHO
            if (atomicAdd_system(e_err + 15, 1u) == 0u) { e_err[12] = e_ticket; e_err[13] = ga[1]; }
#endif
            ga[0] = ga[2] = gb[0] = gb[2] = 0x7fc00000u;
            break;
          }
          OP_POLL_SLEEP(spin);
        }
        a4.x = __uint_as_float(ga[0]) + a4.x;
        a4.y = __uint_as_float(ga[2]) + a4.y;
        a4.z = __uint_as_float(gb[0]) + a4.z;
        a4.w = __uint_as_float(gb[2]) + a4.w;
        fin(a4, wave);
      }
      OP_STAMP(13);
      if constexpr (PERSIST && OP_PF_AT == 5) prefetch_next();
      OP_DONE;
    }
  }
  for (int it = 0; it < 5; ++it) {
    const int jj = wave < 3 ? (it == 0 ? NF + wave : (it == 4 ? wave : wave + 4 * it)) : (it < 4 ? 3 + 4 * it : -1);
    if (jj < 0) break;
    const int64_t h = e_tf + jj;
    if (h >= e_hend || h < e_hbegin) continue;
    float4 a4 = make_float4(0.f, 0.f, 0.f, 0.f);
    bool all_valid = true;
#pragma unroll
    for (int q = 0; q < 4; ++q) {
      const int64_t ti = e_tf + jj - q;
      if (ti < 0 || ti >= e_T) all_valid = false;
    }
    {
      const int wh = jj >> 2, lh = jj & 3;
      if (wh >= 1 && wh - 1 < WAVES && lh <= 2) {
        a4 = *reinterpret_cast<const float4*>(&fr[(wh - 1) * WAVE_CX_H * 2 + (lh + 4) * HPITCH + s4]);
      }
      if (wh < WAVES) {
        const float4 f4 = *reinterpret_cast<const float4*>(&fr[wh * WAVE_CX_H * 2 + lh * HPITCH + s4]);
        a4.x += f4.x; a4.y += f4.y; a4.z += f4.z; a4.w += f4.w;
      }
    }
    if (jj >= NF) {
      const int k = jj - NF;
      unsigned long long* dst = e_part2 + (((size_t)e_u * e_ntiles + e_jt) * 3 + k) * 256 + s4;
      const op_v4u ga = {__float_as_uint(a4.x + poison), e_epoch, __float_as_uint(a4.y + poison), e_epoch};
      const op_v4u gb = {__float_as_uint(a4.z + poison), e_epoch, __float_as_uint(a4.w + poison), e_epoch};
      op_st16_sc1(dst, ga);
      op_st16_sc1(dst + 2, gb);
      continue;
    }
    if (jj < 3) {
      const unsigned long long* src = e_part2 + (((size_t)e_u * e_ntiles + e_jt - 1) * 3 + jj) * 256 + s4;
      op_v4u ga, gb;
      for (int spin = 0;; ++spin) {
        asm volatile("global_load_dwordx4 %0, %2, off sc1\n\tglobal_load_dwordx4 %1, %2, off offset:16 sc1\n\ts_waitcnt vmcnt(0)"
                     : "=&v"(ga), "=&v"(gb) : "v"(src) : "memory");
        const unsigned e = e_epoch;
        if ((OP_ABLATE & 16) || (!LOSE && ga[1] == e && ga[3] == e && gb[1] == e && gb[3] == e)) break;
        if (LOSE || spin >= OP_SPIN_MAX) {
          atomicOr_system(e_err, 2u);
          ga[0] = ga[2] = gb[0] = gb[2] = 0x7fc00000u;
          break;
        }
        OP_POLL_SLEEP(spin);
      }
      a4.x = __uint_as_float(ga[0]) + a4.x;
      a4.y = __uint_as_float(ga[2]) + a4.y;
      a4.z = __uint_as_float(gb[0]) + a4.z;
      a4.w = __uint_as_float(gb[2]) + a4.w;
    }
    a4.x += poison; a4.y += poison; a4.z += poison; a4.w += poison;
    if (!e_normalize) {
    } else if (all_valid) {
      a4.x *= n4.x; a4.y *= n4.y; a4.z *= n4.z; a4.w *= n4.w;
    } else {
      float4 nrm = make_float4(0.f, 0.f, 0.f, 0.f);
#pragma unroll
      for (int q = 0; q < 4; ++q) {
        const int64_t ti = h - q;
        if (ti >= 0 && ti < e_T) {
          const float4 w4 = *reinterpret_cast<const float4*>(&reinterpret_cast<const float*>(e_tab + OP_TAB_WSQ)[256 * q + s4]);
          nrm.x += w4.x; nrm.y += w4.y; nrm.z += w4.z; nrm.w += w4.w;
        }
      }
      a4.x /= (nrm.x > 1e-10f ? nrm.x : 1.f);
      a4.y /= (nrm.y > 1e-10f ? nrm.y : 1.f);
      a4.z /= (nrm.z > 1e-10f ? nrm.z : 1.f);
      a4.w /= (nrm.w > 1e-10f ? nrm.w : 1.f);
    }
    {
      const int64_t pb = h * 256 - e_padL;
      const int64_t gi0 = e_chunk * e_gstep + (pb - e_p0);
      if (e_odtype == 0 && pb >= e_p0 && pb + 256 <= e_p1 && pb + 256 <= e_Lout && gi0 >= e_glo &&
          gi0 + 256 <= e_ghi) {
        float* dst = (float*)e_out + (e_row * e_ostride + gi0 - e_g0 + s4);
        if ((reinterpret_cast<uintptr_t>(dst) & 15) == 0) {
          *reinterpret_cast<float4*>(dst) = a4;
          continue;
        }
      }
    }
    const float vals[4] = {a4.x, a4.y, a4.z, a4.w};
#pragma unroll
    for (int e = 0; e < 4; ++e) {
      const int64_t p = h * 256 + s4 + e - e_padL;
      if (p < e_p0 || p >= e_p1) continue;
      const int64_t gi = e_chunk * e_gstep + (p - e_p0);
      if (gi < e_glo || gi >= e_ghi) continue;
      store_sample(e_out, e_odtype, e_row * e_ostride + gi - e_g0, p < e_Lout ? vals[e] : 0.f);
    }
  }
  if constexpr (PERSIST && OP_PF_AT == 5) prefetch_next();
  }
}
// ... 4 lines not shown
```

Baseline: 101,300.

## Defer noise-statistics kernels into the persistent one-pass gate launch

Noise statistics (column stats and final threshold) are no longer launched as separate kernels when the stationary one-pass path will follow. Extra workgroups in the persistent gate launch compute them. Gate tiles first do their peak-amplitude scan, then spin on per-block ready tags before loading the thresholds. A flush path runs the old kernels whenever the deferred tail cannot be folded in. This removes two kernel launches and a serialisation point per call, at the cost of inter-workgroup spin waits, extra gate-kernel complexity and a new timeout error path.

Result: slower. 85530 (-15.5%).

```diff
diff --git a/include/mi355gate_debug.h b/include/mi355gate_debug.h
--- a/include/mi355gate_debug.h
+++ b/include/mi355gate_debug.h
@@ -35,6 +35,7 @@
 #define SG_OPT_TILE_ORDER 15
 #define SG_OPT_EXACT_MATERIALISED 16
 #define SG_OPT_FORCE_NOFAST 2
+#define SG_OPT_STATS_IN_GATE 17
 
 #define SG_STAGE_CHANNEL_MEAN 0
 #define SG_STAGE_STFT_POWER 1
diff --git a/noisereduce_amd/_ffi.py b/noisereduce_amd/_ffi.py
--- a/noisereduce_amd/_ffi.py
+++ b/noisereduce_amd/_ffi.py
@@ -30,6 +30,7 @@
 SG_OPT_FLOOR_TEST = 13
 SG_OPT_TILE_ORDER = 15
 SG_OPT_EXACT_MATERIALISED = 16
+SG_OPT_STATS_IN_GATE = 17
 SG_OPT_FORCE_UNFUSED = 1
 SG_OPT_FORCE_NOFAST = 2
 SG_BWD_ROW, SG_BWD_FAST, SG_BWD_REG, SG_BWD_OLA, SG_BWD_ROWS = 1, 2, 3, 4, 5
diff --git a/noisereduce_amd/csrc/api.hip b/noisereduce_amd/csrc/api.hip
--- a/noisereduce_amd/csrc/api.hip
+++ b/noisereduce_amd/csrc/api.hip
@@ -87,6 +87,9 @@
 }
 }
 
+#ifndef SG_STATS_IN_GATE_DEFAULT
+#define SG_STATS_IN_GATE_DEFAULT 1
+#endif
 struct RegGeom;
 struct sg_handle {
   sg_params p{};
@@ -116,6 +119,15 @@
   unsigned inject_fault = 0;
   unsigned lose_now = 0;
   unsigned ticket_base = 0;
+  struct StatsTail {
+    bool on = false;
+    int nts = 0;
+    Geom g{};
+    hipStream_t st = nullptr;
+  } sp;
+  hipEvent_t sp_ev = nullptr;
+  bool stats_in_gate = SG_STATS_IN_GATE_DEFAULT != 0;
+  DevBuf stag;
   unsigned epoch = 0;
   bool fast_integer = false;
   bool force_exact = false;
@@ -317,9 +329,11 @@
   return e;
 }
 
+static int stats_flush(sg_handle* h, hipStream_t st);
 static int ensure(sg_handle* h, DevBuf& b, size_t bytes) {
   if (b.bytes >= bytes) return SG_OK;
   if (b.p) {
+    if (h->sp.on) { int rc = stats_flush(h, h->sp.st); if (rc) return rc; }
     HIPCHK(h, hipDeviceSynchronize());
     HIPCHK(h, hipFree(b.p));
     b.p = nullptr;
@@ -1205,7 +1219,8 @@
   for (auto& r : h->prof_live) { (void)hipEventDestroy(r.a); (void)hipEventDestroy(r.b); }
   for (auto e : h->prof_pool) (void)hipEventDestroy(e);
   if (h->err_host) (void)hipHostFree(h->err_host);
-  for (DevBuf* b : {&h->tw64, &h->tw32, &h->wfull64, &h->wa32, &h->ws32, &h->wsq32, &h->kf, &h->kt, &h->thresh,
+  if (h->sp_ev) (void)hipEventDestroy(h->sp_ev);
+  for (DevBuf* b : {&h->stag, &h->tw64, &h->tw32, &h->wfull64, &h->wa32, &h->ws32, &h->wsq32, &h->kf, &h->kt, &h->thresh,
                     &h->P, &h->pmax, &h->thr_rows, &h->raw, &h->M, &h->seg, &h->yn, &h->bits, &h->K16, &h->umax,
                     &h->need, &h->T2, &h->part, &h->tw512, &h->invn, &h->seam, &h->ftab, &h->xbits, &h->xpart,
                     &h->xticket, &h->xtick2, &h->ftab3, &h->xexp, &h->optab, &h->nsp, &h->nsc, &h->xin, &h->czt_tw64, &h->czt_ch64,
@@ -1316,6 +1331,52 @@
   return SG_OK;
 }
 
+static int stats_tail(sg_handle* h, const Geom& g, int64_t ub, int nts, double* thresh_out, hipStream_t st, bool gate_consts) {
+  int rc;
+  dim3 grid((g.F + 63) / 64, (unsigned)ub, nts);
+  hipLaunchKernelGGL(k_colstats1, grid, dim3(64 * STAT_TG), 0, st, (const double*)h->P.p, g, h->mag_scale,
+                     (double*)h->part.p, db_fast_consts(h));
+  HIPCHK(h, hipGetLastError());
+  GateConsts gc{};
+  if (gate_consts && ub == 1 && grid.x <= 62) {
+    if ((rc = ensure(h, h->T2, (size_t)g.FS * 8))) return rc;
+    if ((rc = ensure_zeroed(h, h->alim, 256, st))) return rc;
+    gc.T2 = (double*)h->T2.p; gc.alim_b = (unsigned*)h->alim.p + 2; gc.sum_abs_w = h->sum_abs_w;
+  }
+  hipLaunchKernelGGL(k_colstats1_final, dim3((unsigned)((g.FS + 63) / 64), (unsigned)ub), dim3(64 * STAT_TG), 0, st,
+                     (const double*)h->part.p, (const double*)h->P.p, g, nts, h->mag_scale, h->p.top_db,
+                     h->p.n_std_thresh, h->p.ddof, (double*)h->pmax.p, thresh_out, gc);
+  HIPCHK(h, hipGetLastError());
+  if (gc.T2 != nullptr) h->t2_ready = true;
+  return SG_OK;
+}
+
+static bool stats_defer_ok(const sg_handle* h, const Geom& g) {
+  return h->stats_in_gate && h->p.variant == SG_VARIANT_S && h->p.stationary && h->fast_ok && h->fused_ok && g.F == 513 &&
+         (g.F + 63) / 64 == OP_ALIM_BLOCKS && (g.FS + 63) / 64 == OP_ALIM_BLOCKS && !h->force_unfused && !h->force_nofast && !h->force_split && !h->force_f64_decide &&
+         !h->force_noseam && !h->force_nolean && !h->force_exact && h->tile_order == 0 && h->floor_test != 1 && !h->inject_fault &&
+         h->p.smooth_mask && h->p.n_grad_freq <= 8 && h->p.n_grad_time <= fast::OP_MAX_NT && h->ftab3.p && h->optab.p;
+}
+
+static int stats_flush(sg_handle* h, hipStream_t st) {
+  if (!h->sp.on) return SG_OK;
+  h->sp.on = false;
+  if (st != h->sp.st) {
+    if (!h->sp_ev) HIPCHK(h, hipEventCreateWithFlags(&h->sp_ev, hipEventDisableTiming));
+    HIPCHK(h, hipEventRecord(h->sp_ev, h->sp.st));
+    HIPCHK(h, hipStreamWaitEvent(st, h->sp_ev, 0));
+  }
+  const int keep = h->prof_override;
+  h->prof_override = SG_STAGE_NOISE_STATS;
+  int rc;
+  {
+    ProfScope ps(h, SG_STAGE_COLSTATS, st);
+    rc = stats_tail(h, h->sp.g, 1, h->sp.nts, (double*)h->thresh.p, st, true);
+  }
+  h->prof_override = keep;
+  return rc;
+}
+
 static int stage_stats(sg_handle* h, const View& v, const Geom& g, int64_t ub, double* thresh_out, hipStream_t st,
                        bool gate_consts = false) {
   if (ub < 16) {
@@ -1323,26 +1384,18 @@
       ProfScope ps(h, SG_STAGE_STFT_POWER, st);
       HIPCHK(h, stft_any<double>(h, v, g, ub, (double*)h->P.p, nullptr, nullptr, 1.0, st));
     }
-    ProfScope ps(h, SG_STAGE_COLSTATS, st);
     const int nts = (int)std::max<int64_t>(1, std::min<int64_t>(std::min(stat_slices(g, ub), STAT_TG * STAT1_MAXS), g.T / SG_STAT_FRAMES_PER_SLICE));
     int rc = ensure(h, h->part, (size_t)ub * nts * STAT1_NP * g.FS * 8);
     if (rc) return rc;
-    dim3 grid((g.F + 63) / 64, (unsigned)ub, nts);
-    hipLaunchKernelGGL(k_colstats1, grid, dim3(64 * STAT_TG), 0, st, (const double*)h->P.p, g, h->mag_scale,
-                       (double*)h->part.p, db_fast_consts(h));
-    HIPCHK(h, hipGetLastError());
-    GateConsts gc{};
-    if (gate_consts && ub == 1 && grid.x <= 62) {
+    if (gate_consts && ub == 1 && thresh_out == (double*)h->thresh.p && stats_defer_ok(h, g) && nts <= 64) {
       if ((rc = ensure(h, h->T2, (size_t)g.FS * 8))) return rc;
       if ((rc = ensure_zeroed(h, h->alim, 256, st))) return rc;
-      gc.T2 = (double*)h->T2.p; gc.alim_b = (unsigned*)h->alim.p + 2; gc.sum_abs_w = h->sum_abs_w;
-    }
-    hipLaunchKernelGGL(k_colstats1_final, dim3((unsigned)((g.FS + 63) / 64), (unsigned)ub), dim3(64 * STAT_TG), 0, st,
-                       (const double*)h->part.p, (const double*)h->P.p, g, nts, h->mag_scale, h->p.top_db,
-                       h->p.n_std_thresh, h->p.ddof, (double*)h->pmax.p, thresh_out, gc);
-    HIPCHK(h, hipGetLastError());
-    if (gc.T2 != nullptr) h->t2_ready = true;
-    return SG_OK;
+      if ((rc = ensure_zeroed(h, h->stag, (size_t)(fast::OP_ST_READY + 64) * 4, st))) return rc;
+      h->sp.on = true; h->sp.nts = nts; h->sp.g = g; h->sp.st = st;
+      return SG_OK;
+    }
+    ProfScope ps(h, SG_STAGE_COLSTATS, st);
+    return stats_tail(h, g, ub, nts, thresh_out, st, gate_consts);
   }
   int rc = stage_power(h, v, g, ub, st);
   if (rc) return rc;
@@ -1459,7 +1512,7 @@
   ThreshConsts tc{};
   FloorLazy fl{};
 };
-static int floor_setup(sg_handle* h, const Geom& g, int64_t ub, int nb, hipStream_t st, FloorSetup* out) {
+static int floor_setup(sg_handle* h, const Geom& g, int64_t ub, int nb, hipStream_t st, FloorSetup* out, bool fuse_ok = false) {
   int rc;
   if ((rc = handoff_prepare(h, st))) return rc;
   const unsigned live_stamp = h->err_host[1];
@@ -1473,13 +1526,14 @@
   FloorSetup f;
   f.lazy = need_tag != 0u &&
            (h->floor_test == 2 || (h->floor_test == 0 && !(live_stamp != 0u && h->epoch - live_stamp <= 16u)));
+  if (h->sp.on && !(f.lazy && fuse_ok && !h->lose_now) && (rc = stats_flush(h, st))) return rc;
   if (f.lazy) {
     const int wpr = (g.F + 63) / 64;
     if ((rc = ensure(h, h->bits, (size_t)ub * g.T * wpr * 8))) return rc;
     if ((rc = ensure_zeroed(h, h->need, (size_t)ub * 4, st))) return rc;
     if ((rc = ensure(h, h->T2, (size_t)g.FS * 8))) return rc;
     if ((rc = ensure_zeroed(h, h->alim, 256, st))) return rc;
-    if (!h->t2_ready) {
+    if (!h->t2_ready && !h->sp.on) {
       ProfScope ps(h, SG_STAGE_PREP, st);
       hipLaunchKernelGGL(k_prep_thresh_lazy, dim3(1), dim3(256), 0, st, (const double*)h->thresh.p, g.F, h->mag_scale,
                          h->sum_abs_w, h->p.top_db, (double*)h->T2.p, (unsigned*)h->alim.p, nb);
@@ -1964,6 +2018,7 @@
   if (++h->epoch == 0) {
     if (h->xbits.p) HIPCHK(h, hipMemsetAsync(h->xbits.p, 0, h->xbits.bytes, st));
     if (h->xpart.p) HIPCHK(h, hipMemsetAsync(h->xpart.p, 0, h->xpart.bytes, st));
+    if (h->stag.p) HIPCHK(h, hipMemsetAsync(h->stag.p, 0, h->stag.bytes, st));
     h->epoch = 1;
     if (h->err_host) h->err_host[1] = 0u;
   }
@@ -2002,11 +2057,11 @@
   if (h->err_host && *h->err_host != 0u) {
     const unsigned e = *h->err_host;
     *h->err_host = 0u;
-    FAIL(h, SG_E_HANDOFF, "a tile hand-off timed out (code %u: %s%s%s): the output of the call(s) enqueued since the "
+    FAIL(h, SG_E_HANDOFF, "a tile hand-off timed out (code %u: %s%s%s%s): the output of the call(s) enqueued since the "
                           "last check is invalid; re-run them (SG_OPT_FORCE_SPLIT + SG_OPT_FORCE_NOLEAN select the "
                           "kernels without in-launch hand-offs)",
          e, (e & 1u) ? "mask bits " : "", (e & 2u) ? "partial hops (one-pass gate) " : "",
-         (e & 4u) ? "partial hops (fused apply)" : "");
+         (e & 4u) ? "partial hops (fused apply) " : "", (e & 8u) ? "noise statistics (one-pass gate)" : "");
   }
   return SG_OK;
 }
@@ -2104,7 +2159,8 @@
   constexpr int WAVES = 4, NF = 16;
   int rc;
   FloorSetup fs;
-  if ((rc = floor_setup(h, g, ub, OP_ALIM_BLOCKS, st, &fs))) return rc;
+  const int64_t ntt_pre = (((om.p1 - 1 + g.padL) / 256 + 1 - (om.p0 + g.padL) / 256) + 3 + NF - 1) / NF + 2;
+  if ((rc = floor_setup(h, g, ub, OP_ALIM_BLOCKS, st, &fs, h->tile_order == 0 && ub * ntt_pre >= 2))) return rc;
   const bool lazy = fs.lazy;
   const ThreshConsts& tc = fs.tc;
   ++(lazy ? h->n_floor_lazy : h->n_floor_apriori);
@@ -2166,8 +2222,33 @@
   const unsigned pgrid = persist ? (unsigned)std::min<int64_t>(ub * ntt, (int64_t)pg_per_cu * h->n_cu) : 0u;
 #endif
   P.total_tiles = (unsigned)(ub * ntt);
+  P.n_stat = P.n_final = 0u;
+  unsigned n_role = 0u;
+  if (h->sp.on) {
+    if (!persist) FAIL(h, SG_E_STATE, "one-pass gate: statistics tail pending outside the persistent launch");
+    const Geom& sgm = h->sp.g;
+    if (st != h->sp.st) {
+      if (!h->sp_ev) HIPCHK(h, hipEventCreateWithFlags(&h->sp_ev, hipEventDisableTiming));
+      HIPCHK(h, hipEventRecord(h->sp_ev, h->sp.st));
+      HIPCHK(h, hipStreamWaitEvent(st, h->sp_ev, 0));
+    }
+    P.n_final = (unsigned)((sgm.FS + 63) / 64);
+    P.n_stat = P.n_final * (unsigned)h->sp.nts;
+    P.st_nts = h->sp.nts; P.st_ddof = h->p.ddof;
+    P.st_P = (const double*)h->P.p; P.st_part = (double*)h->part.p;
+    P.st_pmax = (double*)h->pmax.p; P.st_thresh = (double*)h->thresh.p;
+    P.st_n_std = h->p.n_std_thresh;
+    P.st_g = sgm;
+    P.st_gc = GateConsts{(double*)h->T2.p, (unsigned*)h->alim.p + 2, h->sum_abs_w};
+    P.st_dbk = db_fast_consts(h);
+    P.st_tags = (unsigned*)h->stag.p;
+    n_role = P.n_stat + P.n_final;
+    P.ticket_base += n_role;
+    h->sp.on = false;
+    h->t2_ready = true;
+  }
   if (h->tile_order == 1) P.ticket_base = 0xffffffffu;
-  else h->ticket_base += (unsigned)(ub * ntt) + (OP_MAX_ITERS == 1 ? 0u : pgrid);
+  else h->ticket_base += n_role + (unsigned)(ub * ntt) + (OP_MAX_ITERS == 1 ? 0u : pgrid);
   P.nf = h->p.n_grad_freq; P.nt = h->p.n_grad_time;
   P.prop = (float)h->p.prop_decrease;
   P.inv_ktot = 1.0f / (float)h->ktot;
@@ -2219,7 +2300,7 @@
     auto go = [&](auto kern) -> hipError_t {
       hipError_t e = set_lds(reinterpret_cast<const void*>(kern), lds);
       if (e != hipSuccess) return e;
-      hipLaunchKernelGGL(kern, dim3(persist ? pgrid : (unsigned)(ub * ntt)), dim3(WAVES * 64), lds, st, P);
+      hipLaunchKernelGGL(kern, dim3(persist ? pgrid + n_role : (unsigned)(ub * ntt)), dim3(WAVES * 64), lds, st, P);
       return hipGetLastError();
     };
     if (persist && prop) HIPCHK(h, go(fast::k_gate_onepass<WAVES, true, false, false, true>));
@@ -2237,6 +2318,7 @@
     P.epoch = h->epoch;
     P.ticket = (unsigned*)h->xticket.p + 8;
     P.ticket_base = 0;
+    P.n_stat = P.n_final = 0u;
     const size_t lds = (size_t)(fast::FN + WAVES * fast::WAVE_CX_H) * sizeof(fast::cf) + (1024 + T2_FLOATS) * sizeof(float) +
                        256 * 8 + 514 * 8 + 32 + (prop ? 528 : 0);
     auto redo = [&](auto kern) -> hipError_t {
@@ -2502,16 +2584,20 @@
                         (long long)v.Lp, h->W);
   if (h->p.stationary && !h->has_thresh)
     FAIL(h, SG_E_STATE, "stationary gate: call sg_noise_stats or sg_set_noise_threshold first");
-  if (h->force_exact || ((om.dtype == SG_I16 || om.dtype == SG_I32) && !h->fast_integer))
+  if (h->force_exact || ((om.dtype == SG_I16 || om.dtype == SG_I32) && !h->fast_integer)) {
+    int rcf = stats_flush(h, st);
+    if (rcf) return rcf;
     return exact_fused_ok(h, g) ? run_S_exact_fused(h, v, total_units, om, st) : run_S_exact(h, v, total_units, om, st);
+  }
   const bool onepass = h->fused_ok && !h->force_unfused && h->fast_ok && !h->force_nofast && onepass_ok(h, g, om);
   const RegGeom* r = reg_geom(h);
   const bool onepass_r = r && onepass_reg_ok(h, r, g, om);
   const bool lean = onepass || onepass_r || (h->fused_ok && !h->force_unfused && h->fast_ok && !h->force_nofast &&
                                              h->p.prop_decrease == 1.0);
   int64_t ub = units_per_batch(h, g, total_units, lean);
-  int rc = ensure_ws(h, g, ub, lean);
-  if (rc) return rc;
+  int rc;
+  if (!onepass && (rc = stats_flush(h, st))) return rc;
+  if ((rc = ensure_ws(h, g, ub, lean))) return rc;
   const View vx = v;
   if (v.dtype != SG_F32 && ((h->fast_ok && !h->force_nofast && (onepass || (!h->p.stationary && nonstat2_ok(h, g)))) || onepass_r)) {
     const int64_t rows = total_units / std::max<int64_t>(1, v.n_chunks), len = v.hi - v.lo;
@@ -2720,6 +2806,7 @@
   if (!noise_dev || !dtype_ok(dtype) || C < 1 || n < 1) FAIL(h, SG_E_INVALID, "sg_noise_stats: bad argument");
   if (h->p.variant != SG_VARIANT_S) FAIL(h, SG_E_INVALID, "sg_noise_stats is a variant-S entry point");
   if (n < h->W) FAIL(h, SG_E_INVALID, "noise clip of %lld samples is shorter than win_length=%d", (long long)n, h->W);
+  h->sp.on = false;
 #ifdef SG_EXP_SKIP_STATS
   if (h->has_thresh && h->t2_ready) return SG_OK;
 #endif
@@ -2753,6 +2840,7 @@
   if (!h) return SG_E_INVALID;
   if (!thresh_host || n_bins != h->F) FAIL(h, SG_E_INVALID, "sg_get_noise_threshold: n_bins must be %d", h->F);
   if (!h->has_thresh) FAIL(h, SG_E_STATE, "no noise threshold set");
+  { int rc = stats_flush(h, (hipStream_t)stream); if (rc) return rc; }
   HIPCHK(h, hipMemcpyAsync(thresh_host, h->thresh.p, (size_t)h->F * sizeof(double), hipMemcpyDeviceToHost,
                            (hipStream_t)stream));
   HIPCHK(h, hipStreamSynchronize((hipStream_t)stream));
@@ -2762,6 +2850,7 @@
 extern "C" int sg_set_noise_threshold(sg_handle* h, const double* thresh_host, int32_t n_bins, void* stream) {
   if (!h) return SG_E_INVALID;
   if (!thresh_host || n_bins != h->F) FAIL(h, SG_E_INVALID, "sg_set_noise_threshold: n_bins must be %d", h->F);
+  h->sp.on = false;
   h->t2_ready = false;
   HIPCHK(h, hipMemcpyAsync(h->thresh.p, thresh_host, (size_t)h->F * sizeof(double), hipMemcpyHostToDevice,
                            (hipStream_t)stream));
@@ -2774,6 +2863,7 @@
   if (!h) return SG_E_INVALID;
   if (!thresh_dev || n_bins != h->F) FAIL(h, SG_E_INVALID, "sg_get_noise_threshold_dev: n_bins must be %d", h->F);
   if (!h->has_thresh) FAIL(h, SG_E_STATE, "no noise threshold set");
+  { int rc = stats_flush(h, (hipStream_t)stream); if (rc) return rc; }
   HIPCHK(h, hipMemcpyAsync(thresh_dev, h->thresh.p, (size_t)h->F * sizeof(double), hipMemcpyDeviceToDevice,
                            (hipStream_t)stream));
   return SG_OK;
@@ -2782,6 +2872,7 @@
 extern "C" int sg_set_noise_threshold_dev(sg_handle* h, const double* thresh_dev, int32_t n_bins, void* stream) {
   if (!h) return SG_E_INVALID;
   if (!thresh_dev || n_bins != h->F) FAIL(h, SG_E_INVALID, "sg_set_noise_threshold_dev: n_bins must be %d", h->F);
+  h->sp.on = false;
   h->t2_ready = false;
   HIPCHK(h, hipMemcpyAsync(h->thresh.p, thresh_dev, (size_t)h->F * sizeof(double), hipMemcpyDeviceToDevice,
                            (hipStream_t)stream));
@@ -3064,6 +3155,7 @@
 
 extern "C" int sg_set_option(sg_handle* h, int32_t option, int64_t value) {
   if (!h) return SG_E_INVALID;
+  { int rcf = stats_flush(h, h->sp.st); if (rcf) return rcf; }
   switch (option) {
     case SG_OPT_FORCE_UNFUSED: h->force_unfused = value != 0; return SG_OK;
     case SG_OPT_FORCE_NOFAST: h->force_nofast = value != 0; return SG_OK;
@@ -3092,6 +3184,7 @@
       if (value < 0 || value > 2) FAIL(h, SG_E_INVALID, "SG_OPT_FLOOR_TEST: 0 (predicted), 1 (a priori) or 2 (in the gate kernel)");
       h->floor_test = (int)value;
       return SG_OK;
+    case SG_OPT_STATS_IN_GATE: h->stats_in_gate = value != 0; return SG_OK;
   }
   FAIL(h, SG_E_INVALID, "sg_set_option: unknown option %d", option);
 }
@@ -3114,6 +3207,7 @@
     case SG_OPT_TILE_ORDER: *value = h->tile_order; return SG_OK;
     case SG_OPT_EXACT_MATERIALISED: *value = h->exact_materialised; return SG_OK;
     case SG_OPT_FLOOR_TEST: *value = h->floor_test; return SG_OK;
+    case SG_OPT_STATS_IN_GATE: *value = h->stats_in_gate; return SG_OK;
   }
   return SG_E_INVALID;
 }
@@ -3192,6 +3286,7 @@
 
 extern "C" int sg_debug_counter(sg_handle* h, int32_t which, int64_t* value, void* stream) {
   if (!h || !value) return SG_E_INVALID;
+  { int rcf = stats_flush(h, (hipStream_t)stream); if (rcf) return rcf; }
   if (which == 1 || which == 2) {
     *value = which == 1 ? h->n_floor_lazy : h->n_floor_apriori;
     return SG_OK;
@@ -3261,6 +3356,7 @@
 
 extern "C" int sg_debug_fetch(sg_handle* h, int32_t what, void* host, int64_t bytes, void* stream) {
   if (!h) return SG_E_INVALID;
+  { int rcf = stats_flush(h, (hipStream_t)stream); if (rcf) return rcf; }
   if (!host || h->dbg_units == 0) FAIL(h, SG_E_STATE, "sg_debug_fetch: nothing processed yet");
   size_t cells = (size_t)h->dbg_units * h->dbg_T * h->FS;
   const void* src;
@@ -3355,6 +3451,7 @@
                                 void* out_dev, int out_dtype, int64_t max_workspace_bytes, void* stream) {
   if (!h) return SG_E_INVALID;
   if (!rg_variant_ok(h)) return SG_E_INVALID;
+  { int rcf = stats_flush(h, (hipStream_t)stream); if (rcf) return rcf; }
   if (n_clips < 0 || (n_clips > 0 && (!clips || !x_dev || !out_dev)) || !dtype_ok(in_dtype) || !dtype_ok(out_dtype) ||
       n_noise < 0 || (n_noise > 0 && !noise) || (h->p.stationary && n_noise > 0 && !dtype_ok(noise_dtype) && noise_dev))
     FAIL(h, SG_E_INVALID, "sg_process_clips: bad argument");
@@ -3530,6 +3627,7 @@
   sg_handle* h = b->h;
   if (n_bins != h->F) FAIL(h, SG_E_INVALID, "sg_stream_set_threshold: n_bins must be %d", h->F);
   if (!thresh_host && !h->has_thresh) FAIL(h, SG_E_STATE, "no noise threshold set");
+  if (!thresh_host) { int rcf = stats_flush(h, (hipStream_t)stream); if (rcf) return rcf; }
   return sg::st_set_threshold(b->b, slots, n_slots, thresh_host ? nullptr : (const double*)h->thresh.p, thresh_host,
                               (hipStream_t)stream, &h->err);
 }
diff --git a/noisereduce_amd/csrc/kernels.hpp b/noisereduce_amd/csrc/kernels.hpp
--- a/noisereduce_amd/csrc/kernels.hpp
+++ b/noisereduce_amd/csrc/kernels.hpp
@@ -333,18 +333,26 @@
   m2 = fmin(m2, hi);
 }
 
-__global__ __launch_bounds__(64 * STAT_TG) void k_colstats1(const double* __restrict__ P, Geom g, double mag_scale,
-                                                            double* __restrict__ part ,
-                                                            DbFast dbk) {
-  __shared__ double r[STAT1_NP][STAT_TG][64];
-  __shared__ __attribute__((aligned(16))) double s_tab[256];
-  s_tab[threadIdx.x] = dbk.tab[threadIdx.x];
-  __syncthreads();
-  const int l = threadIdx.x & 63;
-  const int f = blockIdx.x * 64 + l;
-  const int tg = threadIdx.x >> 6;
-  const int64_t u = blockIdx.y;
-  const int ts = blockIdx.z, nts = gridDim.z;
+template <bool WT>
+__device__ __forceinline__ void stat_st(double* p, double v) {
+  if constexpr (WT) __hip_atomic_store(p, v, __ATOMIC_RELAXED, __HIP_MEMORY_SCOPE_AGENT);
+  else *p = v;
+}
+template <bool WT>
+__device__ __forceinline__ double stat_ld(const double* p) {
+  if constexpr (WT) return __hip_atomic_load(p, __ATOMIC_RELAXED, __HIP_MEMORY_SCOPE_AGENT);
+  else return *p;
+}
+
+template <bool WT>
+__device__ __forceinline__ void colstats1_body(const double* __restrict__ P, const Geom& g, double mag_scale,
+                                               double* __restrict__ part , const DbFast& dbk,
+                                               int bx, int64_t u, int ts, int nts, double (*r)[STAT_TG][64], double* s_tab, int tid) {
+  s_tab[tid] = dbk.tab[tid];
+  __syncthreads();
+  const int l = tid & 63;
+  const int f = bx * 64 + l;
+  const int tg = tid >> 6;
   const int64_t tb = g.T * ts / nts, te = g.T * (ts + 1) / nts;
   double mx = 0.0, m1 = 1e300, m2 = 1e300, s1 = 0.0, s2 = 0.0;
   if (f < g.F) {
@@ -383,8 +391,16 @@
       s2 += r[4][i][l];
     }
     double* o = part + ((u * nts + ts) * STAT1_NP) * (int64_t)g.FS + f;
-    o[0] = mx; o[g.FS] = m1; o[2 * g.FS] = m2; o[3 * g.FS] = s1; o[4 * g.FS] = s2;
-  }
+    stat_st<WT>(o, mx); stat_st<WT>(o + g.FS, m1); stat_st<WT>(o + 2 * g.FS, m2); stat_st<WT>(o + 3 * g.FS, s1); stat_st<WT>(o + 4 * g.FS, s2);
+  }
+}
+
+__global__ __launch_bounds__(64 * STAT_TG) void k_colstats1(const double* __restrict__ P, Geom g, double mag_scale,
+                                                            double* __restrict__ part ,
+                                                            DbFast dbk) {
+  __shared__ double r[STAT1_NP][STAT_TG][64];
+  __shared__ __attribute__((aligned(16))) double s_tab[256];
+  colstats1_body<false>(P, g, mag_scale, part, dbk, (int)blockIdx.x, (int64_t)blockIdx.y, (int)blockIdx.z, (int)gridDim.z, r, s_tab, (int)threadIdx.x);
 }
 
 constexpr int STAT1_MAXS = 16;
@@ -393,15 +409,13 @@
   unsigned* alim_b;
   double sum_abs_w;
 };
-__global__ __launch_bounds__(64 * STAT_TG) void k_colstats1_final(const double* __restrict__ part,
-                                                                  const double* __restrict__ P, Geom g, int nts,
-                                                                  double mag_scale, double top_db, double n_std,
-                                                                  int ddof, double* __restrict__ pmax,
-                                                                  double* __restrict__ thresh, GateConsts gc) {
-  __shared__ double r[3][STAT_TG][64];
-  const int l = threadIdx.x & 63, tg = threadIdx.x >> 6;
-  const int f = blockIdx.x * 64 + l;
-  const int64_t u = blockIdx.y;
+template <bool WT>
+__device__ __forceinline__ void colstats1_final_body(const double* __restrict__ part, const double* __restrict__ P,
+                                                     const Geom& g, int nts, double mag_scale, double top_db, double n_std,
+                                                     int ddof, double* __restrict__ pmax, double* __restrict__ thresh,
+                                                     const GateConsts& gc, int bx, int64_t u, double (*r)[STAT_TG][64], int tid) {
+  const int l = tid & 63, tg = tid >> 6;
+  const int f = bx * 64 + l;
   const int64_t i = u * g.FS + f;
   const bool live = f < g.F;
   const double Tn = (double)g.T;
@@ -410,25 +424,29 @@
   double m1[STAT1_MAXS];
   {
     const int fc = live ? f : g.F - 1;
-    double a0[STAT1_MAXS], a3[STAT1_MAXS], a4[STAT1_MAXS];
-#pragma unroll
-    for (int k = 0; k < STAT1_MAXS; ++k) {
-      const int ts = tg + STAT_TG * k;
-      const double* o = part + ((u * nts + (ts < nts ? ts : nts - 1)) * STAT1_NP) * (int64_t)g.FS + fc;
-      a0[k] = o[0];
-      m1[k] = o[g.FS];
-      a3[k] = o[3 * g.FS];
-      a4[k] = o[4 * g.FS];
-    }
-#pragma unroll
-    for (int k = 0; k < STAT1_MAXS; ++k) {
-      const bool on = live && tg + STAT_TG * k < nts;
-      if (on) {
-        mx = fmax(mx, a0[k]);
-        s1 += a3[k];
-        s2 += a4[k];
-      } else {
-        m1[k] = 1e300;
+    constexpr int KB = WT ? STAT1_MAXS / 2 : STAT1_MAXS;
+#pragma unroll
+    for (int k0 = 0; k0 < STAT1_MAXS; k0 += KB) {
+      double a0[KB], a3[KB], a4[KB];
+#pragma unroll
+      for (int k = k0; k < k0 + KB; ++k) {
+        const int ts = tg + STAT_TG * k;
+        const double* o = part + ((u * nts + (ts < nts ? ts : nts - 1)) * STAT1_NP) * (int64_t)g.FS + fc;
+        a0[k - k0] = stat_ld<WT>(o);
+        m1[k] = stat_ld<WT>(o + g.FS);
+        a3[k - k0] = stat_ld<WT>(o + 3 * g.FS);
+        a4[k - k0] = stat_ld<WT>(o + 4 * g.FS);
+      }
+#pragma unroll
+      for (int k = k0; k < k0 + KB; ++k) {
+        const bool on = live && tg + STAT_TG * k < nts;
+        if (on) {
+          mx = fmax(mx, a0[k - k0]);
+          s1 += a3[k - k0];
+          s2 += a4[k - k0];
+        } else {
+          m1[k] = 1e300;
+        }
       }
     }
   }
@@ -455,7 +473,7 @@
         bool both = false;
         if ((km >> k) & 1u) {
           const double* o = part + ((u * nts + ts) * STAT1_NP) * (int64_t)g.FS + f;
-          const double a1 = o[g.FS], a2 = o[2 * g.FS];
+          const double a1 = stat_ld<WT>(o + g.FS), a2 = stat_ld<WT>(o + 2 * g.FS);
           both = a1 < Pfl && a2 < Pfl;
           if (a1 < Pfl && !both) {
             const double d = cell_db(a1, mag_scale) - pivot;
@@ -469,7 +487,7 @@
         while (todo) {
           const int src = __ffsll((long long)todo) - 1;
           todo &= todo - 1;
-          const int fb = blockIdx.x * 64 + src;
+          const int fb = bx * 64 + src;
           const double Pfl_s = __shfl(Pfl, src), piv_s = __shfl(pivot, src), dfl_s = __shfl(dfl, src);
           const int64_t tb = g.T * ts / nts, te = g.T * (ts + 1) / nts;
           double c1 = 0.0, c2 = 0.0;
@@ -514,13 +532,13 @@
     s2 += r[2][k][l];
   }
   if (live) {
-    pmax[i] = mx;
+    stat_st<WT>(pmax + i, mx);
     double var = (s2 - s1 * s1 / Tn) / (Tn - (double)ddof);
     if (var < 0.0) var = 0.0;
     thr_out = (pivot + s1 / Tn) + sqrt(var) * n_std;
-    thresh[i] = thr_out;
+    stat_st<WT>(thresh + i, thr_out);
   } else if (f < g.FS) {
-    pmax[i] = 0.0;
+    stat_st<WT>(pmax + i, 0.0);
   }
   if (gc.T2 == nullptr || u != 0) return;
   const double eps = 2.220446049250313e-16;
@@ -536,7 +554,7 @@
       const double tm = (exp10(thr_out / 20.0) - eps) / mag_scale;
       t2 = tm > 0.0 ? tm * tm : 0.0;
     }
-    gc.T2[f] = t2;
+    stat_st<WT>(gc.T2 + f, t2);
     mn = fmin(mn, thr_out);
   }
   for (int off = 32; off > 0; off >>= 1) mn = fmin(mn, __shfl_xor(mn, off));
@@ -544,8 +562,19 @@
     const double lim = (exp10((mn + top_db - 1e-6) / 20.0) - eps) / (gc.sum_abs_w * mag_scale);
     unsigned bits = 0u;
     if (lim > 0.0) bits = __float_as_uint(__double2float_rd(lim * (1.0 - 1e-6)));
-    gc.alim_b[blockIdx.x] = bits;
-  }
+    if constexpr (WT) __hip_atomic_store(gc.alim_b + bx, bits, __ATOMIC_RELAXED, __HIP_MEMORY_SCOPE_AGENT);
+    else gc.alim_b[bx] = bits;
+  }
+}
+
+__global__ __launch_bounds__(64 * STAT_TG) void k_colstats1_final(const double* __restrict__ part,
+                                                                  const double* __restrict__ P, Geom g, int nts,
+                                                                  double mag_scale, double top_db, double n_std,
+                                                                  int ddof, double* __restrict__ pmax,
+                                                                  double* __restrict__ thresh, GateConsts gc) {
+  __shared__ double r[3][STAT_TG][64];
+  colstats1_final_body<false>(part, P, g, nts, mag_scale, top_db, n_std, ddof, pmax, thresh, gc, (int)blockIdx.x,
+                              (int64_t)blockIdx.y, r, (int)threadIdx.x);
 }
 
 __global__ void k_colstats_final(const double* __restrict__ s_part, Geom g, int nts,
diff --git a/noisereduce_amd/csrc/onepass.hpp b/noisereduce_amd/csrc/onepass.hpp
--- a/noisereduce_amd/csrc/onepass.hpp
+++ b/noisereduce_amd/csrc/onepass.hpp
@@ -1,4 +1,5 @@
 #pragma once
+#include "kernels.hpp"
 #include "fastpath.hpp"
 
 namespace sg {
@@ -82,6 +83,17 @@
   unsigned* alim;
   int scan_q;
   unsigned total_tiles;
+  unsigned n_stat, n_final;
+  int st_nts, st_ddof;
+  const double* st_P;
+  double* st_part;
+  double* st_pmax;
+  double* st_thresh;
+  double st_n_std;
+  Geom st_g;
+  GateConsts st_gc;
+  DbFast st_dbk;
+  unsigned* st_tags;
 #if OP_TRACE
   unsigned* trace;
 #endif
@@ -129,6 +141,57 @@
     im += __shfl_xor(im, off);
   }
   return re * re + im * im;
+}
+
+constexpr int OP_ST_READY = 64 * OP_ALIM_BLOCKS;
+constexpr unsigned OP_ERR_STATS = 8u;
+
+__device__ __forceinline__ void op_stat_role_body(const OnePassArgs& R, unsigned r, char* lds) {
+  static_assert(STAT_TG * 64 == 256, "the gate's workgroup shape");
+  double (*rr)[STAT_TG][64] = reinterpret_cast<double (*)[STAT_TG][64]>(lds);
+  int tid = threadIdx.x;
+  asm volatile("" : "+v"(tid));
+  if (r < R.n_stat) {
+    const int bx = (int)(r / (unsigned)R.st_nts), ts = (int)(r % (unsigned)R.st_nts);
+    double* s_tab = reinterpret_cast<double*>(lds + STAT1_NP * STAT_TG * 64 * 8);
+    colstats1_body<true>(R.st_P, R.st_g, R.mag_scale, R.st_part, R.st_dbk, bx, 0, ts, R.st_nts, rr, s_tab, tid);
+    if (tid < 64) {
+      asm volatile("s_waitcnt vmcnt(0)" ::: "memory");
+      if (tid == 0) __hip_atomic_store(R.st_tags + bx * 64 + ts, R.epoch, __ATOMIC_RELAXED, __HIP_MEMORY_SCOPE_AGENT);
+    }
+    return;
+  }
+  const int bx = (int)(r - R.n_stat);
+  bool lost = false;
+  if (tid < R.st_nts) {
+    const unsigned* tg = R.st_tags + bx * 64 + tid;
+    for (int spin = 0; __hip_atomic_load(tg, __ATOMIC_RELAXED, __HIP_MEMORY_SCOPE_AGENT) != R.epoch; ++spin) {
+      if (spin >= OP_SPIN_MAX) {
+        lost = true;
+        break;
+      }
+      __builtin_amdgcn_s_sleep(8);
+    }
+  }
+  if (__syncthreads_or(lost ? 1 : 0)) {
+    if (tid == 0) atomicOr_system(R.err, OP_ERR_STATS);
+    return;
+  }
+  colstats1_final_body<true>(R.st_part, R.st_P, R.st_g, R.st_nts, R.mag_scale, R.top_db, R.st_n_std, R.st_ddof, R.st_pmax,
+                             R.st_thresh, R.st_gc, bx, 0, rr, tid);
+  if (tid < 64) {
+    asm volatile("s_waitcnt vmcnt(0)" ::: "memory");
+    if (tid == 0) __hip_atomic_store(R.st_tags + OP_ST_READY + bx, R.epoch, __ATOMIC_RELAXED, __HIP_MEMORY_SCOPE_AGENT);
+  }
+}
+
+__device__ __noinline__ __attribute__((noreturn)) void op_stat_role(unsigned long long kargs, unsigned r, unsigned lds_addr) {
+  const unsigned long long ka = ((unsigned long long)(unsigned)__builtin_amdgcn_readfirstlane((int)(unsigned)(kargs >> 32)) << 32) |
+                                (unsigned)__builtin_amdgcn_readfirstlane((int)(unsigned)kargs);
+  const __attribute__((address_space(4))) char* kp = (const __attribute__((address_space(4))) char*)(uintptr_t)ka;
+  __attribute__((address_space(3))) char* lds = (__attribute__((address_space(3))) char*)(uintptr_t)(unsigned)__builtin_amdgcn_readfirstlane((int)lds_addr);
+  op_stat_role_body(*reinterpret_cast<const OnePassArgs*>((const char*)kp), (unsigned)__builtin_amdgcn_readfirstlane((int)r), (char*)lds);
+  __builtin_amdgcn_endpgm();
 }
 
 #ifndef OP_ABLATE
@@ -216,21 +279,39 @@
       }
     }
     if constexpr (PERSIST) {
-#pragma unroll
-      for (int k = 0; k < 3; ++k) {
-        const int i = tid + k * WAVES * 64;
-        if (i > 512) break;
-        s_t2[t2_pos(i)] = t2_to_f32(t2pre[k], 4.0);
-        s_t2d[i] = t2pre[k];
+      const bool tail = Pk.n_stat != 0u;
+      if (!tail) {
+#pragma unroll
+        for (int k = 0; k < 3; ++k) {
+          const int i = tid + k * WAVES * 64;
+          if (i > 512) break;
+          s_t2[t2_pos(i)] = t2_to_f32(t2pre[k], 4.0);
+          s_t2d[i] = t2pre[k];
+        }
       }
       for (int off = 1; off < 16; off <<= 1) alim_v = min(alim_v, (unsigned)__shfl_xor((int)alim_v, off));
-      if (tid == 0) s_misc[2] = alim_v;
+      if (tid == 0) {
+        s_misc[2] = alim_v;
+        s_misc[0] = tail ? 0u : 1u;
+        s_misc[3] = 0u;
+        s_misc[6] = 0u;
+      }
 #if OP_TILECOUNT == 2
       if (tid == 0) { s_misc[3] = Pk.total_tiles; s_misc[6] = (unsigned)(uintptr_t)Pk.err; s_misc[7] = (unsigned)((uintptr_t)Pk.err >> 32); }
 #endif
     }
   }
   __syncthreads();
+
+  if constexpr (PERSIST) {
+    const OnePassArgs& R = *late_args<OnePassArgs>();
+    const unsigned nr = R.n_stat + R.n_final;
+    const unsigned tk = (unsigned)__builtin_amdgcn_readfirstlane((int)s_misc[4]);
+    if (__builtin_expect(tk + nr < nr, 0)) {
+      op_stat_role((unsigned long long)(uintptr_t)&R, tk + nr,
+                   (unsigned)(uintptr_t)(__attribute__((address_space(3))) char*)reinterpret_cast<char*>(regions));
+    }
+  }
 
   struct TileSrc {
     const float* sp;
@@ -278,9 +359,14 @@
 #if OP_EXP_STALL_NS
   const unsigned long long op_exp_t0_ = wall_clock64();
 #endif
+  [[maybe_unused]] const int wave_s = __builtin_amdgcn_readfirstlane((int)(threadIdx.x >> 6));
   for (unsigned iter = 0; iter == 0u || PERSIST; ++iter) {
   const OnePassArgs& P = (PERSIST || OP_LATE_P) ? *late_args<OnePassArgs>() : Pk;
-  int tid = threadIdx.x;
+  int wave_o = wave_s;
+  if constexpr (PERSIST) asm volatile("" : "+s"(wave_o));
+  unsigned ones_o = ~0u;
+  if constexpr (PERSIST) asm volatile("" : "+s"(ones_o));
+  int tid = PERSIST ? (wave_o << 6) | (int)__builtin_amdgcn_mbcnt_hi(ones_o, __builtin_amdgcn_mbcnt_lo(ones_o, 0u)) : (int)threadIdx.x;
 #if OP_ARGCHECK
 #if OP_ARGCHECK == 2
   if (PERSIST && threadIdx.x == 1) {
@@ -306,6 +392,20 @@
       asm volatile("s_waitcnt lgkmcnt(0)" ::: "memory");
 #endif
       __syncthreads();
+      if (tid < 64) {
+        const unsigned hit1 = s_misc[6] & 3u;
+        if (__builtin_expect(hit1 != 0u, 0)) {
+          const int64_t u1 = s_misc[7];
+          double* pm = const_cast<double*>(P.tc.pmax) + u1 * P.A.g.FS;
+          for (int f = tid; f < P.A.g.FS; f += 64) pm[f] = 0.0;
+          if (tid == 0) {
+            atomicMax(reinterpret_cast<unsigned*>(const_cast<int*>(P.tc.need_floor)) + u1, (P.tc.need_tag << 2) | hit1);
+            P.alim[1] = P.tc.need_tag;
+            P.err[1] = P.epoch;
+            s_misc[6] = 0u;
+          }
+        }
+      }
     }
 #if OP_DRAW_TOP
     if (iter != 0u) {
@@ -355,7 +455,7 @@
   }
 #endif
   if (PERSIST && tid == 0) {
-    s_misc[1] = 0u;
+    s_misc[1] = s_misc[0] >> 1;
 #if OP_TK_LATE
     s_misc[tk_slot ^ 1u] = 0xffffffffu;
 #endif
@@ -445,6 +545,15 @@
           mi = max(mi, ab((float)view_sample(A.view, row, chunk, i < S.sc_lenA ? S.sc_lo + i : S.sc_last + (i - S.sc_lenA))));
       }
       unsigned alim_t = PERSIST ? s_misc[2] : alim_v;
+      if constexpr (PERSIST) {
+        if (__builtin_expect(s_misc[0] == 0u, 0)) {
+          unsigned wm = mi;
+          for (int off = 32; off > 0; off >>= 1) wm = max(wm, (unsigned)__shfl_xor((int)wm, off));
+          if (lane == 0) atomicMax(&s_misc[3], wm);
+          if (tid == 0) s_misc[7] = (unsigned)u;
+          alim_t = 0xffffffffu;
+        }
+      }
       if constexpr (!PERSIST)
         for (int off = 1; off < 16; off <<= 1) alim_t = min(alim_t, (unsigned)__shfl_xor((int)alim_t, off));
       const bool hit = mi >= alim_t;
@@ -562,6 +671,59 @@
   if (PERSIST && iter == 0u)
     while ((long long)(wall_clock64() - op_exp_t0_) * 10 < (long long)OP_EXP_STALL_NS) __builtin_amdgcn_s_sleep(2);
 #endif
+  if constexpr (PERSIST) {
+    if (__builtin_expect(s_misc[0] == 0u, 0)) {
+      typedef const __attribute__((address_space(4))) char* op_kps_t;
+      op_kps_t kps = (op_kps_t)__builtin_amdgcn_kernarg_segment_ptr();
+      asm volatile("" : "+s"(kps));
+#define OP_SARG(type, member) (*(const __attribute__((address_space(4))) type*)(kps + __builtin_offsetof(OnePassArgs, member)))
+      const unsigned s_epoch = OP_SARG(unsigned, epoch);
+      const unsigned* const s_tags = (const unsigned*)(uintptr_t)OP_SARG(unsigned long long, st_tags);
+      const double* const s_T2 = (const double*)(uintptr_t)OP_SARG(unsigned long long, tc.T2);
+      const unsigned* const s_alim = (const unsigned*)(uintptr_t)OP_SARG(unsigned long long, alim);
+      int zb = min(lane & 15, OP_ALIM_BLOCKS - 1);
+      asm volatile("" : "+v"(zb));
+      if (tid < 64) {
+        bool gave_up = false;
+        for (int spin = 0;; ++spin) {
+          const unsigned rw = __hip_atomic_load(s_tags + OP_ST_READY + zb, __ATOMIC_RELAXED, __HIP_MEMORY_SCOPE_AGENT);
+          if (__all(rw == s_epoch)) break;
+          if (spin >= OP_SPIN_MAX / 16) {
+            gave_up = true;
+            break;
+          }
+          __builtin_amdgcn_s_sleep(16);
+        }
+        if (tid == 0 && gave_up) s_misc[6] = 0x80u;
+      }
+      asm volatile("s_waitcnt lgkmcnt(0)" ::: "memory");
+      __syncthreads();
+      const bool lost = (s_misc[6] & 0x80u) != 0u;
+#pragma unroll
+      for (int k = 0; k < 3; ++k) {
+        const int i = tid + k * WAVES * 64;
+        if (i > 512) break;
+        const double tv = __hip_atomic_load(s_T2 + perm_inv(i), __ATOMIC_RELAXED, __HIP_MEMORY_SCOPE_AGENT);
+        s_t2[t2_pos(i)] = t2_to_f32(tv, 4.0);
+        s_t2d[i] = tv;
+      }
+      unsigned al = __hip_atomic_load(s_alim + 2 + zb, __ATOMIC_RELAXED, __HIP_MEMORY_SCOPE_AGENT);
+      for (int off = 1; off < 16; off <<= 1) al = min(al, (unsigned)__shfl_xor((int)al, off));
+      if (tid == 0) {
+        const unsigned wmax = s_misc[3];
+        s_misc[2] = al;
+        s_misc[6] = lost ? 0x80u : (wmax >= al ? (wmax >= 0x7f800000u ? 2u : 1u) : 0u);
+        if (lost) atomicOr_system((unsigned*)(uintptr_t)OP_SARG(unsigned long long, err), OP_ERR_STATS);
+      }
+      asm volatile("s_waitcnt lgkmcnt(0)" ::: "memory");
+      __syncthreads();
+      if (tid == 0) {
+        s_misc[0] = lost ? 2u : 1u;
+        if (lost) s_misc[1] = 1u;
+      }
+      asm volatile("s_waitcnt lgkmcnt(0)" ::: "memory");
+    }
+  }
   unsigned long long myword;
   {
     int zt = 0;
@@ -1076,7 +1238,9 @@
 #if OP_WHO
             if (atomicAdd_system(e_err + 15, 1u) == 0u) { e_err[12] = e_ticket; e_err[13] = ga[1]; }
 #endif
-            ga[0] = ga[2] = gb[0] = gb[2] = 0x7fc00000u;
+            unsigned nan_ = 0x7fc00000u;
+            asm volatile("" : "+v"(nan_));
+            ga[0] = ga[2] = gb[0] = gb[2] = nan_;
             break;
           }
           OP_POLL_SLEEP(spin);
@@ -1133,7 +1297,9 @@
         if ((OP_ABLATE & 16) || (!LOSE && ga[1] == e && ga[3] == e && gb[1] == e && gb[3] == e)) break;
         if (LOSE || spin >= OP_SPIN_MAX) {
           atomicOr_system(e_err, 2u);
-          ga[0] = ga[2] = gb[0] = gb[2] = 0x7fc00000u;
+          unsigned nan_ = 0x7fc00000u;
+          asm volatile("" : "+v"(nan_));
+          ga[0] = ga[2] = gb[0] = gb[2] = nan_;
           break;
         }
         OP_POLL_SLEEP(spin);
```
